# lachinov/brats2019

Measured on AMD Instinct MI355X. Metric: volumes_per_sec_fwd_bwd_128cubed_x4ch, higher is better.
Workload: dtype bf16

## Files before the change

brats2019_amd/_lib.py:

```python
from __future__ import annotations

import ctypes as C
import os

import torch

_PKG = os.path.dirname(os.path.abspath(__file__))
LIB_PATH = os.environ.get("RU_LIB_PATH") or os.path.join(_PKG, "lib", "libresunet_hip.so")

_lib = None
PRECISIONS = {"f32": 0, "bf16x3": 1}
GRAD_PRECISIONS = {"bf16x3": 1, "bf16": 2}
FUSE_GN_BWD_STATS, FUSE_GN_BWD_APPLY, FUSE_SIDE_STREAM, FUSE_BATCH_WREDUCE, FUSE_TAIL_FINALIZE, FUSE_PW_DGRAD = 1, 2, 4, 8, 16, 32

_vp, _f, _d, _i, _sz = C.c_void_p, C.c_float, C.c_double, C.c_int, C.c_size_t

SIGNATURES = {
    "ru_last_error": (C.c_char_p, []),
    "ru_version": (_i, []),
    "ru_device_ok": (_i, []),
    "ru_conv3d_workspace_bytes": (_sz, [_i] * 7),
    "ru_conv3d_fwd": (_i, [_vp, _vp, _vp, _vp] + [_i] * 7 + [_vp, _sz, _vp]),
    "ru_conv3d_bwd_data": (_i, [_vp, _vp, _vp] + [_i] * 7 + [_vp, _sz, _vp]),
    "ru_conv3d_fwd_p": (_i, [_vp, _vp, _vp, _vp] + [_i] * 8 + [_vp, _sz, _vp]),
    "ru_conv3d_bwd_data_p": (_i, [_vp, _vp, _vp] + [_i] * 8 + [_vp, _sz, _vp]),
    "ru_conv3d_bwd_weight": (_i, [_vp, _vp, _vp, _vp] + [_i] * 7 + [_vp, _sz, _vp]),
    "ru_conv3d_bwd_weight_p": (_i, [_vp, _vp, _vp, _vp] + [_i] * 8 + [_vp, _sz, _vp]),
    "ru_groupnorm_workspace_bytes": (_sz, [_i, _i, _sz]),
    "ru_groupnorm_fwd": (_i, [_vp] * 7 + [_i, _i, _sz, _i, _f, _f, _vp, _sz, _vp]),
    "ru_groupnorm_bwd": (_i, [_vp] * 9 + [_i, _i, _sz, _i, _f, _vp, _sz, _vp]),
    "ru_leaky_relu_fwd": (_i, [_vp, _vp, _sz, _f, _vp]),
    "ru_leaky_relu_bwd": (_i, [_vp, _vp, _vp, _sz, _f, _vp]),
    "ru_upsample2x_trilinear_fwd": (_i, [_vp, _vp] + [_i] * 5 + [_vp]),
    "ru_upsample2x_trilinear_bwd": (_i, [_vp, _vp] + [_i] * 5 + [_vp]),
    "ru_sigmoid_fwd": (_i, [_vp, _vp, _sz, _vp]),
    "ru_criterion_workspace_bytes": (_sz, [_i, _i, _sz]),
    "ru_criterion_sums": (_i, [_vp, _vp, _vp, _i, _i, _sz, _f, _vp, _sz, _vp]),
    "ru_criterion_grad": (_i, [_vp, _vp, _vp, _d, _f, _f, _f, _f, _vp, _i, _i, _sz, _vp]),
    "ru_criterion_value": (_i, [C.POINTER(_d), _i, _d, _d, C.POINTER(_d), C.POINTER(_d)]),
    "ru_criterion_value_device": (_i, [_vp, _i, _d, _d, _d, _d, _vp, _vp]),
    "ru_crit_moments_workspace_bytes": (_sz, [_i, _i, _sz]),
    "ru_crit_moments": (_i, [_vp, _vp, _i, _i, _sz, C.c_uint, _vp, _vp, _sz, _vp]),
    "ru_crit_reduce": (_i, [_vp, _i, _i, _vp, _vp]),
    "ru_crit_eval": (_i, [_vp, _vp, _i, _i, _d, _d, _vp, _i, _vp, _vp, _vp]),
    "ru_crit_grad": (_i, [_vp, _vp, _vp, _vp, _i, _i, _sz, _i, _vp, _vp]),
    "ru_adam_amsgrad_step": (_i, [_vp] * 5 + [_sz] + [_f] * 5 + [_i, _vp]),
    "ru_adam_step": (_i, [_vp] * 5 + [_sz] + [_f] * 5 + [_i, _vp]),
    "ru_unet_create": (_vp, [_i, C.POINTER(_i), C.POINTER(_i), C.POINTER(_i), _i]),
    "ru_unet_destroy": (None, [_vp]),
    "ru_unet_set_precision": (_i, [_vp, _i]),
    "ru_unet_freeze_params": (_i, [_vp, _i]),
    "ru_unet_get_precision": (_i, [_vp]),
    "ru_unet_set_grad_precision": (_i, [_vp, _i]),
    "ru_unet_get_grad_precision": (_i, [_vp]),
    "ru_unet_set_fusion": (_i, [_vp, C.c_uint]),
    "ru_unet_probe": (_i, [_vp, _i]),
    "ru_unet_probe_read": (_i, [_vp, C.POINTER(C.c_double), C.POINTER(_i)]),
    "ru_unet_probe_read_families": (_i, [_vp, C.POINTER(C.c_double), C.POINTER(_i), _i]),
    "ru_unet_param_count": (_i, [_vp]),
    "ru_unet_param_name": (C.c_char_p, [_vp, _i]),
    "ru_unet_param_ndim": (_i, [_vp, _i]),
    "ru_unet_param_dim": (_i, [_vp, _i, _i]),
    "ru_unet_param_offset": (_sz, [_vp, _i]),
    "ru_unet_param_total": (_sz, [_vp]),
    "ru_unet_param_is_dead": (_i, [_vp, _i]),
    "ru_unet_workspace_bytes": (_sz, [_vp] + [_i] * 5),
    "ru_unet_forward": (_i, [_vp, _vp, _vp, _vp] + [_i] * 5 + [_vp, _sz, _vp]),
    "ru_unet_backward": (_i, [_vp] * 6),
    "ru_unet_backward_criterion": (_i, [_vp, _vp, _vp, _vp, _d, _f, _f, _f, _f, _vp, _vp, _vp]),
    "ru_unet_gn_stats": (_i, [_vp, _i, _vp, _vp, _vp]),
    "ru_comm_unique_id": (_i, [_vp]),
    "ru_comm_init": (_i, [C.POINTER(_vp), _vp, _i, _i]),
    "ru_comm_destroy": (_i, [_vp]),
    "ru_comm_rank": (_i, [_vp]),
    "ru_comm_world": (_i, [_vp]),
    "ru_allreduce": (_i, [_vp, _vp, _sz, _i, _vp]),
    "ru_comm_group_begin": (_i, []),
    "ru_comm_group_end": (_i, []),
    "ru_tta_merge": (_i, [_vp, _i, C.c_uint, _vp, _vp, _vp, _i, _i, _i, _i, _vp]),
    "ru_compose_labels": (_i, [_vp, _vp, C.c_ulonglong, _vp, _sz, _vp]),
    "ru_dice_counts": (_i, [_vp, _vp, _vp, _i, _i, _sz, _vp]),
    "ru_dice_accumulate": (_i, [_vp, _vp, _i, _i, _i, _vp]),
    "ru_hausdorff_workspace_bytes": (_sz, [_i] * 6),
    "ru_hausdorff_sq": (_i, [_vp, _vp] + [_i] * 6 + [_vp, _vp, _sz, _vp]),
    "ru_hausdorff_accumulate": (_i, [_vp, _vp] + [_i] * 4 + [_vp]),
    "ru_label_confusion": (_i, [_vp, _vp, _i, _i, _i, _sz, _vp, _vp, _vp]),
    "ru_overlap_accumulate": (_i, [_vp, _i, _i, _i, _i, _vp, _vp, _vp]),
    "ru_dice1d_accumulate": (_i, [_vp, _vp, _i, _i, _i, _vp]),
# ... 13 lines not shown
    "ru_case_stats": (_i, [_vp, _vp, _i, _i, _i, _i, C.POINTER(_i), C.POINTER(_i), _vp, _sz, _vp]),
    "ru_case_prepare": (_i, [_vp, _vp, _vp, _i, _i, _i, _i, C.POINTER(_i), C.POINTER(_i), C.POINTER(_i), C.POINTER(_i), _i, C.c_uint, _vp]),
    "ru_tta_merge_box": (_i, [_vp, _i, C.c_uint, _vp, _vp, _vp, _i, _i, _i, _i, C.POINTER(_i), C.POINTER(_i), _vp]),
    "ru_cc_workspace_bytes": (_sz, [_i, _i, _i]),
    "ru_cc_reject": (_i, [_vp, _i, _i, _i, _d, _vp, _sz, _vp]),
    "ru_paste_labels": (_i, [_vp, _vp, _i, _i, _i, C.POINTER(_i), C.POINTER(_i), _vp]),
    "ru_postprocess_workspace_bytes": (_sz, [_i, _i, _i, _i]),
    "ru_postprocess_regions": (_i, [_vp, _vp, _i, _i, _i, _i, C.POINTER(C.c_longlong), C.POINTER(C.c_ulonglong), C.c_uint, C.c_uint, _i, _vp, _vp, _vp, _vp, _sz, _vp]),
    "ru_ens_accumulate": (_i, [_vp, _i, C.c_uint, _vp, _i, _i, _i, _i, _i, C.POINTER(_i), C.POINTER(_i), _vp]),
    "ru_ens_finalize": (_i, [_vp, _i, _vp, _vp, _vp, _i, _sz, _vp]),
    "ru_ens_accumulate_finalize": (_i, [_vp, _i, C.c_uint, _vp, _i, _i, _vp, _vp, _vp, _i, _i, _i, _i, C.POINTER(_i), C.POINTER(_i), _vp]),
    "ru_ens_argmax": (_i, [_vp, _i, _vp, _i, _sz, _vp]),
    "ru_paste_probs": (_i, [_vp, _vp, _i, _i, _i, _i, C.POINTER(_i), C.POINTER(_i), _vp]),
    "ru_unc_accumulate": (_i, [_vp, _i, C.c_uint, _vp, _vp, _i, _i, _i, _i, _i, C.POINTER(_i), C.POINTER(_i), _vp]),
    "ru_unc_accumulate_finalize": (_i, [_vp, _i, C.c_uint, _vp, _vp, _i, _i, _i, _vp, _vp, _vp, _vp, _i, _i, _i, _i, C.POINTER(_i), C.POINTER(_i), _vp]),
    "ru_unc_finalize": (_i, [_vp, _vp, _i, _i, _i, _vp, _vp, _vp, _vp, _i, _sz, _vp]),
    "ru_unc_histogram": (_i, [_vp, _vp, _vp, _i, _i, _i, _vp, _vp, _vp]),
    "ru_unc_score": (_i, [_vp, C.POINTER(_i), _i, _vp, _vp, _vp]),
    "ru_paste_u8c": (_i, [_vp, _vp, _i, _i, _i, _i, C.POINTER(_i), C.POINTER(_i), _vp]),
    "ru_zscore_workspace_bytes": (_sz, [_i, _sz]),
    "ru_zscore_stats": (_i, [_vp, _vp, _i, _sz, _vp, _sz, _vp]),
    "ru_augment_patch": (_i, [_vp, _vp, _vp, _vp, _i, _i, _i, _i, _vp, _vp, _vp, _i, _vp, _vp, _vp, _vp, _vp]),
    "ru_augment_patch_soft": (_i, [_vp, _vp, _vp, _vp, _vp, _i, _i, _i, _i, _vp, _vp, _vp, _i, _vp, _vp, _vp, _vp, _vp]),
    "ru_augment_patch_affine": (_i, [_vp, _vp, _vp, _vp, _vp, _i, _i, _i, _i, _vp, _vp, _vp, _i, _vp, _vp, _i, _vp, _vp, _vp]),
    "ru_elastic_workspace_bytes": (_sz, [_i, _i, _i]),
    "ru_elastic_noise": (_i, [C.c_ulonglong, _i, _i, _i, _vp, _vp]),
    "ru_elastic_field": (_i, [_vp, _d, _d, _i, _i, _i, _vp, _vp, _sz, _vp]),
    "ru_elastic_warp": (_i, [_vp, _i, _vp, _i, _vp, _i, _i, _i, _i, _vp, _vp, _vp, _vp, _vp]),
    "ru_intensity_workspace_bytes": (_sz, [_i, _i, _i, _i]),
    "ru_intensity_augment": (_i, [_vp, _vp, _i, _i, _i, _i, _vp, _vp, _sz, _vp]),
    "ru_layout_convert": (_i, [_vp, _vp, _i, _i, _sz, _i, _vp]),
    "ru_upsample2x_trilinear_fwd_l": (_i, [_vp, _vp] + [_i] * 5 + [_f, _vp]),
    "ru_upsample2x_trilinear_bwd_l": (_i, [_vp, _vp] + [_i] * 5 + [_vp]),
    "ru_conv3d_fwd_l": (_i, [_vp, _vp, _vp, _vp] + [_i] * 7 + [_vp, _sz, _vp]),
    "ru_conv3d_bwd_weight_l": (_i, [_vp, _vp, _vp] + [_i] * 7 + [_vp, _sz, _vp]),
    "ru_conv1_l_workspace_bytes": (_sz, [_i, _i, _i]),
    "ru_conv1_l": (_i, [_vp, _i, _vp, _i, _vp, _i, _vp, _vp, _i, _vp, _f, _vp, _f, _i, _i, _sz, _i, _i, _i, _i, _vp, _vp, _f, _vp, _sz,
                        C.POINTER(_i), C.POINTER(_i), _vp, _sz, _vp]),
    "ru_conv3_l_workspace_bytes": (_sz, [_i] * 7),
    "ru_conv3_l": (_i, [_vp, _vp, _vp, _vp] + [_i] * 8 + [_vp, _vp, _vp, _f, _vp, _vp, _i, _i, _vp, _vp, _f, _vp, _sz, C.POINTER(_i), C.POINTER(_i), _vp, _sz, _vp]),
    "ru_wgrad1_l_workspace_bytes": (_sz, [_i, _i, _i, _sz]),
    "ru_wgrad3_l_workspace_bytes": (_sz, [_i] * 7),
    "ru_wgrad3_l": (_i, [_vp, _vp, _vp] + [_i] * 8 + [_vp, _vp, _f, _i, _i, _vp, _vp, _vp, _vp, _vp, _f, _vp, C.POINTER(_i), _vp, _sz, _vp]),
    "ru_wgrad1_l": (_i, [_vp, _vp, _i, _vp, _vp, _i, _i, _i, _i, _sz] + [_i] * 6 + [_vp, _i, _vp, _vp, _f, C.POINTER(_i), _vp, _sz, _vp]),
}


CRIT_KINDS = {"Dice_loss_joint": 0, "BCE_Loss": 1, "MSE_Loss": 2, "CE_Loss": 3, "Dice1D": 4, "GDL_joint": 5, "sens_loss_joint": 6,
              "Dice_loss_separate": 7}
CRIT_MOMENTS, CRIT_MAX_TERMS = 7, 8
CRIT_MASK_LOGS, CRIT_MASK_ALL = (1 << 4) | (1 << 5), 0x7F
CRIT_M_D2 = 6

CONF_PROB, CONF_LABEL, OVERLAP_MAX_LABELS = 0, 1, 8
OVERLAP_MODES = {"itk": 0, "wt": 1, "validate": 2}

UNC_MEASURES = {"std": 0, "entropy": 1}
UNC_REGIONS, UNC_LEVELS, UNC_CLASSES = 3, 101, 4

SURFACE_PROB, SURFACE_LABEL, SURFACE_REGIONS, SURFACE_COUNTS = 0, 1, 3, 6
SURFACE_COLUMNS = {"dice": 0, "sensitivity": 1, "specificity": 2, "hd95": 3}

LESION_COUNTS, LESION_TABLE_COLUMNS, LESION_CHUNK = 6, 5, 8
LESION_COLUMNS = {"dice": 0, "hd95": 1}

POSTPROCESS_MASKS, POSTPROCESS_LABELS, POSTPROCESS_REGIONS, POSTPROCESS_STATS = 0, 1, 3, 6


INT_BLUR, INT_LOWRES, INT_NOISE, INT_BRIGHTNESS, INT_CONTRAST, INT_GAMMA, INT_GAMMA_INVERT, INT_GAMMA_RETAIN = 1, 2, 4, 8, 16, 32, 64, 128
INT_MAXC, INT_MAX_RADIUS = 8, 8


AFFINE_MAPPINGS = {"default": 0, "row": 1, "brick": 2}


class IntensityParams(C.Structure):
    _fields_ = [("mask", _i * 8), ("blur_sigma", _d * 8), ("lowres_zoom", _d * 8), ("noise_variance", _d * 8), ("noise_seed", C.c_ulonglong * 8),
# ... 66 lines not shown
```

brats2019_amd/csrc/engine.hip:

```cpp
#include "ru_common.h"

#include <vector>
#include <math.h>
#include <stdlib.h>
#include <string.h>

#include <string>
#include <vector>

namespace ru {

static thread_local char g_err[512] = "";
void set_error(const char* fmt, ...) {
    va_list ap;
    va_start(ap, fmt);
    vsnprintf(g_err, sizeof(g_err), fmt, ap);
    va_end(ap);
}
int hip_fail(hipError_t e, const char* what) {
    set_error("%s: %s", what, hipGetErrorString(e));
    return RU_EHIP;
}

constexpr float kSlope = 1e-2f;
// ... 15 lines not shown
        return reinterpret_cast<float*>(base + o);
    }
    float* alloc_keep(size_t nfloats) {
        keep += align_up(nfloats * sizeof(float), 256);
        if (dry) return nullptr;
        const size_t top = cap & ~(size_t)255;
        if (off + keep > top) { failed = true; return nullptr; }
        return reinterpret_cast<float*>(base + top - keep);
    }
    void rewind(size_t mark) { off = mark; }
    size_t need() const { return peak + keep; }
};

static bool env_is(const char* name, char c) { const char* e = getenv(name); return e && *e == c; }
Switches switches_from_env() {
    Switches sw;
    sw.wz = !env_is("RU_WZ", '0');
    sw.wz32 = !(conv3_wz16_form_built() && env_is("RU_WZ32", '0'));
    sw.mx = !env_is("RU_MX", '0');
    sw.mx_wz = sw.mx && !env_is("RU_MX", '1');
    sw.mxg = !env_is("RU_MXG", '0');
    sw.head_form = !env_is("RU_HEAD_FORM", '0');
    sw.head_res = !env_is("RU_HEAD_RES", '0');
    return sw;
}
bool env_trace() { static const bool on = [] { const char* e = getenv("RU_TRACE"); return e && *e && *e != '0'; }(); return on; }
bool env_f32c_off() { static const bool off = env_is("RU_F32C", '0'); return off; }
bool env_sb1_no22() { static const bool on = env_is("RU_SB1_NO22", '1'); return on; }
int env_c1_scatter_cob() { static const int forced = [] { const char* e = getenv("RU_C1_SCATTER_COB"); return e ? atoi(e) : 0; }(); return forced; }
bool env_c1_pair_off() { static const bool off = env_is("RU_C1_PAIR", '0'); return off; }
unsigned env_fusion(unsigned fusion) {
    if (env_is("RU_SIDE_STREAM", '0')) fusion &= ~(unsigned)RU_FUSE_SIDE_STREAM;
    if (const char* e = getenv("RU_FUSION_OFF")) fusion &= ~(unsigned)strtoul(e, nullptr, 0);
    if (const char* e = getenv("RU_FUSION_ON")) fusion |= (unsigned)strtoul(e, nullptr, 0) & 63u;
    return fusion;
}

static int trace_sync(const char* what, hipStream_t s) {
    fprintf(stderr, "[ru] %s\n", what);
    const hipError_t e = hipStreamSynchronize(s);
    if (e != hipSuccess) { fprintf(stderr, "[ru]   -> %s\n", hipGetErrorString(e)); return hip_fail(e, what); }
    return RU_OK;
}

enum { FAM_CONV_L0 = 0, FAM_CONV_DEEP, FAM_WGRAD_L0, FAM_WGRAD_DEEP, FAM_GN, FAM_PW, FAM_OTHER, FAM_COUNT };
enum { INST_CONV16_FWD = 0, INST_CONV16_DGRAD, INST_CONV_DEEP_FWD, INST_CONV_DEEP_DGRAD, INST_WGRAD16_FUSED, INST_WGRAD16_PLAIN, INST_WGRAD_DEEP, INST_COUNT };
struct FamilySink {
    std::vector<hipEvent_t> ev;
    std::vector<int> fam;
    std::vector<int> inst;
    size_t used = 0;
    ~FamilySink() { for (hipEvent_t e : ev) (void)hipEventDestroy(e); }
};
static thread_local FamilySink* t_sink = nullptr;
static thread_local int t_hint_c = 16;
static thread_local int t_hint_inst = -1;
struct RedQueues { WgradRedList main, side; hipStream_t side_stream = nullptr; };
static thread_local RedQueues* t_red = nullptr;
static WgradRedList* red_for(hipStream_t s) { return t_red ? ((t_red->side_stream && s == t_red->side_stream) ? &t_red->side : &t_red->main) : nullptr; }
static int family_of(const char* call) {
    auto has = [&](const char* k) { return strstr(call, k) != nullptr; };
    if (has("wgrad3_launch")) return t_hint_c <= 16 ? FAM_WGRAD_L0 : FAM_WGRAD_DEEP;
    if (has("wgrad_reduce_flush")) return FAM_WGRAD_DEEP;
    if (has("conv3_launch") || has("conv3_sb_launch")) return t_hint_c <= 16 ? FAM_CONV_L0 : FAM_CONV_DEEP;
    if (has("gn_")) return FAM_GN;
    if (has("conv1_") || has("wgrad1_launch") || has("up2_") || has("s2d_launch") || has("d2s_launch") || has("lrelu_bwd_launch")) return FAM_PW;
    return FAM_OTHER;
// ... 51 lines not shown
    size_t offset, numel;
    bool dead;
};

struct BlockP {
    int down = -1, conv1 = -1, conv2 = -1, n1w = -1, n1b = -1, n2w = -1, n2b = -1;
    int cin_down = 0, c = 0;
    size_t pk_f1 = 0, pk_f2 = 0, pk_d1 = 0, pk_d2 = 0, pk_downT = 0, pk_down16 = 0;
    size_t fk_f1 = 0, fk_f2 = 0, fk_d1 = 0, fk_d2 = 0;
};

struct GNSave {
    float *mean = nullptr, *rstd = nullptr, *scale = nullptr, *shift = nullptr;
    float act_slope = 0.01f;
    float* k = nullptr;
};

struct BlockSave {
    const BlockP* bp = nullptr;
    const float* xprev = nullptr;
    float* xs2d = nullptr;
    const float* x = nullptr;
    const GNSave* xg = nullptr;
    float *y1 = nullptr, *y2 = nullptr, *out = nullptr;
    GNSave g1, g2;
    int N = 0, C = 0, D = 0, H = 0, W = 0;
};

struct DecSave {
    const float* z = nullptr;
    float *u = nullptr, *v = nullptr, *c = nullptr;
    const float* skip = nullptr;
    int level = 0;
};

constexpr int kOneProduct = 0x100;
struct ru_unet {
    int depth = 0, nout = 0;
    std::vector<int> enc, dec, ch;
    std::vector<ParamInfo> params;
    size_t total = 0;
    std::vector<std::vector<BlockP>> enc_blocks, dec_blocks;
    std::vector<BlockP> first_blocks;
    std::vector<int> up_w, dec1_w;
    std::vector<size_t> pk_upT, pk_decT;
    int conv_in = -1, nin_w = -1, nin_b = -1, conv_out_w = -1, conv_out_b = -1;
    size_t pk_in = 0, pk_out = 0, pk_out_d = 0, pk_total = 0;
    size_t fk_in = 0, fk_out = 0, fk_out_d = 0, fk_total = 0;
    int precision = RU_PREC_F32;
    unsigned fusion = RU_FUSE_GN_BWD_STATS | RU_FUSE_GN_BWD_APPLY | RU_FUSE_SIDE_STREAM | RU_FUSE_BATCH_WREDUCE | RU_FUSE_PW_DGRAD;
    int grad_precision = RU_PREC_BF16X3;
    int grad_products() const { return (precision == RU_PREC_BF16X3 && grad_precision == RU_PREC_BF16) ? 1 : 3; }
    int wgrad_mode() const { return precision | (grad_products() == 1 ? kOneProduct : 0); }
    bool c16 = false;
    char* fpack = nullptr;

    bool have_fwd = false, training = false;
    int N = 0, D = 0, H = 0, W = 0;
    char* ws = nullptr;
    size_t ws_bytes = 0, fwd_end = 0, fwd_keep = 0;
    float* pack = nullptr;
    const float* x_in = nullptr;
    const float* x_in4 = nullptr;
    bool x_in4_planned = false;
    bool params_frozen = false;
    const float* packed_params = nullptr;
    const void* packed_base = nullptr;
    int packed_prec = -1;
    bool packed_c16 = false;
    ru::Switches sw;
    ru::Switches pack_sw;
    float *y0 = nullptr, *t0 = nullptr, *probs = nullptr;
    GNSave g0;
    const float* head_in = nullptr;
    std::vector<BlockSave> first_s;
    std::vector<std::vector<BlockSave>> enc_s, dec_s;
    std::vector<DecSave> dstage;
    std::vector<const float*> skips;
    std::vector<GNSave> gn_order;
    bool probe_on = false;
    bool probe_families = false;
    ru::FamilySink* sink = nullptr;
    std::vector<hipEvent_t> probe_ev;
// ... 111 lines not shown
    h->pk_out_d = h->pk_total; h->pk_total += conv3_packed_floats(number_of_outputs, ch[0]);
    h->fk_total = 0;
    h->fk_in = h->fk_total; h->fk_total += conv3_sb_frag_bytes(kInCh, ch[0]);
    h->fk_out = h->fk_total; h->fk_total += conv3_sb_frag_bytes(ch[0], number_of_outputs);
    h->fk_out_d = h->fk_total; h->fk_total += conv3_sb_frag_bytes(number_of_outputs, ch[0]);
    for (auto& b : h->first_blocks) assign_block_packs(h, b);
    for (auto& lv : h->enc_blocks) for (auto& b : lv) assign_block_packs(h, b);
    for (int i = 0; i < depth - 1; ++i) for (auto& b : h->dec_blocks[i]) assign_block_packs(h, b);
    for (int i = 0; i < depth - 1; ++i) {
        h->pk_upT.push_back(h->pk_total); h->pk_total += (size_t)ch[i + 1] * ch[i];
        h->pk_decT.push_back(h->pk_total); h->pk_total += (size_t)2 * ch[i] * ch[i];
    }
    return h;
}

extern "C" void ru_unet_destroy(ru_unet_t h) { delete h; }
extern "C" int ru_unet_set_precision(ru_unet_t h, int precision) {
    RU_REQUIRE(h && (precision == RU_PREC_F32 || precision == RU_PREC_BF16X3), "ru_unet_set_precision: bad argument");
    h->precision = precision;
    h->have_fwd = false;
    return RU_OK;
}
extern "C" int ru_unet_get_precision(ru_unet_t h) { return h ? h->precision : -1; }
extern "C" int ru_unet_set_fusion(ru_unet_t h, unsigned mask) {
    RU_REQUIRE(h && (mask & ~(unsigned)(RU_FUSE_GN_BWD_STATS | RU_FUSE_GN_BWD_APPLY | RU_FUSE_SIDE_STREAM | RU_FUSE_BATCH_WREDUCE | RU_FUSE_TAIL_FINALIZE | RU_FUSE_PW_DGRAD)) == 0, "ru_unet_set_fusion: bad argument");
    if ((mask & RU_FUSE_TAIL_FINALIZE) && !h->tickets) {
        hipError_t e = hipMalloc((void**)&h->tickets, 256 * sizeof(unsigned));
        if (e != hipSuccess) { h->tickets = nullptr; (void)hipGetLastError(); }
    }
    h->fusion = mask;
    h->have_fwd = false;
    return RU_OK;
}
extern "C" int ru_unet_probe(ru_unet_t h, int enable) {
    RU_REQUIRE(h, "ru_unet_probe: null handle");
    h->probe_on = enable == 1;
    h->probe_families = enable == 2;
    h->probe_used = 0;
    if (h->probe_families && !h->sink) h->sink = new ru::FamilySink();
    if (h->sink) h->sink->used = 0;
    return RU_OK;
}
extern "C" int ru_unet_probe_read_families(ru_unet_t h, double* ms, int* launches, int nfam) {
    RU_REQUIRE(h && ms && launches && (nfam == ru::FAM_COUNT || nfam == ru::FAM_COUNT + ru::INST_COUNT),
               "ru_unet_probe_read_families: %d families (+ %d instance rows behind them)", (int)ru::FAM_COUNT, (int)ru::INST_COUNT);
    for (int f = 0; f < nfam; ++f) { ms[f] = 0.0; launches[f] = 0; }
    if (!h->sink) return RU_OK;
    ru::FamilySink& k = *h->sink;
    for (size_t i = 0; i + 1 < k.used; i += 2) {
        hipError_t e = hipEventSynchronize(k.ev[i + 1]);
        if (e != hipSuccess) return hip_fail(e, "hipEventSynchronize(family probe)");
        float t = 0.f;
        e = hipEventElapsedTime(&t, k.ev[i], k.ev[i + 1]);
        if (e != hipSuccess) return hip_fail(e, "hipEventElapsedTime(family probe)");
        ms[k.fam[i / 2]] += t;
        launches[k.fam[i / 2]] += 1;
        const int in = k.inst[i / 2];
        if (in >= 0 && ru::FAM_COUNT + in < nfam) { ms[ru::FAM_COUNT + in] += t; launches[ru::FAM_COUNT + in] += 1; }
    }
    k.used = 0;
    return RU_OK;
}
extern "C" int ru_unet_probe_read(ru_unet_t h, double* total_ms, int* launches) {
    RU_REQUIRE(h && total_ms && launches, "ru_unet_probe_read: null argument");
    double sum = 0.0;
    for (size_t i = 0; i + 1 < h->probe_used; i += 2) {
// ... 246 lines not shown
    }
    const float* cur = stem_fused ? h->y0 : h->t0;
    h->first_s.assign(h->first_blocks.size(), BlockSave());
    for (size_t j = 0; j < h->first_blocks.size(); ++j) {
        rc = block_fwd(h, params, A, s, h->first_blocks[j], cur, N, Dl[0], Hl[0], Wl[0], h->first_s[j], &cur, (stem_fused && j == 0) ? &h->g0 : nullptr);
        if (rc) return rc;
    }
    h->skips.assign(depth - 1, nullptr);
    h->enc_s.assign(depth - 1, {});
    for (int i = 0; i < depth - 1; ++i) {
        h->skips[i] = cur;
        h->enc_s[i].assign(h->enc_blocks[i].size(), BlockSave());
        for (size_t j = 0; j < h->enc_blocks[i].size(); ++j) {
            const int lv = j == 0 ? i : i + 1;
            rc = block_fwd(h, params, A, s, h->enc_blocks[i][j], cur, N, Dl[lv], Hl[lv], Wl[lv], h->enc_s[i][j], &cur);
            if (rc) return rc;
        }
    }
    h->dstage.assign(depth - 1, DecSave());
    h->dec_s.assign(depth - 1, {});
    for (int i = depth - 2; i >= 0; --i) {
        DecSave& ds = h->dstage[i];
        ds.level = i;
        ds.z = cur;
        ds.skip = h->skips[i];
        const int Ci = h->ch[i], Cc = h->ch[i + 1];
        const bool recycle = !h->training;
        float* c_early = recycle ? A.alloc((size_t)N * Ci * Vl(i)) : nullptr;
        const size_t dmark = A.off;
        if (!h->c16) {
            ds.u = A.alloc((size_t)N * Cc * Vl(i));
            RU_RUN(up2_fwd_launch(cur, ds.u, N, Cc, Dl[i + 1], Hl[i + 1], Wl[i + 1], s));
        }
        ds.v = A.alloc((size_t)N * Ci * Vl(i));
        Conv1Args c1{};
        c1.x0 = ds.u; c1.C0 = Cc; c1.y = ds.v; c1.out_slope = kSlope;
        c1.N = N; c1.Cout = Ci; c1.V = Vl(i);
        ds.c = recycle ? c_early : A.alloc((size_t)N * Ci * Vl(i));
        Conv1Args c2{};
        c2.x0 = ds.skip; c2.C0 = Ci; c2.x1 = ds.v; c2.C1 = Ci;
        c2.y = ds.c; c2.out_slope = 1.f; c2.N = N; c2.Cout = Ci; c2.V = Vl(i);
        if (h->c16) {
            float* zc = A.alloc((size_t)N * Ci * Vl(i + 1));
            c1.x0 = cur; c1.y = zc; c1.out_slope = 1.f; c1.V = Vl(i + 1);
            c1.wT = P(h, params, h->up_w[i]); c1.ldw = Cc;
            RU_RUN(conv1_16_launch(c1, s));
            RU_RUN(up2_fwd16_launch(zc, ds.v, N, Ci, Dl[i + 1], Hl[i + 1], Wl[i + 1], kSlope, s));
            c2.wT = P(h, params, h->dec1_w[i]); c2.ldw = 2 * Ci;
            RU_RUN(conv1_16_launch(c2, s));
        } else {
            c1.wT = h->pack + h->pk_upT[i]; c1.ldw = Ci;
            RU_RUN(conv1_launch(c1, s));
            c2.wT = h->pack + h->pk_decT[i]; c2.ldw = Ci;
            RU_RUN(conv1_launch(c2, s));
        }
        if (recycle) A.rewind(dmark);
        cur = ds.c;
        h->dec_s[i].assign(h->dec_blocks[i].size(), BlockSave());
        for (size_t j = 0; j < h->dec_blocks[i].size(); ++j) {
            const bool defer = i == 0 && j + 1 == h->dec_blocks[i].size() && h->c16 &&
                               (h->precision == RU_PREC_BF16X3 ? conv3_sb_head_takes_residual(h->sw, N, C0, h->nout, Dl[0], Hl[0], Wl[0])
                                                               : (!h->training && conv3_f32c_head_takes_residual(h->sw, C0, h->nout, Wl[0])));
            rc = block_fwd(h, params, A, s, h->dec_blocks[i][j], cur, N, Dl[i], Hl[i], Wl[i], h->dec_s[i][j], &cur, nullptr, defer);
            if (rc) return rc;
            if (defer) head_block = &h->dec_s[i][j];
        }
    }
    h->head_in = cur;
    t_hint_c = C0;
    float* pdst = probs_out;
    h->probs = probs_out;
    Conv3Args a{};
    a.x = cur; a.wp = h->pack + h->pk_out; a.bias = P(h, params, h->conv_out_b); a.y = pdst; a.sigmoid = 1;
    a.mode = h->precision; a.wfrag = h->fpack + h->fk_out; a.in_c16 = h->c16;
    a.N = N; a.Cin = C0; a.Cout = h->nout; a.D = Dl[0]; a.H = Hl[0]; a.W = Wl[0];
    if (head_block) {
        a.x = head_block->y2; a.in_scale = head_block->g2.scale; a.in_shift = head_block->g2.shift; a.in_slope = kSlope; a.in_res = head_block->x;
        a.in_sum_out = head_block->out;
    }
    RU_RUN(conv3_launch(a, h->sw, s));
// ... 285 lines not shown
    const BlockSave* hb = (depth >= 2 && !h->dec_s[0].empty()) ? &h->dec_s[0].back() : nullptr;
    FusedSums hsums;
    if (head4 && hb && !no_bst && conv3_sb_bst_usable(N, C0, Dl[0], Hl[0], Wl[0])) {
        dh.bst_y = hb->y2; dh.bst_k = hb->g2.k; dh.bst_slope = kSlope;
        hsums.nblk = sb_nblk(h, dh);
        hsums.part = A.alloc((size_t)N * C0 * hsums.nblk * 2);
        hsums.coef = A.alloc((size_t)N * C0 * 3);
        dh.stat_partials = hsums.part;
        if (!A.dry && h->tails()) {
            const BlockP& lb = *hb->bp;
            fill_bwd_tail(h, dh.fin, hsums, hb->g2, P(h, params, lb.n2w), G(h, grads, lb.n2w), G(h, grads, lb.n2b), N, C0, Vl(0), 1);
            hsums.done = true;
        }
    }
    RU_RUN(conv3_launch(dh, h->sw, s));
    const float* dcur = dcur_buf;
    std::vector<const float*> dskip(depth - 1, nullptr);
    FusedSums carry = hsums;
    for (int i = 0; i <= depth - 2; ++i) {
        for (int j = (int)h->dec_s[i].size() - 1; j >= 0; --j) {
            const bool fused2 = carry.nblk > 0 && j == (int)h->dec_s[i].size() - 1;
            const FusedSums sin = carry;
            rc = block_bwd(h, params, grads, A, s, h->dec_s[i][j], dcur, &dcur, nullptr, nullptr, fused2 ? &sin : nullptr);
            if (rc) return rc;
        }
        carry = FusedSums();
        const DecSave& ds = h->dstage[i];
        const int Ci = h->ch[i], Cc = h->ch[i + 1];
        const size_t V = Vl(i);
        const float* wdec = P(h, params, h->dec1_w[i]);
        float* gdec = G(h, grads, h->dec1_w[i]);
        float* dsk = A.alloc((size_t)N * Ci * V);
        float* dv = A.alloc((size_t)N * Ci * V);
        float* dpre = A.alloc((size_t)N * Ci * V);
        const bool dg_fused = c16 && Ci <= 32 && (h->fusion & RU_FUSE_PW_DGRAD);
        if (c16) {
            Wgrad1Args w{};
            w.x = ds.skip; w.x1 = ds.v; w.C0 = Ci; w.dy = dcur; w.dw = gdec; w.ldw = 2 * Ci; w.c16 = 1; w.defer = red_for(s);
            w.ws_bytes = wgrad1_workspace_bytes(N, 2 * Ci, Ci, V);
            w.ws = A.alloc(w.ws_bytes / sizeof(float));
            w.N = N; w.Cin = 2 * Ci; w.Cout = Ci; w.V = V;
            if (dg_fused) { w.dg_w = wdec; w.dg_ldw = 2 * Ci; w.dg_y0 = dsk; w.dg_y1 = dpre; w.dg_mask_slope = kSlope; }
            RU_RUN(wgrad1_launch(w, s));
        } else {
            rc = wgrad1_run(A, s, ds.skip, dcur, gdec, 2 * Ci, N, Ci, Ci, V, c16);
            if (rc) return rc;
            rc = wgrad1_run(A, s, ds.v, dcur, A.dry ? nullptr : gdec + Ci, 2 * Ci, N, Ci, Ci, V, c16);
            if (rc) return rc;
        }
        Conv1Args a1{};
        a1.x0 = dcur; a1.C0 = Ci; a1.y = dsk; a1.out_slope = 1.f; a1.N = N; a1.Cout = Ci; a1.V = V;
        Conv1Args a2 = a1;
        a2.y = dv;
        if (dg_fused) {
        } else if (c16) {
            a1.wT = h->pack + h->pk_decT[i]; a1.ldw = Ci;
            a2.wT = h->pack + h->pk_decT[i] + (size_t)Ci * Ci; a2.ldw = Ci;
            a2.y = dpre; a2.mask = ds.v; a2.mask_slope = kSlope;
            Conv1Args a12 = a1;
            a12.Cout = 2 * Ci; a12.Cout0 = Ci; a12.y1 = dpre; a12.mask = ds.v; a12.mask_slope = kSlope;
            RU_RUN(conv1_16_launch(a12, s));
        } else {
            a1.wT = wdec; a1.ldw = 2 * Ci;
            a2.wT = A.dry ? nullptr : wdec + Ci; a2.ldw = 2 * Ci;
            RU_RUN(conv1_launch(a1, s));
            RU_RUN(conv1_launch(a2, s));
        }
        dskip[i] = dsk;
        if (!c16) RU_RUN(lrelu_bwd_launch(ds.v, dv, dpre, (size_t)N * Ci * V, kSlope, s));
        Conv1Args a3{};
        a3.x0 = dpre; a3.C0 = Ci; a3.out_slope = 1.f; a3.N = N; a3.Cout = Cc; a3.V = V;
        float* dz = A.alloc((size_t)N * Cc * Vl(i + 1));
        float* du = nullptr;
        if (c16) {
            float* dzc = A.alloc((size_t)N * Ci * Vl(i + 1));
            RU_RUN(up2_bwd16_launch(dpre, dzc, N, Ci, Dl[i + 1], Hl[i + 1], Wl[i + 1], s));
            rc = wgrad1_run(A, s, ds.z, dzc, G(h, grads, h->up_w[i]), Cc, N, Cc, Ci, Vl(i + 1), true);
            if (rc) return rc;
            a3.x0 = dzc; a3.y = dz; a3.V = Vl(i + 1);
            a3.wT = h->pack + h->pk_upT[i]; a3.ldw = Ci;
            carry = FusedSums();
            const BlockSave* zb = (i + 1 <= depth - 2) ? (!h->dec_s[i + 1].empty() ? &h->dec_s[i + 1].back() : nullptr)
                                  : (!h->enc_s[depth - 2].empty() ? &h->enc_s[depth - 2].back() : nullptr);
            if (zb && (zb->g2.k || A.dry) && (h->fusion & RU_FUSE_GN_BWD_STATS) && conv1_16_bst_nblk(a3) > 0) {
                carry.nblk = conv1_16_bst_nblk(a3);
                carry.part = A.alloc((size_t)N * Cc * carry.nblk * 2);
                carry.coef = A.alloc((size_t)N * Cc * 3);
                a3.bst_y = zb->y2; a3.bst_k = zb->g2.k; a3.bst_slope = kSlope; a3.stat_partials = carry.part;
            }
            RU_RUN(conv1_16_launch(a3, s));
        } else {
            rc = wgrad1_run(A, s, ds.u, dpre, G(h, grads, h->up_w[i]), Cc, N, Cc, Ci, V, false);
            if (rc) return rc;
            du = A.alloc((size_t)N * Cc * V);
            a3.y = du;
            a3.wT = P(h, params, h->up_w[i]); a3.ldw = Cc;
            RU_RUN(conv1_launch(a3, s));
            RU_RUN(up2_bwd_launch(du, dz, N, Cc, Dl[i + 1], Hl[i + 1], Wl[i + 1], s));
        }
        dcur = dz;
    }
    for (int i = depth - 2; i >= 0; --i) {
        bool joined = false;
        FusedSums snext = carry;
        carry = FusedSums();
        for (int j = (int)h->enc_s[i].size() - 1; j >= 0; --j) {
            GNNext nx{};
            nx.slope = kSlope;
            const BlockSave* pb = j >= 1 ? &h->enc_s[i][j - 1] : (i >= 1 ? (h->enc_s[i - 1].empty() ? nullptr : &h->enc_s[i - 1].back())
// ... 441 lines not shown

extern "C" int ru_tta_merge(const float* probs, int K, unsigned flips, float* mean_out, unsigned char* mask, unsigned long long* counts,
                            int C, int D, int H, int W, ru_stream_t stream) {
    RU_REQUIRE(probs && mask && counts, "ru_tta_merge: null argument");
    return tta_merge_launch(probs, K, flips, mean_out, mask, counts, C, D, H, W, (hipStream_t)stream);
}
extern "C" int ru_compose_labels(const unsigned char* mask, const unsigned long long* counts, unsigned long long et_min, unsigned char* labels,
                                 size_t V, ru_stream_t stream) {
    RU_REQUIRE(mask && counts && labels, "ru_compose_labels: null argument");
    return compose_labels_launch(mask, counts, et_min, labels, V, (hipStream_t)stream);
}

extern "C" int ru_dice_accumulate(const unsigned long long* counts, double* acc, int N, int C, int nacc, ru_stream_t stream) {
    return dice_accumulate_launch(counts, acc, N, C, nacc, (hipStream_t)stream);
}
extern "C" int ru_dice_counts(const float* p, const float* g, unsigned long long* counts, int N, int C, size_t V, ru_stream_t stream) {
    RU_REQUIRE(p && g && counts && N > 0 && C > 0, "ru_dice_counts: bad argument");
    return dice_counts_launch(p, g, counts, N * C, V, (hipStream_t)stream);
}

extern "C" int ru_layout_convert(const float* src, float* dst, int N, int C, size_t V, int to_c16, ru_stream_t stream) {
    RU_REQUIRE(src && dst && N > 0, "ru_layout_convert: bad argument");
    return layout_convert_launch(src, dst, N, C, V, to_c16, (hipStream_t)stream);
}

extern "C" int ru_upsample2x_trilinear_fwd_l(const float* x, float* y, int N, int C, int D, int H, int W, float out_slope, ru_stream_t stream) {
    RU_REQUIRE(x && y && N > 0 && C > 0 && D > 0 && H > 0 && W > 0, "ru_upsample2x_trilinear_fwd_l: bad argument");
    return up2_fwd16_launch(x, y, N, C, D, H, W, out_slope, (hipStream_t)stream);
}
extern "C" int ru_upsample2x_trilinear_bwd_l(const float* dy, float* dx, int N, int C, int D, int H, int W, ru_stream_t stream) {
    RU_REQUIRE(dy && dx && N > 0 && C > 0 && D > 0 && H > 0 && W > 0, "ru_upsample2x_trilinear_bwd_l: bad argument");
    return up2_bwd16_launch(dy, dx, N, C, D, H, W, (hipStream_t)stream);
}
extern "C" int ru_conv3d_fwd_l(const float* x, const float* w, const float* bias, float* y, int N, int Cin, int Cout, int D, int H, int W,
                               int flags, void* ws, size_t ws_bytes, ru_stream_t stream) {
    RU_REQUIRE(x && w && y, "ru_conv3d_fwd_l: null argument");
    const Switches sw = switches_from_env();
    hipStream_t s = (hipStream_t)stream;
    WsCarver C(ws, ws_bytes);
    Conv3Args a{};
    void* wf = C.take(conv3_sb_frag_bytes(Cin, Cout) / 4 + 64);
    RU_WS_OK(C);
    const bool f32 = (flags & 16) != 0;
    a.products = (flags & 32) ? 2 : 0;
    RU_REQUIRE(!f32 || ((flags & 3) != 0 && !(flags & (4 | 8))), "ru_conv3d_fwd_l: the exact-f32 form needs a voxel-major side and takes neither the 4-channel copy nor a split-form input");
    const bool gop = (flags & 64) && !f32 && (flags & 3) == 3 && !(flags & (4 | 8)) && !bias && conv3_mxg_usable(sw, N, Cin, Cout, D, H, W);
    int rc = f32 ? conv3_f32c_pack_weights(w, wf, Cin, Cout, 0, s) : conv3_sb_pack_weights(w, wf, Cin, Cout, 0, s, gop);
    if (rc) return rc;
    a.mode = f32 ? RU_PREC_F32 : RU_PREC_BF16X3; a.wfrag = wf;
    a.in_c16 = flags & 1; a.out_c16 = (flags >> 1) & 1;
    a.in_s16 = (flags >> 3) & 1;
    RU_REQUIRE(!a.in_s16 || a.in_c16, "ru_conv3d_fwd_l: the split form is a voxel-major layout");
    a.x = x; a.bias = bias; a.y = y; a.N = N; a.Cin = Cin; a.Cout = Cout; a.D = D; a.H = H; a.W = W;
    if (gop) {
        const size_t nvox = (size_t)N * D * H * W;
        float* g16 = C.take(nvox * 16);
        RU_WS_OK(C);
        rc = conv3_mxg_split_launch(x, g16, nvox, s);
        if (rc) return rc;
        a.x = g16; a.in_s16 = 1; a.in_g16 = 1; a.products = 0;
    }
    if (flags & 4) {
        RU_REQUIRE(!(flags & 1) && conv3_sb4_usable(N, Cin, Cout, D, H, W), "ru_conv3d_fwd_l: shape does not fit the 4-channel kernel");
        const size_t V = (size_t)D * H * W;
        float* x4 = C.take((size_t)N * 4 * V);
        void* wf4 = C.take(conv3_sb4_frag_bytes(Cout) / 4 + 64);
        RU_WS_OK(C);
        rc = pad_to_c4_launch(x, x4, N, Cin, V, s);
        if (rc) return rc;
        rc = conv3_sb4_pack_weights(w, wf4, Cin, Cout, 0, s);
        if (rc) return rc;
        a.x = x4; a.wfrag = wf4; a.in_c4 = 1;
    }
    return f32 ? conv3_launch(a, sw, s) : conv3_sb_launch(a, sw, s);
}

extern "C" int ru_conv3d_bwd_weight_l(const float* x, const float* dy, float* dw, int N, int Cin, int Cout, int D, int H, int W,
                                      int flags, void* ws, size_t ws_bytes, ru_stream_t stream) {
    RU_REQUIRE(x && dy && dw, "ru_conv3d_bwd_weight_l: null argument");
    WsCarver C(ws, ws_bytes);
    Wgrad3Args a{};
    a.x = x; a.dy = dy; a.dw = dw; a.mode = RU_PREC_BF16X3; a.x_c16 = flags & 1; a.dy_c16 = (flags >> 1) & 1;
    a.N = N; a.Cin = Cin; a.Cout = Cout; a.D = D; a.H = H; a.W = W;
    a.ws_bytes = wgrad3_workspace_bytes(N, Cin, Cout, D, H, W);
    a.ws = C.take(a.ws_bytes / 4);
    RU_WS_OK(C);
    return wgrad3_launch(a, (hipStream_t)stream);
}

extern "C" size_t ru_conv1_l_workspace_bytes(int C0, int Cout, int s2d) {
    return 4096 + (s2d ? 2 * align_up((size_t)C0 * Cout * sizeof(float), 256) : 0);
}
extern "C" int ru_conv1_l(const float* x0, int C0, const float* x1, int C1, const float* w, int ldw, float* y, float* y1, int Cout0,
                          const float* add, float out_slope, const float* mask, float mask_slope, int N, int Cout, size_t V,
                          int s2d, int Dc, int Hc, int Wc, const float* bst_y, const float* bst_k, float bst_slope,
                          float* stat_partials, size_t stat_floats, int* nblk, int* inst, void* ws, size_t ws_bytes, ru_stream_t stream) {
    RU_REQUIRE(x0 && w && y, "ru_conv1_l: null argument");
    RU_REQUIRE(s2d >= 0 && s2d <= 2, "ru_conv1_l: s2d is 0 (plain), 1 (gather) or 2 (scatter)");
    hipStream_t s = (hipStream_t)stream;
    WsCarver C(ws, ws_bytes);
    Conv1Args a{};
    a.x0 = x0; a.C0 = C0; a.x1 = x1; a.C1 = C1; a.wT = w; a.ldw = ldw; a.y = y; a.add = add; a.out_slope = out_slope;
    a.N = N; a.Cout = Cout; a.V = V; a.s2d = s2d; a.Dc = Dc; a.Hc = Hc; a.Wc = Wc; a.mask = mask; a.mask_slope = mask_slope;
    a.y1 = y1; a.Cout0 = Cout0; a.bst_y = bst_y; a.bst_k = bst_k; a.bst_slope = bst_slope; a.stat_partials = stat_partials;
    if (s2d) {
        RU_REQUIRE(C0 > 0 && Cout > 0 && (s2d == 1 ? C0 : Cout) % 8 == 0, "ru_conv1_l: stride-2 modes need 8 x channels on the gathered side");
        const int co = s2d == 1 ? Cout : C0, ci = (s2d == 1 ? C0 : Cout) / 8;
        float* wd = C.take((size_t)8 * ci * co);
        float* wdT = C.take((size_t)8 * ci * co);
        RU_WS_OK(C);
        int rc = pack_down16_launch(w, wd, wdT, co, ci, s);
        if (rc) return rc;
        a.wT = s2d == 1 ? wd : wdT;
        a.ldw = C0;
    }
    if (inst) *inst = conv1_16_choose(a).packed();
    if (nblk) *nblk = 0;
    if (bst_y) {
        const int nb = conv1_16_bst_nblk(a);
        RU_REQUIRE(nb == 0 || (stat_partials && stat_floats >= (size_t)N * (s2d == 2 ? Cout / 8 : Cout) * nb * 2), "ru_conv1_l: statistics buffer too small");
        if (nblk) *nblk = nb;
    }
    return conv1_16_launch(a, s);
}

static size_t c3l_frag_bytes(int Cin, int Cout) { const size_t sb = conv3_sb_frag_bytes(Cin, Cout), f = conv3_f32c_frag_bytes(Cin, Cout); return sb > f ? sb : f; }
extern "C" size_t ru_conv3_l_workspace_bytes(int N, int Cin, int Cout, int D, int H, int W, int flags) {
    const size_t nvox = (size_t)N * D * H * W;
    return 4096 + align_up(c3l_frag_bytes(Cin, Cout) + 256, 256) + ((flags & 4) ? align_up(nvox * 16, 256) + align_up(conv3_sb4_frag_bytes(Cout) + 256, 256) : 0) +
           ((flags & 64) ? align_up(nvox * 64, 256) : 0);
}
extern "C" int ru_conv3_l(const float* x, const float* w, const float* bias, float* y, int N, int Cin, int Cout, int D, int H, int W, int flags, int weight_mode,
                          const float* add, const float* in_scale, const float* in_shift, float in_slope, const float* in_res, float* in_sum_out,
                          int sigmoid, int products, const float* bst_y, const float* bst_k, float bst_slope, float* stat_partials, size_t stat_floats,
                          int* nblk, int* route, void* ws, size_t ws_bytes, ru_stream_t stream) {
    RU_REQUIRE(x && w && y, "ru_conv3_l: null argument");
    RU_REQUIRE(N > 0 && Cin > 0 && Cout > 0 && D > 0 && H > 0 && W > 0, "ru_conv3_l: bad shape");
// ... 16 lines not shown
    RU_REQUIRE(!a.in_s16 || a.in_c16, "ru_conv3_l: the split form is a voxel-major layout");
    a.x = x; a.bias = bias; a.y = y; a.N = N; a.Cin = Cin; a.Cout = Cout; a.D = D; a.H = H; a.W = W;
    a.add = add; a.in_scale = in_scale; a.in_shift = in_shift; a.in_slope = in_slope; a.in_res = in_res; a.in_sum_out = in_sum_out; a.sigmoid = sigmoid;
    a.bst_y = bst_y; a.bst_k = bst_k; a.bst_slope = bst_slope; a.stat_partials = stat_partials;
    if (gop) {
        const size_t nvox = (size_t)N * D * H * W;
        float* g16 = C.take(nvox * 16);
        RU_WS_OK(C);
        rc = conv3_mxg_split_launch(x, g16, nvox, s);
        if (rc) return rc;
        a.x = g16; a.in_s16 = 1; a.in_g16 = 1; a.products = 0;
    }
    if (flags & 4) {
        RU_REQUIRE(!(flags & 1) && conv3_sb4_usable(N, Cin, Cout, D, H, W), "ru_conv3_l: shape does not fit the 4-channel kernel");
        const size_t V = (size_t)D * H * W;
        float* x4 = C.take((size_t)N * 4 * V);
        void* wf4 = C.take(conv3_sb4_frag_bytes(Cout) / 4 + 64);
        RU_WS_OK(C);
        rc = pad_to_c4_launch(x, x4, N, Cin, V, s);
        if (rc) return rc;
        rc = conv3_sb4_pack_weights(w, wf4, Cin_f, Cout_f, weight_mode, s);
        if (rc) return rc;
        a.x = x4; a.wfrag = wf4; a.in_c4 = 1;
    }
    const int r = f32 ? conv3_f32c_route(a) : conv3_sb_route(a, sw);
    if (route) *route = r;
    const int nb = f32 ? conv3_f32c_tiles_per_sample(N, Cin, Cout, D, H, W) : conv3_sb_route_nblk(r, N, Cout, D, H, W);
    if (nblk) *nblk = nb;
    RU_REQUIRE(!stat_partials || stat_floats >= (size_t)N * Cout * nb * 2, "ru_conv3_l: statistics buffer too small");
    return f32 ? conv3_launch(a, sw, s) : conv3_sb_launch(a, sw, s);
}

extern "C" size_t ru_wgrad1_l_workspace_bytes(int N, int Cin, int Cout, size_t V) { return 4096 + align_up(wgrad1_workspace_bytes(N, Cin, Cout, V), 256); }
extern "C" int ru_wgrad1_l(const float* x, const float* x1, int C0, const float* dy, float* dw, int ldw, int N, int Cin, int Cout, size_t V,
                           int c16, int s2d, int Dc, int Hc, int Wc, int tap_split, const float* dg_w, int dg_ldw, float* dg_y0, float* dg_y1,
                           float dg_mask_slope, int* inst, void* ws, size_t ws_bytes, ru_stream_t stream) {
    RU_REQUIRE(x && dy && dw, "ru_wgrad1_l: null argument");
    WsCarver C(ws, ws_bytes);
    Wgrad1Args a{};
    a.x = x; a.x1 = x1; a.C0 = C0; a.dy = dy; a.dw = dw; a.ldw = ldw; a.N = N; a.Cin = Cin; a.Cout = Cout; a.V = V;
    a.c16 = c16; a.s2d = s2d; a.Dc = Dc; a.Hc = Hc; a.Wc = Wc; a.tap_split = tap_split;
    a.dg_w = dg_w; a.dg_ldw = dg_ldw; a.dg_y0 = dg_y0; a.dg_y1 = dg_y1; a.dg_mask_slope = dg_mask_slope;
    RU_REQUIRE(N > 0 && Cin > 0 && Cout > 0 && V > 0, "ru_wgrad1_l: bad shape");
    a.ws_bytes = wgrad1_workspace_bytes(N, Cin, Cout, V);
    a.ws = C.take(a.ws_bytes / 4);
    RU_WS_OK(C);
    if (inst) *inst = wgrad1_inst(a);
    return wgrad1_launch(a, (hipStream_t)stream);
}

extern "C" size_t ru_wgrad3_l_workspace_bytes(int N, int Cin, int Cout, int D, int H, int W, int flags) {
    return 4096 + align_up(wgrad3_tr_workspace_bytes(N, Cin, Cout, D, H, W), 256) + ((flags & 2) ? align_up((size_t)N * D * H * W * 16, 256) : 0) + ((flags & 4) ? align_up((size_t)N * D * H * W * 16, 256) : 0);
}
extern "C" int ru_wgrad3_l(const float* x, const float* dy, float* dw, int N, int Cin, int Cout, int D, int H, int W, int flags, int products,
                           const float* in_scale, const float* in_shift, float in_slope, int dw_cin, int dw_cout,
                           const float* gb_y, const float* gb_d, const float* gb_scale, const float* gb_shift, const float* gb_coef, float gb_slope, float* gb_out,
                           int* inst, void* ws, size_t ws_bytes, ru_stream_t stream) {
    RU_REQUIRE(x && (dy || gb_y) && dw, "ru_wgrad3_l: null argument");
    RU_REQUIRE(N > 0 && Cin > 0 && Cout > 0 && D > 0 && H > 0 && W > 0, "ru_wgrad3_l: bad shape");
    hipStream_t s = (hipStream_t)stream;
    WsCarver C(ws, ws_bytes);
    Wgrad3Args a{};
    a.x = x; a.dy = dy ? dy : gb_y; a.dw = dw; a.mode = RU_PREC_BF16X3; a.x_c16 = 1; a.dy_c16 = 1;
    a.N = N; a.Cin = Cin; a.Cout = Cout; a.D = D; a.H = H; a.W = W;
    a.in_scale = in_scale; a.in_shift = in_shift; a.in_slope = in_slope; a.dw_cin = dw_cin; a.dw_cout = dw_cout;
    a.dy_s16 = flags & 1; a.x_c4 = (flags >> 1) & 1; a.dy_c4 = (flags >> 2) & 1; a.swapped = (flags >> 3) & 1; a.gb_g16 = (flags >> 4) & 1; a.products = products;
    a.gb_y = gb_y; a.gb_d = gb_d; a.gb_scale = gb_scale; a.gb_shift = gb_shift; a.gb_coef = gb_coef; a.gb_slope = gb_slope; a.gb_out = gb_out;
    a.ws_bytes = wgrad3_tr_workspace_bytes(N, Cin, Cout, D, H, W);
    a.ws = C.take(a.ws_bytes / 4);
    RU_WS_OK(C);
    for (int side = 0; side < 2; ++side) {
        if (!(side == 0 ? a.x_c4 : a.dy_c4)) continue;
        const int cfew = side == 0 ? dw_cin : dw_cout;
        const size_t V = (size_t)D * H * W;
        RU_REQUIRE(cfew > 0 && cfew <= 4 && (side == 0 || dy), "ru_wgrad3_l: a 4-channel copy holds 1..4 channels (dw_cin / dw_cout)");
// ... 47 lines not shown
```

brats2019_amd/csrc/pointwise_c16.hip:

```cpp
#include "pw_helpers.hpp"
#include "fin_tail.hpp"
#include <type_traits>
#include <stdlib.h>

namespace ru {

typedef float f32x4_c16 __attribute__((ext_vector_type(4)));
template <int I, int N, class F> __device__ __forceinline__ void static_for_c1_impl(F&& f) {
    if constexpr (I < N) { f(std::integral_constant<int, I>{}); static_for_c1_impl<I + 1, N>(f); }
}
template <int N, class F> __device__ __forceinline__ void static_for_c1(F&& f) { static_for_c1_impl<0, N>(f); }

static inline dim3 c16_grid(size_t V, int blocks_nc, unsigned cap = 2048) {
    size_t bx = (V * 4 + 255) / 256;
    if (bx > cap) bx = cap;
    if (bx < 1) bx = 1;
    return dim3((unsigned)bx, (unsigned)blocks_nc);
}

template <int RES, bool NT = false>
__global__ __launch_bounds__(256) void gn_apply16_kernel(const float* __restrict__ x, const float* __restrict__ scale, const float* __restrict__ shift,
                                                         const float* __restrict__ res, float* __restrict__ y, int C, size_t V, float slope,
                                                         const float* __restrict__ rscale, const float* __restrict__ rshift, float rslope) {
    const int nb = blockIdx.y, CB = C >> 4;
// ... 209 lines not shown
#undef RU_UPX
#pragma unroll
        for (int dz = 0; dz < 2; ++dz) {
            const int zo = 2 * kz + 1 + dz;
            if (zo < 0 || zo >= Do) continue;
            int z0, z1; float lz0, lz1;
            up2_src(zo, D, z0, z1, lz0, lz1);
#pragma unroll
            for (int dy = 0; dy < 2; ++dy) {
                const int yo = 2 * ky + 1 + dy;
                if (yo < 0 || yo >= Ho) continue;
                int y0, y1; float ly0, ly1;
                up2_src(yo, H, y0, y1, ly0, ly1);
                float4 o;
#define RU_UP2(c) o.c = lrelu(lz0 * (ly0 * e00.c + ly1 * e01.c) + lz1 * (ly0 * e10.c + ly1 * e11.c), slope)
                RU_UP2(x); RU_UP2(y); RU_UP2(z); RU_UP2(w);
#undef RU_UP2
                if (nt_out) __builtin_nontemporal_store(f32x4_c16{o.x, o.y, o.z, o.w}, reinterpret_cast<f32x4_c16*>(yp + (((size_t)zo * Ho + yo) * Wo + xo) * 4 + q));
                else yp[(((size_t)zo * Ho + yo) * Wo + xo) * 4 + q] = o;
            }
        }
    }
}
int up2_fwd16_launch(const float* x, float* y, int N, int C, int D, int H, int W, float slope, hipStream_t s) {
    RU_REQUIRE(C % 16 == 0, "up2_fwd16: C must be a multiple of 16");
    const size_t total = (size_t)(D + 1) * (H + 1) * (2 * W) * 4;
    size_t bx = (total + 255) / 256;
    if (bx > 16384) bx = 16384;
    hipLaunchKernelGGL(up2_fwd16_kernel, dim3((unsigned)bx, (unsigned)(N * (C / 16))), dim3(256), 0, s, x, y, D, H, W, slope);
    RU_CHECK_LAUNCH("up2_fwd16_kernel");
    return RU_OK;
}

#ifndef RU_UP2B_ZC
#define RU_UP2B_ZC 8
#endif
constexpr int UP2B_ZC = RU_UP2B_ZC;
__global__ __launch_bounds__(256) void up2_bwd16_kernel(const float* __restrict__ dy, float* __restrict__ dx, int D, int H, int W) {
    const int Do = 2 * D, Ho = 2 * H, Wo = 2 * W;
    const size_t nb = blockIdx.y;
    const size_t Vi = (size_t)D * H * W, Vo = Vi * 8;
    const float4* dp = reinterpret_cast<const float4*>(dy) + nb * Vo * 4;
    float4* op = reinterpret_cast<float4*>(dx) + nb * Vi * 4;
    const int nch = (D + UP2B_ZC - 1) / UP2B_ZC;
    const size_t total = (size_t)nch * H * W * 4;
    for (size_t f = (size_t)blockIdx.x * 256 + threadIdx.x; f < total; f += (size_t)gridDim.x * 256) {
        const int q = (int)(f & 3);
        size_t r = f >> 2;
        const int kx = (int)(r % W); r /= W;
        const int ky = (int)(r % H);
        const int k0 = (int)(r / H) * UP2B_ZC;
        const int k1 = k0 + UP2B_ZC < D ? k0 + UP2B_ZC : D;
        float wy[4], wx[4];
        size_t oy[4], ox[4];
#pragma unroll
        for (int t = 0; t < 4; ++t) {
            const int y = 2 * ky - 1 + t, xx = 2 * kx - 1 + t;
            wy[t] = (y >= 0 && y < Ho) ? up2_coef(y, H, ky) : 0.f;
            wx[t] = (xx >= 0 && xx < Wo) ? up2_coef(xx, W, kx) : 0.f;
            oy[t] = (size_t)(y < 0 ? 0 : (y >= Ho ? Ho - 1 : y)) * Wo;
            ox[t] = (size_t)(xx < 0 ? 0 : (xx >= Wo ? Wo - 1 : xx)) * 4 + q;
        }
        float4 accP = make_float4(0.f, 0.f, 0.f, 0.f), accC = accP;
        for (int m = k0; m <= k1; ++m) {
#pragma unroll
            for (int h = 0; h < 2; ++h) {
                const int z = 2 * m - 1 + h;
                const bool in = z >= 0 && z < Do;
                const size_t zrow = (size_t)(z < 0 ? 0 : (z >= Do ? Do - 1 : z)) * Ho * Wo;
                float4 pz = make_float4(0.f, 0.f, 0.f, 0.f);
#pragma unroll
                for (int b = 0; b < 4; ++b) {
                    const float4* row = dp + (zrow + oy[b]) * 4;
                    const float4 p0 = row[ox[0]], p1 = row[ox[1]], p2 = row[ox[2]], p3 = row[ox[3]];
                    pz.x += wy[b] * (wx[0] * p0.x + wx[1] * p1.x + wx[2] * p2.x + wx[3] * p3.x);
                    pz.y += wy[b] * (wx[0] * p0.y + wx[1] * p1.y + wx[2] * p2.y + wx[3] * p3.y);
                    pz.z += wy[b] * (wx[0] * p0.z + wx[1] * p1.z + wx[2] * p2.z + wx[3] * p3.z);
                    pz.w += wy[b] * (wx[0] * p0.w + wx[1] * p1.w + wx[2] * p2.w + wx[3] * p3.w);
                }
                const float cP = (in && m - 1 >= k0) ? up2_coef(z, D, m - 1) : 0.f;
                const float cC = (in && m < k1) ? up2_coef(z, D, m) : 0.f;
                accP.x += cP * pz.x; accP.y += cP * pz.y; accP.z += cP * pz.z; accP.w += cP * pz.w;
                accC.x += cC * pz.x; accC.y += cC * pz.y; accC.z += cC * pz.z; accC.w += cC * pz.w;
            }
            if (m - 1 >= k0) op[(((size_t)(m - 1) * H + ky) * W + kx) * 4 + q] = accP;
            accP = accC;
            accC = make_float4(0.f, 0.f, 0.f, 0.f);
        }
    }
}
int up2_bwd16_launch(const float* dy, float* dx, int N, int C, int D, int H, int W, hipStream_t s) {
    RU_REQUIRE(C % 16 == 0, "up2_bwd16: C must be a multiple of 16");
    const size_t total = (size_t)((D + UP2B_ZC - 1) / UP2B_ZC) * H * W * 4;
    size_t bx = (total + 255) / 256;
    if (bx > 16384) bx = 16384;
    hipLaunchKernelGGL(up2_bwd16_kernel, dim3((unsigned)bx, (unsigned)(N * (C / 16))), dim3(256), 0, s, dy, dx, D, H, W);
    RU_CHECK_LAUNCH("up2_bwd16_kernel");
    return RU_OK;
}

__global__ void pack_down16_kernel(const float* __restrict__ w, float* __restrict__ wd, float* __restrict__ wdT, int Cout, int Cin) {
    const int i = blockIdx.x * blockDim.x + threadIdx.x;
    if (i >= Cout * Cin * 8) return;
    const int tap = i & 7, c = (i >> 3) % Cin, o = i / (8 * Cin);
    const float v = w[i];
    wd[(size_t)o * 8 * Cin + tap * Cin + c] = v;
    wdT[(size_t)(tap * Cin + c) * Cout + o] = v;
}
int pack_down16_launch(const float* w, float* wd, float* wdT, int Cout, int Cin, hipStream_t s) {
    const int total = Cout * Cin * 8;
    hipLaunchKernelGGL(pack_down16_kernel, dim3(cdiv(total, 256)), dim3(256), 0, s, w, wd, wdT, Cout, Cin);
    RU_CHECK_LAUNCH("pack_down16_kernel");
    return RU_OK;
}

template <int COB, int S2D, int NSLOT, bool PAIR = false>
__global__ __launch_bounds__(256, (PAIR || NSLOT > 0) ? 2 : 1) void conv1_16_kernel(const Conv1Args a, int nvt) {
    static_assert(!PAIR || (S2D == 2 && COB == 4 && (NSLOT == 1 || NSLOT == 2)), "paired stores: the scatter mode with statistics, four blocks per workgroup");
    constexpr bool BST = NSLOT > 0;
    constexpr int NSL = BST ? NSLOT : 1;
    __shared__ float red[BST ? 4 * NSL * 16 * 2 : 1];
    const int lane = threadIdx.x & 63, wave = threadIdx.x >> 6;
    const int n = blockIdx.z, cog = blockIdx.y;
    const size_t V = a.V;
    const int r = lane & 15, g = lane >> 4;
    const int nkb0 = a.C0 >> 4, nkb1 = a.C1 >> 4, nkb = nkb0 + nkb1, CBo = a.Cout >> 4;
    const int Hf = 2 * a.Hc, Wf = 2 * a.Wc;
    const size_t Vf = V * 8;
    const int CBf_out = CBo >> 3;
    const int Cstat = S2D == 2 ? (a.Cout >> 3) : a.Cout;
    f32x4_c16 bs1[NSL], bs2[NSL], bk[NSL][3];
    if constexpr (BST) {
#pragma unroll
        for (int sl = 0; sl < NSL; ++sl) {
            bs1[sl] = f32x4_c16{0.f, 0.f, 0.f, 0.f}; bs2[sl] = f32x4_c16{0.f, 0.f, 0.f, 0.f};
            const int cob = cog * COB + sl, chb = S2D == 2 ? cob % CBf_out : cob;
            const float* kp = a.bst_k + (size_t)n * 3 * Cstat + (cob < CBo ? chb : 0) * 16 + 4 * g;
#pragma unroll
            for (int t3 = 0; t3 < 3; ++t3) { const float4 q = *reinterpret_cast<const float4*>(kp + (size_t)t3 * Cstat); bk[sl][t3] = f32x4_c16{q.x, q.y, q.z, q.w}; }
        }
    }
    const bool nt_out = (size_t)a.N * a.Cout * V * sizeof(float) >= ((size_t)128 << 20);
    const int vt = blockIdx.x * 4 + wave;
    const bool live = vt < nvt;
    if (!live) { if constexpr (!BST) return; }
    if (live) {
    const size_t v0 = (size_t)vt * 64;
    size_t vb[4], fv[4];
#pragma unroll
    for (int t = 0; t < 4; ++t) {
        size_t v = v0 + 16 * t + r;
        if (v >= V) v = V - 1;
        vb[t] = v * 16 + 4 * g;
        fv[t] = 0;
        if constexpr (S2D != 0) {
            const int xc = (int)(v % a.Wc);
            const size_t rr = v / a.Wc;
            const int yc = (int)(rr % a.Hc), zc = (int)(rr / a.Hc);
            fv[t] = ((size_t)(2 * zc) * Hf + 2 * yc) * Wf + 2 * xc;
        }
    }
    const float* wrow[COB];
#pragma unroll
    for (int cb = 0; cb < COB; ++cb) {
        const int cob = cog * COB + cb;
        wrow[cb] = a.wT + (size_t)((cob < CBo ? cob : CBo - 1) * 16 + r) * a.ldw + 4 * g;
    }
    f32x4_c16 acc[4][COB];
#pragma unroll
    for (int t = 0; t < 4; ++t)
#pragma unroll
        for (int cb = 0; cb < COB; ++cb) acc[t][cb] = f32x4_c16{0.f, 0.f, 0.f, 0.f};
    const int CBf_in = nkb0 >> 3;
    auto kstep = [&](int kb) __attribute__((always_inline)) {
        float4 xb[4];
        if constexpr (S2D == 1) {
            const int tap = kb / CBf_in, cbf = kb - tap * CBf_in;
            const size_t toff = ((size_t)(tap >> 2) * Hf + ((tap >> 1) & 1)) * Wf + (tap & 1);
            const float* src = a.x0 + ((size_t)(n * CBf_in + cbf) * Vf) * 16 + 4 * g;
#pragma unroll
            for (int t = 0; t < 4; ++t) xb[t] = *reinterpret_cast<const float4*>(src + (fv[t] + toff) * 16);
        } else {
            const float* src = kb < nkb0 ? a.x0 + ((size_t)(n * nkb0 + kb) * V) * 16 : a.x1 + ((size_t)(n * nkb1 + kb - nkb0) * V) * 16;
#pragma unroll
            for (int t = 0; t < 4; ++t) xb[t] = *reinterpret_cast<const float4*>(src + vb[t]);
        }
#pragma unroll
        for (int cb = 0; cb < COB; ++cb) {
            const float4 wv = *reinterpret_cast<const float4*>(wrow[cb] + kb * 16);
#pragma unroll
            for (int t = 0; t < 4; ++t) {
                acc[t][cb] = __builtin_amdgcn_mfma_f32_16x16x4f32(wv.x, xb[t].x, acc[t][cb], 0, 0, 0);
                acc[t][cb] = __builtin_amdgcn_mfma_f32_16x16x4f32(wv.y, xb[t].y, acc[t][cb], 0, 0, 0);
                acc[t][cb] = __builtin_amdgcn_mfma_f32_16x16x4f32(wv.z, xb[t].z, acc[t][cb], 0, 0, 0);
                acc[t][cb] = __builtin_amdgcn_mfma_f32_16x16x4f32(wv.w, xb[t].w, acc[t][cb], 0, 0, 0);
            }
        }
    };
    int kb = 0;
    for (; kb + 1 < nkb; kb += 2) { kstep(kb); kstep(kb + 1); }
    if (kb < nkb) kstep(kb);
    if constexpr (PAIR) {
        const int k = r & 1;
        constexpr int CBf = NSLOT;
        const bool has_add = a.add != nullptr;
        const float* addp = has_add ? a.add : a.bst_y;
#pragma unroll
        for (int t = 0; t < 4; ++t) {
            size_t idx[2][2];
            bool ok[2];
            int srcl[2];
            float4 dadd[2][2], dyq[2][2];
#pragma unroll
            for (int h = 0; h < 2; ++h) {
// ... 185 lines not shown
    }
    if constexpr (BST) {
#pragma unroll
        for (int sl = 0; sl < NSL; ++sl) {
#pragma unroll
            for (int e = 0; e < 4; ++e) {
#pragma unroll
                for (int o = 1; o < 16; o <<= 1) { bs1[sl][e] += __shfl_xor(bs1[sl][e], o); bs2[sl][e] += __shfl_xor(bs2[sl][e], o); }
            }
            if (r == 0) {
#pragma unroll
                for (int e = 0; e < 4; ++e) { red[((wave * NSL + sl) * 16 + 4 * g + e) * 2] = bs1[sl][e]; red[((wave * NSL + sl) * 16 + 4 * g + e) * 2 + 1] = bs2[sl][e]; }
            }
        }
        __syncthreads();
        const int nblk = S2D == 2 ? gridDim.x * gridDim.y : gridDim.x;
        const int blk = S2D == 2 ? blockIdx.y * gridDim.x + blockIdx.x : blockIdx.x;
        for (int i = threadIdx.x; i < NSL * 16; i += 256) {
            const int slot = i >> 4, c = i & 15;
            const int cob0 = cog * COB + slot;
            if (cob0 >= CBo) continue;
            const int chb = S2D == 2 ? cob0 % CBf_out : cob0;
            float u1 = 0.f, u2 = 0.f;
#pragma unroll
            for (int w = 0; w < 4; ++w) { u1 += red[((w * NSL + slot) * 16 + c) * 2]; u2 += red[((w * NSL + slot) * 16 + c) * 2 + 1]; }
            float* p = a.stat_partials + (((size_t)n * Cstat + chb * 16 + c) * nblk + blk) * 2;
            p[0] = u1; p[1] = u2;
        }
    }
}
Conv1Inst conv1_16_choose(const Conv1Args& a) {
    const int CBo = a.Cout / 16;
    Conv1Inst c{CBo >= 4 ? 4 : (CBo >= 2 ? 2 : 1), a.s2d, 0, 0};
    if (a.s2d == 2) {
        const int forced = env_c1_scatter_cob();
        if ((forced == 2 || forced == 4 || forced == 1) && forced <= CBo) c.cob = forced;
    }
    if (a.bst_y) c.nslot = a.s2d == 2 ? (CBo >> 3) : c.cob;
    c.pair = a.s2d == 2 && a.bst_y && !env_c1_pair_off() && a.Wc % 8 == 0 && c.cob == 4 && !a.mask && (c.nslot == 1 || c.nslot == 2);
    return c;
}
int conv1_16_bst_nblk(const Conv1Args& a) {
    if (a.s2d == 1 || a.y1 || a.Cout % 16 || a.V == 0) return 0;
    const int nvt = (int)((a.V + 63) / 64), CBo = a.Cout / 16;
    const int cob = conv1_16_choose(a).cob;
    const int gx = cdiv(nvt, 4), gy = cdiv(CBo, cob);
    if (a.s2d == 2) {
        const int cbf = CBo >> 3;
        if (a.Cout % 128 || (cbf != 1 && cbf != 2 && cbf != 4) || !(cob % cbf == 0 || cbf % cob == 0)) return 0;
        if (cbf > cob) return 0;
        return gx * gy;
    }
    return gx;
}
int conv1_16_launch(const Conv1Args& a, hipStream_t s) {
    RU_REQUIRE(a.N > 0 && a.C0 > 0 && a.Cout > 0 && a.V > 0, "conv1_16: bad shape");
    RU_REQUIRE(a.C0 % 16 == 0 && a.C1 % 16 == 0 && a.Cout % 16 == 0 && a.ldw >= a.C0 + a.C1 && a.ldw % 4 == 0, "conv1_16: channels must be multiples of 16");
    RU_REQUIRE(!a.y1 || (!a.s2d && !a.add && a.Cout0 > 0 && a.Cout0 < a.Cout && a.Cout0 % 16 == 0), "conv1_16: a split output needs the plain mode, no residual and a split at a multiple of 16");
    if (a.s2d) {
        RU_REQUIRE(a.Dc > 0 && a.Hc > 0 && a.Wc > 0 && (size_t)a.Dc * a.Hc * a.Wc == a.V && a.C1 == 0, "conv1_16: bad stride-2 geometry");
        RU_REQUIRE(a.s2d == 1 ? a.C0 % 128 == 0 : a.Cout % 128 == 0, "conv1_16: stride-2 modes need 8 x (multiple of 16) channels");
    }
    const int nvt = (int)((a.V + 63) / 64), CBo = a.Cout / 16;
    const Conv1Inst c = conv1_16_choose(a);
    const bool bst = a.bst_y != nullptr;
    RU_REQUIRE(!bst || (a.bst_k && a.stat_partials && a.s2d != 1 && !a.y1 && conv1_16_bst_nblk(a) > 0), "conv1_16: fused GroupNorm-backward statistics need the plain or scatter mode with whole channel blocks per workgroup");
    dim3 grid((unsigned)cdiv(nvt, 4), (unsigned)cdiv(CBo, c.cob), (unsigned)a.N);
    switch (c.packed()) {
#define RU_C1_CASE(COB_, S2D_, NSLOT_, PAIR_)                                                                      \
    case COB_ | (S2D_ << 4) | (NSLOT_ << 8) | (PAIR_ << 12):                                                        \
        hipLaunchKernelGGL((conv1_16_kernel<COB_, S2D_, NSLOT_, PAIR_ != 0>), grid, dim3(256), 0, s, a, nvt);       \
        break
        RU_C1_CASE(4, 0, 0, 0); RU_C1_CASE(2, 0, 0, 0); RU_C1_CASE(1, 0, 0, 0);
        RU_C1_CASE(4, 0, 4, 0); RU_C1_CASE(2, 0, 2, 0); RU_C1_CASE(1, 0, 1, 0);
        RU_C1_CASE(4, 1, 0, 0); RU_C1_CASE(2, 1, 0, 0); RU_C1_CASE(1, 1, 0, 0);
        RU_C1_CASE(4, 2, 0, 0); RU_C1_CASE(2, 2, 0, 0); RU_C1_CASE(1, 2, 0, 0);
        RU_C1_CASE(4, 2, 1, 1); RU_C1_CASE(4, 2, 2, 1);
        RU_C1_CASE(4, 2, 1, 0); RU_C1_CASE(4, 2, 2, 0); RU_C1_CASE(4, 2, 4, 0);
        RU_C1_CASE(2, 2, 1, 0); RU_C1_CASE(2, 2, 2, 0); RU_C1_CASE(1, 2, 1, 0);
#undef RU_C1_CASE
    default:
        set_error("conv1_16: no kernel for cob %d, mode %d, %d statistic slots", c.cob, c.s2d, c.nslot);
        return RU_EINVAL;
    }
    RU_CHECK_LAUNCH("conv1_16_kernel");
    return RU_OK;
}

}
```

brats2019_amd/csrc/pw_helpers.hpp:

```cpp
#pragma once
#include "ru_common.h"

namespace ru {

__device__ __forceinline__ float wave_sum(float v) {
#pragma unroll
    for (int o = 32; o > 0; o >>= 1) v += __shfl_xor(v, o);
    return v;
}
__device__ __forceinline__ double wave_sum_d(double v) {
#pragma unroll
    for (int o = 32; o > 0; o >>= 1) v += __shfl_xor(v, o);
    return v;
}
__device__ __forceinline__ float block_sum(float v, float* buf) {
    v = wave_sum(v);
    __syncthreads();
    if ((threadIdx.x & 63) == 0) buf[threadIdx.x >> 6] = v;
    __syncthreads();
    return buf[0] + buf[1] + buf[2] + buf[3];
}
__device__ __forceinline__ double block_sum_d(double v, double* buf) {
    v = wave_sum_d(v);
    __syncthreads();
    if ((threadIdx.x & 63) == 0) buf[threadIdx.x >> 6] = v;
    __syncthreads();
    return buf[0] + buf[1] + buf[2] + buf[3];
}
__device__ __forceinline__ float lrelu(float v, float slope) { return v > 0.f ? v : v * slope; }

static inline unsigned grid1d(size_t n, int per_block, unsigned cap = 1u << 20) {
    size_t b = (n + per_block - 1) / per_block;
    if (b < 1) b = 1;
    return (unsigned)(b > cap ? cap : b);
}

typedef __bf16 pw_bf16x2 __attribute__((ext_vector_type(2)));
typedef unsigned int pw_u32x4 __attribute__((ext_vector_type(4)));
__device__ __forceinline__ void pw_split8(const float (&t)[8], pw_u32x4& hi, pw_u32x4& lo) {
    split_n<4>(t, hi, lo);
}

__device__ __forceinline__ void up2_src(int o, int n, int& i0, int& i1, float& l0, float& l1) {
    float src = 0.5f * (float)o - 0.25f;
    if (src < 0.f) src = 0.f;
    i0 = (int)src;
    l1 = src - (float)i0;
    l0 = 1.f - l1;
    i1 = i0 + (i0 < n - 1 ? 1 : 0);
}

__device__ __forceinline__ float up2_coef(int o, int n, int k) {
    int i0, i1; float l0, l1;
    up2_src(o, n, i0, i1, l0, l1);
    return (i0 == k ? l0 : 0.f) + (i1 == k ? l1 : 0.f);
}

}
```

brats2019_amd/csrc/ru_common.h:

```cpp
#pragma once
#include <hip/hip_runtime.h>
#include <stddef.h>
#include <stdint.h>
#include <stdio.h>
#include <stdarg.h>

#include <vector>

#include "../../include/resunet_hip.h"
#include "switches.hpp"

namespace ru {

typedef __bf16 ru_bf16x2 __attribute__((ext_vector_type(2)));
__device__ __forceinline__ void split_pair(float a, float b, unsigned& hb, unsigned& lb) {
    ru_bf16x2 h;
    h[0] = (__bf16)a;
    h[1] = (__bf16)b;
    hb = __builtin_bit_cast(unsigned, h);
    const float h0 = __builtin_bit_cast(float, __builtin_amdgcn_perm(hb, hb, 0x01000c0cu));
    const float h1 = __builtin_bit_cast(float, hb & 0xffff0000u);
    ru_bf16x2 l;
    l[0] = (__bf16)(a - h0);
    l[1] = (__bf16)(b - h1);
// ... 212 lines not shown
size_t wgrad3_workspace_bytes(int N, int Cin, int Cout, int D, int H, int W);
int wgrad3_launch(const Wgrad3Args& a, hipStream_t s);
struct WgradRedEntry { const float* partials; float* dw; int nparts, taps, CoP, CiP, Cout, Cin, so, sc, split, flip, lo, blk0; };
struct WgradRedList { std::vector<WgradRedEntry> e; };
int wgrad_reduce_launch(const float* partials, int nparts, int taps, int CoP, int CiP, int Cout, int Cin, float* dw, int so, int sc, int split, hipStream_t s,
                        int flip_taps = 0, WgradRedList* defer = nullptr);
int wgrad_reduce_flush(WgradRedList& l, hipStream_t s);
size_t wgrad3_sb_workspace_bytes(int N, int Cin, int Cout, int D, int H, int W);
int wgrad3_sb_launch(const Wgrad3Args& a, hipStream_t s);
size_t wgrad3_tr_workspace_bytes(int N, int Cin, int Cout, int D, int H, int W);
int wgrad3_tr_launch(const Wgrad3Args& a, hipStream_t s);
int wgrad3_tr_inst(const Wgrad3Args& a);

struct Wgrad1Args {
    const float* x;
    const float* dy;
    float* dw;
    int ldw;
    void* ws;
    size_t ws_bytes;
    int N, Cin, Cout;
    size_t V;
    int c16;
    int s2d, Dc, Hc, Wc;
    int tap_split;
    const float* x1;
    int C0;
    struct WgradRedList* defer;
    const float* dg_w;
    int dg_ldw;
    float* dg_y0;
    float* dg_y1;
    float dg_mask_slope;
};
size_t wgrad1_workspace_bytes(int N, int Cin, int Cout, size_t V);
int wgrad1_launch(const Wgrad1Args& a, hipStream_t s);
int wgrad1_inst(const Wgrad1Args& a);

struct Conv1Args {
    const float* x0; int C0;
    const float* x1; int C1;
    const float* wT;
    int ldw;
    float* y;
    const float* add;
    float out_slope;
    int N, Cout;
    size_t V;
    int s2d, Dc, Hc, Wc;
    const float* mask;
    float mask_slope;
    float* y1;
    int Cout0;
    const float* bst_y;
    const float* bst_k;
    float bst_slope;
    float* stat_partials;
};
int conv1_16_bst_nblk(const Conv1Args& a);
int conv1_launch(const Conv1Args& a, hipStream_t s);
int transpose_launch(const float* src, float* dst, int rows, int cols, hipStream_t s);
int layout_convert_launch(const float* src, float* dst, int N, int C, size_t V, int to_c16, hipStream_t s);
int pad_to_c16_launch(const float* src, float* dst, int N, int C, size_t V, hipStream_t s);
int pad_to_c4_launch(const float* src, float* dst, int N, int C, size_t V, hipStream_t s);

int s2d_launch(const float* x, float* y, int N, int C, int D, int H, int W, hipStream_t s);
int d2s_launch(const float* y, float* x, int N, int C, int D, int H, int W, hipStream_t s);

int gn_stats_tiles(size_t V);
int gn_stats_launch(const float* x, float* partials, int N, int C, size_t V, hipStream_t s);
int gn_finalize_launch(const float* partials, int nblk, const float* gamma, const float* beta, float* mean, float* rstd,
                       float* scale, float* shift, int N, int C, size_t V, int G, float eps, hipStream_t s, float* bst_k = nullptr,
                       bool centred = false);
int gn_apply_launch(const float* x, const float* scale, const float* shift, const float* res, float* y,
                    int N, int C, size_t V, float slope, hipStream_t s);
int gn_bwd_tiles(size_t V);
int gn_bwd_reduce_launch(const float* x, const float* dy, const float* scale, const float* shift, const float* mean,
                         const float* rstd, float slope, float* partials, int N, int C, size_t V, int G, hipStream_t s);
int gn_bwd_finalize_launch(const float* partials, int nblk, const float* gamma, const float* mean, const float* rstd,
                           float* coef, float* dgamma, float* dbeta, int N, int C, size_t V, int G, hipStream_t s, int s2_sign = 0);
bool conv3_sb_bst_usable(int N, int Cout, int D, int H, int W);
int gn_bwd_apply_launch(const float* x, const float* dy, const float* scale, const float* shift, const float* coef,
                        float slope, float* dx, int N, int C, size_t V, hipStream_t s);

int lrelu_fwd_launch(const float* x, float* y, size_t n, float slope, hipStream_t s);
int lrelu_bwd_launch(const float* y, const float* dy, float* dx, size_t n, float slope, hipStream_t s);
int sigmoid_launch(const float* x, float* y, size_t n, hipStream_t s);
int sigmoid_bwd_launch(const float* p, const float* dp, float* dz, size_t n, hipStream_t s);
int add_launch(const float* a, const float* b, float* y, size_t n, hipStream_t s);
int fill_launch(float* p, float v, size_t n, hipStream_t s);
int up2_fwd_launch(const float* x, float* y, int N, int C, int D, int H, int W, hipStream_t s);
int up2_bwd_launch(const float* dy, float* dx, int N, int C, int D, int H, int W, hipStream_t s);
int bias_grad_launch(const float* dy, float* db, int N, int C, size_t V, void* ws, size_t ws_bytes, hipStream_t s);
size_t bias_grad_workspace_bytes(int N, int C, size_t V);
int head_grad_c4_launch(const float* p, const float* dp, float* d4, float* db, int N, int C, size_t V, void* ws, size_t ws_bytes, hipStream_t s);
struct CritGradArgs { const float* target; const double* sums; double count; float w_dice, w_bce, bgw, priority; };
int head_grad_c4_crit_launch(const float* p, const CritGradArgs& cg, float* d4, float* db, int N, int C, size_t V, void* ws, size_t ws_bytes, hipStream_t s);

int gn_apply16_launch(const float* x, const float* scale, const float* shift, const float* res, float* y, int N, int C, size_t V, float slope, hipStream_t s,
                      const float* rscale = nullptr, const float* rshift = nullptr, float rslope = 1.f);
int gn_bwd_tiles16(size_t V);
int gn_bwd_reduce16_launch(const float* x, const float* dy, const float* scale, const float* shift, const float* mean, const float* rstd,
                           float slope, float* partials, int N, int C, size_t V, int G, hipStream_t s, const FinTail* fin = nullptr);
int gn_bwd_apply16_launch(const float* x, const float* dy, const float* scale, const float* shift, const float* coef, float slope, float* dx,
                          int N, int C, size_t V, int split, hipStream_t s);
int up2_fwd16_launch(const float* x, float* y, int N, int C, int D, int H, int W, float slope, hipStream_t s);
int up2_bwd16_launch(const float* dy, float* dx, int N, int C, int D, int H, int W, hipStream_t s);
int pack_down16_launch(const float* w, float* wd, float* wdT, int Cout, int Cin, hipStream_t s);
int conv1_16_launch(const Conv1Args& a, hipStream_t s);
struct Conv1Inst { int cob, s2d, nslot, pair; int packed() const { return cob | (s2d << 4) | (nslot << 8) | (pair << 12); } };
Conv1Inst conv1_16_choose(const Conv1Args& a);

int crit_tiles(size_t total);
int crit_sums_launch(const float* p, const float* g, double* sums, int N, int C, size_t V, float bgw, void* ws, size_t ws_bytes, hipStream_t s);
int crit_grad_launch(const float* p, const float* g, const double* sums, double count, float w_dice, float w_bce,
                     float bgw, float priority, float* dp, int N, int C, size_t V, hipStream_t s);
int crit_value_launch(const double* sums, int C, double count, double priority, double w_dice, double w_bce, double* out3, hipStream_t s);
int tta_merge_launch(const float* p, int K, unsigned flips, float* mean_out, unsigned char* mask, unsigned long long* counts, int C, int D, int H, int W, hipStream_t s);
int compose_labels_launch(const unsigned char* mask, const unsigned long long* counts, unsigned long long et_min, unsigned char* labels, size_t V, hipStream_t s);
int dice_counts_launch(const float* p, const float* g, unsigned long long* counts, int rows, size_t V, hipStream_t s);
int dice_accumulate_launch(const unsigned long long* counts, double* acc, int N, int C, int nacc, hipStream_t s);
constexpr int RU_AUG_MAXC = 8;
struct AugmentArgs {
    const float* image;
    const unsigned char* label;
    const float* soft;
    float* data;
    float* target;
    int C, D, H, W;
    int lo[3], P[3];
    double scale[3];
    int flags;
    float mean[RU_AUG_MAXC], istd[RU_AUG_MAXC], gain[RU_AUG_MAXC], bias[RU_AUG_MAXC];
};
size_t zscore_workspace_bytes(int C, size_t V);
int zscore_stats_launch(const float* x, double* stats, int C, size_t V, void* ws, size_t ws_bytes, hipStream_t s);
int augment_patch_launch(const AugmentArgs& a, hipStream_t s);
int adam_launch(float* w, const float* g, float* m, float* v, float* vmax, size_t n, float lr, float b1, float b2,
                float eps, float wd, int step, hipStream_t s);

}
```

brats2019_amd/csrc/wgrad_f32.hip:

```cpp
#include "ru_common.h"

namespace ru {

typedef float f32x4 __attribute__((ext_vector_type(4)));

constexpr int pad2mod4(int v) { return v + ((2 - (v & 3)) & 3); }

template <int TZ, int TY, int OT, int CT>
struct W3 {
    static constexpr int HZ = TZ + 2, HY = TY + 2, HX = 18;
    static constexpr int HVOL = HZ * HY * HX, TVOL = TZ * TY * 16;
    static constexpr int DS = pad2mod4(TVOL), CS = pad2mod4(HVOL);
    static constexpr int LDS_FLOATS = OT * 16 * DS + CT * 16 * CS;
};

template <int NSX, int NSD>
struct W3Slots {
    int gx[NSX];
    int lx[NSX];
    long gd[NSD];
    int n;
};

template <int TZ, int TY, int OT, int CT>
__global__ __launch_bounds__(512, 4) void wgrad3_f32_kernel(const Wgrad3Args a, float* __restrict__ partials,
                                                           int ntz, int nty, int ntx, int ncg, int CoP, int CiP) {
    using P = W3<TZ, TY, OT, CT>;
    constexpr int DS = P::DS, CS = P::CS, HY = P::HY, HX = P::HX, HVOL = P::HVOL, TVOL = P::TVOL;
    constexpr int NROW = P::HZ * HY;
    constexpr int NT = 512;
    constexpr int NSX = (NROW * 6 + NT - 1) / NT;
    constexpr int Q4 = TVOL / 4;
    constexpr int NSD = (OT * 16 * Q4 + NT - 1) / NT;
// ... 344 lines not shown
        hipError_t e = hipFuncSetAttribute(reinterpret_cast<const void*>(wgrad3_f32_kernel<TZ, TY, OT, CT>),
                                           hipFuncAttributeMaxDynamicSharedMemorySize, (int)lds);
        if (e != hipSuccess) return hip_fail(e, "hipFuncSetAttribute(wgrad3)");
        attr_done.set();
    }
    const int CoP = round_up(a.Cout, 16), CiP = round_up(a.Cin, 16);
    dim3 grid(c.nbx, c.ngroups);
    hipLaunchKernelGGL((wgrad3_f32_kernel<TZ, TY, OT, CT>), grid, dim3(512), lds, s, a, (float*)a.ws,
                       cdiv(a.D, TZ), cdiv(a.H, TY), cdiv(a.W, 16), c.ncg, CoP, CiP);
    RU_CHECK_LAUNCH("wgrad3_f32_kernel");
    return wgrad_reduce_launch((const float*)a.ws, (OT == 2 ? 1 : 2) * c.nbx, 27, CoP, CiP, a.Cout, a.Cin, a.dw, a.Cin * 27, 27, 0, s, 0, a.defer);
}

int wgrad3_launch(const Wgrad3Args& a, hipStream_t s) {
    RU_REQUIRE(a.N > 0 && a.Cin > 0 && a.Cout > 0 && a.D > 0 && a.H > 0 && a.W > 0, "wgrad3: bad shape");
    if (a.x_c16 || a.dy_c16) {
        RU_REQUIRE(a.mode == RU_PREC_BF16X3, "wgrad3: voxel-major tensors need the split-bf16 kernel");
        if (a.x_c16 && a.dy_c16) return wgrad3_tr_launch(a, s);
        return wgrad3_sb_launch(a, s);
    }
    if (a.mode == RU_PREC_BF16X3 && (a.W & 3) == 0) return wgrad3_sb_launch(a, s);
    const W3Choice c = wgrad3_choose(a.N, a.Cin, a.Cout, a.D, a.H, a.W);
    if (a.ws_bytes < wgrad3_f32_workspace_bytes(a.N, a.Cin, a.Cout, a.D, a.H, a.W) || !a.ws) {
        set_error("wgrad3: workspace too small");
        return RU_ENOMEM;
    }
    if (c.ot == 2) return wgrad3_cfg<2, 4, 2, 2>(a, c, s);
    return wgrad3_cfg<2, 8, 1, 1>(a, c, s);
}

constexpr int W1_VC = 256;
constexpr int W1_RS = pad2mod4(W1_VC);

template <int OT, int CT>
__global__ __launch_bounds__(256, 2) void wgrad1_f32_kernel(const Wgrad1Args a, float* __restrict__ partials,
                                                           int nchunk, int ncg, int CoP, int CiP) {
    extern __shared__ __attribute__((aligned(16))) float smem[];
    float* dys = smem;
    float* xs = smem + OT * 16 * W1_RS;
    const int tid = threadIdx.x, lane = tid & 63;
    const int wave = __builtin_amdgcn_readfirstlane(tid >> 6);
    const int og = blockIdx.y / ncg, cgp = blockIdx.y % ncg;
    const int o0 = og * OT * 16, c0 = cgp * CT * 16;
    const size_t V = a.V;
    f32x4 acc[OT][CT];
#pragma unroll
    for (int p = 0; p < OT; ++p)
#pragma unroll
        for (int q = 0; q < CT; ++q) acc[p][q] = f32x4{0.f, 0.f, 0.f, 0.f};
    const int abase = (lane & 15) * W1_RS + (lane >> 4) + wave * 64;
    const long ntot = (long)a.N * nchunk;
    const bool dgrad = a.dg_w != nullptr;
    float dgw[CT][OT * 4];
    if (dgrad) {
#pragma unroll
        for (int q = 0; q < CT; ++q)
#pragma unroll
            for (int ks = 0; ks < OT * 4; ++ks) dgw[q][ks] = a.dg_w[(size_t)(4 * ks + (lane >> 4)) * a.dg_ldw + c0 + q * 16 + (lane & 15)];
    }
    for (long t = blockIdx.x; t < ntot; t += gridDim.x) {
        const int n = (int)(t / nchunk);
        const size_t v0 = (size_t)(t % nchunk) * W1_VC;
        __syncthreads();
        if (a.c16) {
            constexpr int ND = OT * 16 * W1_VC / 4 / 256, NX = CT * 16 * W1_VC / 4 / 256;
            float4 dv[ND], xv[NX];
            const int xCB0 = a.x1 ? a.C0 >> 4 : a.Cin >> 4, xCB1 = a.x1 ? (a.Cin - a.C0) >> 4 : 1;
            const float* xsecond = a.x1 ? a.x1 : a.x;
#pragma unroll
            for (int j = 0; j < ND; ++j) {
                const int e4 = tid + j * 256, q = e4 & 3, r = (e4 >> 2) % W1_VC, p = e4 / (4 * W1_VC);
                const int ob = (o0 >> 4) + p;
                const bool ok = v0 + r < V && ob < (a.Cout >> 4);
                const float4 t4 = *reinterpret_cast<const float4*>(a.dy + (ok ? (((size_t)n * (a.Cout >> 4) + ob) * V + v0 + r) * 16 + 4 * q : 0));
                dv[j] = ok ? t4 : make_float4(0.f, 0.f, 0.f, 0.f);
            }
#pragma unroll
            for (int j = 0; j < NX; ++j) {
                const int e4 = tid + j * 256, q = e4 & 3, r = (e4 >> 2) % W1_VC, p = e4 / (4 * W1_VC);
                const bool ok = v0 + r < V && (c0 >> 4) + p < (a.Cin >> 4);
                const size_t vv = ok ? v0 + r : 0;
                size_t off;
                if (a.s2d) {
                    const int CBf = a.Cin >> 7, kb = ok ? (c0 >> 4) + p : 0, tap = kb / CBf, cbf = kb - tap * CBf;
                    const int xc = (int)(vv % a.Wc);
                    const size_t rr = vv / a.Wc;
                    const int yc = (int)(rr % a.Hc), zc = (int)(rr / a.Hc);
                    const size_t fvx = ((size_t)(2 * zc + (tap >> 2)) * (2 * a.Hc) + 2 * yc + ((tap >> 1) & 1)) * (2 * a.Wc) + 2 * xc + (tap & 1);
                    off = (((size_t)n * CBf + cbf) * (V * 8) + fvx) * 16 + 4 * q;
                } else {
                    off = (((size_t)n * (a.Cin >> 4) + (c0 >> 4) + p) * V + vv) * 16 + 4 * q;
                }
                const int kbx = ok ? (c0 >> 4) + p : 0;
                const bool second = kbx >= xCB0;
                const float* xsrc = second ? xsecond : a.x;
                if (!a.s2d) off = (((size_t)n * (second ? xCB1 : xCB0) + (second ? kbx - xCB0 : kbx)) * V + vv) * 16 + 4 * q;
                const float4 t4 = *reinterpret_cast<const float4*>(xsrc + off);
                xv[j] = ok ? t4 : make_float4(0.f, 0.f, 0.f, 0.f);
            }
#pragma unroll
            for (int j = 0; j < ND; ++j) {
                const int e4 = tid + j * 256, q = e4 & 3, r = (e4 >> 2) % W1_VC, p = e4 / (4 * W1_VC);
                float* d = dys + (p * 16 + 4 * q) * W1_RS + r;
                d[0] = dv[j].x; d[W1_RS] = dv[j].y; d[2 * W1_RS] = dv[j].z; d[3 * W1_RS] = dv[j].w;
            }
#pragma unroll
            for (int j = 0; j < NX; ++j) {
                const int e4 = tid + j * 256, q = e4 & 3, r = (e4 >> 2) % W1_VC, p = e4 / (4 * W1_VC);
                float* d = xs + (p * 16 + 4 * q) * W1_RS + r;
                d[0] = xv[j].x; d[W1_RS] = xv[j].y; d[2 * W1_RS] = xv[j].z; d[3 * W1_RS] = xv[j].w;
            }
        } else if ((V & 3) == 0) {
            constexpr int Q4 = W1_VC / 4;
            constexpr int ND = OT * 16 * Q4 / 256, NX = CT * 16 * Q4 / 256;
            float4 dv[ND], xv[NX];
#pragma unroll
            for (int j = 0; j < ND; ++j) {
                const int e4 = tid + j * 256, ch = e4 / Q4, r = (e4 % Q4) * 4, o = o0 + ch;
                const bool ok = o < a.Cout && v0 + r < V;
                const float4 t4 = *reinterpret_cast<const float4*>(a.dy + (ok ? ((size_t)n * a.Cout + o) * V + v0 + r : 0));
                dv[j] = ok ? t4 : make_float4(0.f, 0.f, 0.f, 0.f);
            }
#pragma unroll
            for (int j = 0; j < NX; ++j) {
                const int e4 = tid + j * 256, ch = e4 / Q4, r = (e4 % Q4) * 4, c = c0 + ch;
                const bool ok = c < a.Cin && v0 + r < V;
                const float4 t4 = *reinterpret_cast<const float4*>(a.x + (ok ? ((size_t)n * a.Cin + c) * V + v0 + r : 0));
                xv[j] = ok ? t4 : make_float4(0.f, 0.f, 0.f, 0.f);
            }
#pragma unroll
// ... 10 lines not shown
            }
        } else {
        for (int e = tid; e < OT * 16 * W1_VC; e += 256) {
                const int ch = e / W1_VC, r = e % W1_VC;
                const int o = o0 + ch;
                float v = 0.f;
                if (o < a.Cout && v0 + r < V) v = a.dy[((size_t)n * a.Cout + o) * V + v0 + r];
                dys[ch * W1_RS + r] = v;
            }
            for (int e = tid; e < CT * 16 * W1_VC; e += 256) {
                const int ch = e / W1_VC, r = e % W1_VC;
                const int c = c0 + ch;
                float v = 0.f;
                if (c < a.Cin && v0 + r < V) v = a.x[((size_t)n * a.Cin + c) * V + v0 + r];
                xs[ch * W1_RS + r] = v;
            }
        }
        __syncthreads();
#pragma unroll
        for (int ks = 0; ks < 16; ++ks) {
            float af[OT], bf[CT];
#pragma unroll
            for (int p = 0; p < OT; ++p) af[p] = dys[abase + p * 16 * W1_RS + ks * 4];
#pragma unroll
            for (int q = 0; q < CT; ++q) bf[q] = xs[abase + q * 16 * W1_RS + ks * 4];
#pragma unroll
            for (int p = 0; p < OT; ++p)
#pragma unroll
                for (int q = 0; q < CT; ++q)
                    acc[p][q] = __builtin_amdgcn_mfma_f32_16x16x4f32(af[p], bf[q], acc[p][q], 0, 0, 0);
        }
        if (dgrad) {
            const int xCB0 = a.x1 ? a.C0 >> 4 : a.Cin >> 4, xCB1 = a.x1 ? (a.Cin - a.C0) >> 4 : 1;
#pragma unroll
            for (int vt = 0; vt < 4; ++vt) {
                const int vl = wave * 64 + vt * 16 + (lane & 15);
                const size_t v = v0 + vl;
#pragma unroll
                for (int q = 0; q < CT; ++q) {
                    f32x4 d = f32x4{0.f, 0.f, 0.f, 0.f};
#pragma unroll
                    for (int ks = 0; ks < OT * 4; ++ks)
                        d = __builtin_amdgcn_mfma_f32_16x16x4f32(dgw[q][ks], dys[(4 * ks + (lane >> 4)) * W1_RS + vl], d, 0, 0, 0);
                    const int kb = (c0 >> 4) + q;
                    const bool second = kb >= xCB0;
                    if (second) {
#pragma unroll
                        for (int r = 0; r < 4; ++r) d[r] = xs[(q * 16 + 4 * (lane >> 4) + r) * W1_RS + vl] > 0.f ? d[r] : d[r] * a.dg_mask_slope;
                    }
                    float* dst = second ? a.dg_y1 : a.dg_y0;
                    const size_t idx = (((size_t)n * (second ? xCB1 : xCB0) + (second ? kb - xCB0 : kb)) * V + v) * 16 + 4 * (lane >> 4);
                    if (v < V && kb < (a.Cin >> 4)) *reinterpret_cast<float4*>(dst + idx) = make_float4(d[0], d[1], d[2], d[3]);
                }
            }
        }
    }
    __syncthreads();
    float* red = smem;
#pragma unroll
    for (int p = 0; p < OT; ++p)
#pragma unroll
        for (int q = 0; q < CT; ++q)
#pragma unroll
            for (int r = 0; r < 4; ++r) red[((wave * OT * CT + p * CT + q) * 4 + r) * 64 + lane] = acc[p][q][r];
    __syncthreads();
    for (int e = tid; e < OT * CT * 256; e += 256) {
        const int pq = e >> 8, r = (e >> 6) & 3, ln = e & 63;
        const float v = (red[((0 * OT * CT + pq) * 4 + r) * 64 + ln] + red[((1 * OT * CT + pq) * 4 + r) * 64 + ln]) +
                        (red[((2 * OT * CT + pq) * 4 + r) * 64 + ln] + red[((3 * OT * CT + pq) * 4 + r) * 64 + ln]);
        const int p = pq / CT, q = pq - p * CT;
        const int c = c0 + q * 16 + (ln & 15), o = o0 + p * 16 + (ln >> 4) * 4 + r;
        if (o < CoP && c < CiP) partials[((size_t)blockIdx.x * CoP + o) * CiP + c] = v;
    }
}

constexpr int W1S_NG = 4;
__global__ __launch_bounds__(256, 2) void wgrad1_s2d_kernel(const Wgrad1Args a, float* __restrict__ partials, int nchunk, int ncgb, int CoP, int CiP) {
    constexpr int OT = 2, CT = 2, NG = W1S_NG;
    extern __shared__ __attribute__((aligned(16))) float smem[];
    float* dys = smem;
    float* xs = smem + OT * 16 * W1_RS;
    const int tid = threadIdx.x, lane = tid & 63;
    const int wave = __builtin_amdgcn_readfirstlane(tid >> 6);
    const int og = blockIdx.y / ncgb, cgb = blockIdx.y % ncgb;
    const int o0 = og * OT * 16, cbase = cgb * NG * CT * 16;
// ... 108 lines not shown
static int wgrad1_s2d_nbx(int N, int Cin, int Cout, size_t V) {
    const int ngroups = (Cout / 32) * (Cin / (W1S_NG * 32));
    long nbx = 512 / ngroups;
    if (nbx < 1) nbx = 1;
    const long ntot = (long)N * (long)((V + W1_VC - 1) / W1_VC);
    return (int)(nbx > ntot ? ntot : nbx);
}

struct W1Choice { int ot, ct, nbx, ngroups, ncg, nchunk; };

static W1Choice wgrad1_choose(int N, int Cin, int Cout, size_t V) {
    W1Choice c;
    const int CoP = round_up(Cout, 16), CiP = round_up(Cin, 16);
    c.ot = CoP >= 32 ? 2 : 1;
    c.ct = CiP >= 32 ? 2 : 1;
    c.ncg = cdiv(CiP, 16 * c.ct);
    c.ngroups = cdiv(CoP, 16 * c.ot) * c.ncg;
    c.nchunk = (int)((V + W1_VC - 1) / W1_VC);
    long nbx = 512 / c.ngroups;
    if (nbx < 1) nbx = 1;
    const long ntot = (long)N * c.nchunk;
    if (nbx > ntot) nbx = ntot;
    c.nbx = (int)nbx;
    return c;
}

size_t wgrad1_workspace_bytes(int N, int Cin, int Cout, size_t V) {
    const W1Choice c = wgrad1_choose(N, Cin, Cout, V);
    int nbx = c.nbx;
    if (wgrad1_s2d_usable(Cin, Cout)) { const int n2 = wgrad1_s2d_nbx(N, Cin, Cout, V); if (n2 > nbx) nbx = n2; }
    return (size_t)nbx * round_up(Cout, 16) * round_up(Cin, 16) * sizeof(float);
}

template <int OT, int CT>
static int wgrad1_cfg(const Wgrad1Args& a, const W1Choice& c, hipStream_t s) {
    static PerDevice attr_done;
    const size_t lds = (size_t)(OT + CT) * 16 * W1_RS * sizeof(float);
    if (!attr_done.get()) {
        hipError_t e = hipFuncSetAttribute(reinterpret_cast<const void*>(wgrad1_f32_kernel<OT, CT>),
                                           hipFuncAttributeMaxDynamicSharedMemorySize, (int)lds);
        if (e != hipSuccess) return hip_fail(e, "hipFuncSetAttribute(wgrad1)");
        attr_done.set();
    }
    const int CoP = round_up(a.Cout, 16), CiP = round_up(a.Cin, 16);
    hipLaunchKernelGGL((wgrad1_f32_kernel<OT, CT>), dim3(c.nbx, c.ngroups), dim3(256), lds, s, a, (float*)a.ws, c.nchunk, c.ncg, CoP, CiP);
    RU_CHECK_LAUNCH("wgrad1_f32_kernel");
    return wgrad_reduce_launch((const float*)a.ws, c.nbx, 1, CoP, CiP, a.Cout, a.Cin, a.dw, a.ldw, 1, a.tap_split, s, 0, a.defer);
}

int wgrad1_inst(const Wgrad1Args& a) {
    const W1Choice c = wgrad1_choose(a.N, a.Cin, a.Cout, a.V);
    return c.ot | (c.ct << 4) | ((a.s2d && wgrad1_s2d_usable(a.Cin, a.Cout)) ? 256 : 0) | (a.dg_w ? 512 : 0);
}

int wgrad1_launch(const Wgrad1Args& a, hipStream_t s) {
    RU_REQUIRE(a.N > 0 && a.Cin > 0 && a.Cout > 0 && a.V > 0 && a.ldw >= a.Cin, "wgrad1: bad shape");
    RU_REQUIRE(!a.c16 || (a.Cin % 16 == 0 && a.Cout % 16 == 0), "wgrad1: C16 tensors need channel counts that are multiples of 16");
    RU_REQUIRE(!a.s2d || (a.c16 && a.Cin % 128 == 0 && (size_t)a.Dc * a.Hc * a.Wc == a.V), "wgrad1: bad stride-2 geometry");
    RU_REQUIRE(!a.x1 || (a.c16 && !a.s2d && a.C0 > 0 && a.C0 < a.Cin && a.C0 % 16 == 0), "wgrad1: a second input tensor needs voxel-major tensors and a split at a multiple of 16");
    const W1Choice c = wgrad1_choose(a.N, a.Cin, a.Cout, a.V);
    RU_REQUIRE(!a.dg_w || (a.c16 && !a.s2d && a.Cout == c.ot * 16 && a.Cin % (c.ct * 16) == 0 && a.dg_y0 && (a.dg_y1 || !a.x1) && a.dg_ldw >= a.Cin),
               "wgrad1: the fused data gradient needs voxel-major tensors, Cout <= 32 and whole channel tiles");
    if (!a.ws || a.ws_bytes < wgrad1_workspace_bytes(a.N, a.Cin, a.Cout, a.V)) {
        set_error("wgrad1: workspace too small");
        return RU_ENOMEM;
    }
    const int inst = wgrad1_inst(a);
    if (inst & 256) {
        static PerDevice attr_done;
        const size_t lds = (size_t)4 * 16 * W1_RS * sizeof(float);
        if (!attr_done.get()) {
            hipError_t e = hipFuncSetAttribute(reinterpret_cast<const void*>(wgrad1_s2d_kernel), hipFuncAttributeMaxDynamicSharedMemorySize, (int)lds);
            if (e != hipSuccess) return hip_fail(e, "hipFuncSetAttribute(wgrad1_s2d)");
            attr_done.set();
        }
        const int nbx = wgrad1_s2d_nbx(a.N, a.Cin, a.Cout, a.V), ncgb = a.Cin / (W1S_NG * 32);
        hipLaunchKernelGGL(wgrad1_s2d_kernel, dim3(nbx, (a.Cout / 32) * ncgb), dim3(256), lds, s, a, (float*)a.ws, c.nchunk, ncgb, a.Cout, a.Cin);
        RU_CHECK_LAUNCH("wgrad1_s2d_kernel");
        return wgrad_reduce_launch((const float*)a.ws, nbx, 1, a.Cout, a.Cin, a.Cout, a.Cin, a.dw, a.ldw, 1, a.tap_split, s, 0, a.defer);
    }
    switch (inst & 255) {
    case 2 | (2 << 4): return wgrad1_cfg<2, 2>(a, c, s);
    case 2 | (1 << 4): return wgrad1_cfg<2, 1>(a, c, s);
    case 1 | (2 << 4): return wgrad1_cfg<1, 2>(a, c, s);
    default: return wgrad1_cfg<1, 1>(a, c, s);
    }
}

}
```

brats2019_amd/engine.py:

```python
from __future__ import annotations

import ctypes as C
from collections import OrderedDict

import torch

from . import _lib as L

DEFAULT_CFG = dict(depth=4, encoder_layers=[1, 2, 2, 4], decoder_layers=[1, 1, 1, 1],
                   number_of_channels=[16, 32, 64, 128], number_of_outputs=3)


class ParamLayout:

    def __init__(self, depth, encoder_layers, decoder_layers, number_of_channels, number_of_outputs):
        lib = L.load()
        self.cfg = dict(depth=int(depth), encoder_layers=[int(v) for v in encoder_layers],
                        decoder_layers=[int(v) for v in decoder_layers],
                        number_of_channels=[int(v) for v in number_of_channels], number_of_outputs=int(number_of_outputs))
        arr = lambda v: (C.c_int * len(v))(*v)
        self.handle = lib.ru_unet_create(self.cfg["depth"], arr(self.cfg["encoder_layers"]), arr(self.cfg["decoder_layers"]),
                                         arr(self.cfg["number_of_channels"]), self.cfg["number_of_outputs"])
        if not self.handle:
            raise RuntimeError("ru_unet_create failed: " + L.last_error())
# ... 16 lines not shown
    def views(self, flat):
        out = OrderedDict()
        for name, (shape, off, _dead) in self.entries.items():
            n = 1
            for s in shape:
                n *= s
            out[name] = flat[off:off + n].view(shape)
        return out


class UNetEngine:

    def __init__(self, depth=4, encoder_layers=(1, 2, 2, 4), decoder_layers=(1, 1, 1, 1),
                 number_of_channels=(16, 32, 64, 128), number_of_outputs=3, precision="f32"):
        self.layout = ParamLayout(depth, encoder_layers, decoder_layers, number_of_channels, number_of_outputs)
        self.h = self.layout.handle
        self.grad_precision = "bf16x3"
        self.set_precision(precision)
        self.n_out = int(number_of_outputs)
        self._ws = None
        self._ws_key = None
        self.generation = 0

    def set_precision(self, precision):
        L.check(L.load().ru_unet_set_precision(self.h, L.PRECISIONS[precision]), "ru_unet_set_precision")
        self.precision = precision

    def set_grad_precision(self, grad_precision):
        if grad_precision not in L.GRAD_PRECISIONS:
            raise ValueError("grad_precision must be one of %s" % sorted(L.GRAD_PRECISIONS))
        L.check(L.load().ru_unet_set_grad_precision(self.h, L.GRAD_PRECISIONS[grad_precision]), "ru_unet_set_grad_precision")
        self.grad_precision = grad_precision

    def set_fusion(self, gn_bwd_stats=True, gn_bwd_apply=True, side_stream=True, batch_wreduce=True, tail_finalize=False, pw_dgrad=True):
        mask = ((L.FUSE_GN_BWD_STATS if gn_bwd_stats else 0) | (L.FUSE_GN_BWD_APPLY if gn_bwd_apply else 0) | (L.FUSE_SIDE_STREAM if side_stream else 0) |
                (L.FUSE_BATCH_WREDUCE if batch_wreduce else 0) | (L.FUSE_TAIL_FINALIZE if tail_finalize else 0) | (L.FUSE_PW_DGRAD if pw_dgrad else 0))
        L.check(L.load().ru_unet_set_fusion(self.h, mask), "ru_unet_set_fusion")
        self._ws_key = None

    FAMILIES = ("conv3_l0", "conv3_deep", "wgrad3_l0", "wgrad3_deep", "groupnorm", "pointwise_1x1_s2_up", "other")

    def probe(self, enable=True):
        L.check(L.load().ru_unet_probe(self.h, int(enable)), "ru_unet_probe")

    INSTANCES = ("conv16_fwd", "conv16_dgrad", "conv_deep_fwd", "conv_deep_dgrad", "wgrad16_fused_apply", "wgrad16_plain", "wgrad_deep")

    def probe_read_families(self, instances=False):
        import ctypes
        names = self.FAMILIES + (self.INSTANCES if instances else ())
        n = len(names)
        ms, cnt = (ctypes.c_double * n)(), (ctypes.c_int * n)()
        L.check(L.load().ru_unet_probe_read_families(self.h, ms, cnt, n), "ru_unet_probe_read_families")
        got = {f: (ms[i], cnt[i]) for i, f in enumerate(names)}
        if not instances:
            return got
        return {f: got[f] for f in self.FAMILIES}, {f: got[f] for f in self.INSTANCES}

    def probe_read(self):
        import ctypes
        ms, n = ctypes.c_double(0.0), ctypes.c_int(0)
        L.check(L.load().ru_unet_probe_read(self.h, ctypes.byref(ms), ctypes.byref(n)), "ru_unet_probe_read")
        return ms.value, n.value

    def freeze_params(self, frozen=True):
        frozen = bool(frozen)
        if frozen and getattr(self, "_frozen", False):
            return
        L.check(L.load().ru_unet_freeze_params(self.h, int(frozen)), "ru_unet_freeze_params")
        self._frozen = frozen

# ... 59 lines not shown
```

brats2019_amd/ops.py:

```python
from __future__ import annotations

import collections
import ctypes as C

import torch

from . import _lib as L

LEAKY_SLOPE = 1e-2


def _dims5(x):
    if x.dim() != 5:
        raise ValueError("expected an NCDHW tensor, got shape %s" % (tuple(x.shape),))
    return [int(v) for v in x.shape]


def _prep(t):
    L.require_gpu()
    if t is None:
        return None
    return t.contiguous().float() if (not t.is_contiguous() or t.dtype != torch.float32) else t


# ... 747 lines not shown
    x = _prep(x)
    n, c, d, h, w = _dims5(x)
    y = torch.empty((n, c // 16, d, h, w, 16), dtype=torch.float32, device=x.device)
    L.check(L.load().ru_layout_convert(L.f32(x), L.f32(y), n, c, d * h * w, 1, L.stream()), "ru_layout_convert")
    return y


def from_c16(x):
    x = _prep(x)
    n, cb, d, h, w, _ = (int(v) for v in x.shape)
    y = torch.empty((n, cb * 16, d, h, w), dtype=torch.float32, device=x.device)
    L.check(L.load().ru_layout_convert(L.f32(x), L.f32(y), n, cb * 16, d * h * w, 0, L.stream()), "ru_layout_convert")
    return y


def upsample2x_c16(x, out_slope=1.0):
    x = _prep(x)
    n, cb, d, h, w, _ = (int(v) for v in x.shape)
    y = torch.empty((n, cb, 2 * d, 2 * h, 2 * w, 16), dtype=torch.float32, device=x.device)
    L.check(L.load().ru_upsample2x_trilinear_fwd_l(L.f32(x), L.f32(y), n, cb * 16, d, h, w, float(out_slope), L.stream()),
            "ru_upsample2x_trilinear_fwd_l")
    return y


def upsample2x_bwd_c16(dy):
    dy = _prep(dy)
    n, cb, d2, h2, w2, _ = (int(v) for v in dy.shape)
    dx = torch.empty((n, cb, d2 // 2, h2 // 2, w2 // 2, 16), dtype=torch.float32, device=dy.device)
    L.check(L.load().ru_upsample2x_trilinear_bwd_l(L.f32(dy), L.f32(dx), n, cb * 16, d2 // 2, h2 // 2, w2 // 2, L.stream()),
            "ru_upsample2x_trilinear_bwd_l")
    return dx


def to_split_c16(x_c16):
    hi = x_c16.to(torch.bfloat16)
    lo = (x_c16 - hi.to(torch.float32)).to(torch.bfloat16)
    return torch.cat([hi, lo], dim=-1).contiguous().view(torch.float32)


def conv3d_layout(x, w, bias=None, in_c16=False, out_c16=False, few_channels=False, in_split=False, exact_f32=False, activations=False, gradient=False):
    x, w, bias = _prep(x), _prep(w), _prep(bias)
    if in_c16:
        n, cb, d, h, wd, _ = (int(v) for v in x.shape)
        cin = cb * 16
    else:
        n, cin, d, h, wd = _dims5(x)
    cout = int(w.shape[0])
    y = torch.empty((n, cout // 16, d, h, wd, 16) if out_c16 else (n, cout, d, h, wd), dtype=torch.float32, device=x.device)
    lib = L.load()
    ws = L.workspace(lib.ru_conv3d_workspace_bytes(n, cin, cout, d, h, wd, 3) + (n * d * h * wd * 16 + 65536 if few_channels else 0)
                     + (n * d * h * wd * 64 + 65536 if gradient else 0), x.device)
    L.check(lib.ru_conv3d_fwd_l(L.f32(x), L.f32(w), L.ptr(bias, True), L.f32(y), n, cin, cout, d, h, wd,
                                int(in_c16) | (int(out_c16) << 1) | (int(few_channels) << 2) | (int(in_split) << 3) | (int(exact_f32) << 4) | (int(activations) << 5) | (int(gradient) << 6),
                                L.ptr(ws), ws.numel(), L.stream()), "ru_conv3d_fwd_l")
    return y


def conv3d_bwd_weight_layout(x, dy, x_c16=False, dy_c16=False):
    x, dy = _prep(x), _prep(dy)
    if x_c16:
        n, cb, d, h, wd, _ = (int(v) for v in x.shape)
        cin = cb * 16
    else:
        n, cin, d, h, wd = _dims5(x)
    cout = int(dy.shape[1]) * 16 if dy_c16 else int(dy.shape[1])
    dw = torch.empty((cout, cin, 3, 3, 3), dtype=torch.float32, device=x.device)
    lib = L.load()
    ws = L.workspace(lib.ru_conv3d_workspace_bytes(n, cin, cout, d, h, wd, 3), x.device)
    L.check(lib.ru_conv3d_bwd_weight_l(L.f32(x), L.f32(dy), L.f32(dw), n, cin, cout, d, h, wd, int(x_c16) | (int(dy_c16) << 1),
                                       L.ptr(ws), ws.numel(), L.stream()), "ru_conv3d_bwd_weight_l")
    return dw


Conv1Result = collections.namedtuple("Conv1Result", "y y1 partials nblk inst")
Wgrad1Result = collections.namedtuple("Wgrad1Result", "dw dx0 dx1 inst")


def conv1_inst(packed):
    return packed & 15, (packed >> 4) & 15, (packed >> 8) & 15, bool((packed >> 12) & 1)


def wgrad1_inst(packed):
    return packed & 15, (packed >> 4) & 15, bool(packed & 256), bool(packed & 512)


def conv1x1_c16(x0, w, x1=None, add=None, out_slope=1.0, mask=None, mask_slope=LEAKY_SLOPE, cout0=0, s2d=0,
                bst_y=None, bst_k=None, bst_slope=LEAKY_SLOPE):
    x0, w, x1, add, mask, bst_y, bst_k = (_prep(t) for t in (x0, w, x1, add, mask, bst_y, bst_k))
    lib = L.load()
    n, cb0, d, h, wd, _ = (int(v) for v in x0.shape)
    c0, c1 = cb0 * 16, (int(x1.shape[1]) * 16 if x1 is not None else 0)
    dc, hc, wc, ldw = d, h, wd, 0
    if s2d == 0:
        cout, ldw = int(w.shape[0]), int(w.shape[1])
        out_sp, cstat = (d, h, wd), cout
    elif s2d == 1:
        cout, c0 = int(w.shape[0]), 8 * c0
        dc, hc, wc = d // 2, h // 2, wd // 2
        out_sp, cstat = (dc, hc, wc), cout
    else:
        cout = 8 * int(w.shape[1])
        out_sp, cstat = (2 * d, 2 * h, 2 * wd), cout // 8
    v = dc * hc * wc
    dev = x0.device
    y1 = None
    if cout0:
        y = torch.empty((n, cout0 // 16) + (d, h, wd) + (16,), dtype=torch.float32, device=dev)
        y1 = torch.empty((n, (cout - cout0) // 16) + (d, h, wd) + (16,), dtype=torch.float32, device=dev)
    else:
        y = torch.empty((n, cstat // 16) + out_sp + (16,), dtype=torch.float32, device=dev)
    part, cap = None, 0
    if bst_y is not None:
        cap = n * cstat * ((v + 255) // 256) * max(cout // 16, 1) * 2
        part = torch.zeros(cap, dtype=torch.float32, device=dev)
    ws = L.workspace(lib.ru_conv1_l_workspace_bytes(c0, cout, s2d), dev)
    nblk, inst = C.c_int(0), C.c_int(0)
    L.check(lib.ru_conv1_l(L.f32(x0), c0, L.ptr(x1, True), c1, L.f32(w), ldw, L.f32(y), L.ptr(y1, True), cout0, L.ptr(add, True), float(out_slope),
                           L.ptr(mask, True), float(mask_slope), n, cout, v, s2d, dc, hc, wc, L.ptr(bst_y, True), L.ptr(bst_k, True), float(bst_slope),
                           L.ptr(part, True), cap, C.byref(nblk), C.byref(inst), L.ptr(ws), ws.numel(), L.stream()), "ru_conv1_l")
    if part is not None:
        part = part[:n * cstat * nblk.value * 2].view(n, cstat, nblk.value, 2)
    return Conv1Result(y, y1, part, nblk.value, inst.value)


def conv1x1_bwd_weight_c16(x, dy, x1=None, ldw=None, s2d=False, tap_split=False, dg_w=None, dg_mask_slope=LEAKY_SLOPE):
    x, dy, x1, dg_w = (_prep(t) for t in (x, dy, x1, dg_w))
    lib = L.load()
    n, cbo, d, h, wd, _ = (int(v) for v in dy.shape)
    c0 = int(x.shape[1]) * 16
    cin = 8 * c0 if s2d else c0 + (int(x1.shape[1]) * 16 if x1 is not None else 0)
    cout, v = cbo * 16, d * h * wd
    ldw = cin if ldw is None else int(ldw)
    dev = x.device
    dw = torch.zeros((cout, cin // 8, 2, 2, 2) if tap_split else (cout, ldw), dtype=torch.float32, device=dev)
    dx0 = torch.empty_like(x) if dg_w is not None else None
    dx1 = torch.empty_like(x1) if dg_w is not None and x1 is not None else None
    ws = L.workspace(lib.ru_wgrad1_l_workspace_bytes(n, cin, cout, v), dev)
    inst = C.c_int(0)
    L.check(lib.ru_wgrad1_l(L.f32(x), L.ptr(x1, True), c0 if x1 is not None else 0, L.f32(dy), L.f32(dw), ldw, n, cin, cout, v, 1, int(bool(s2d)), d, h, wd,
                            cin // 8 if tap_split else 0, L.ptr(dg_w, True), int(dg_w.shape[1]) if dg_w is not None else 0, L.ptr(dx0, True), L.ptr(dx1, True),
                            float(dg_mask_slope), C.byref(inst), L.ptr(ws), ws.numel(), L.stream()), "ru_wgrad1_l")
    return Wgrad1Result(dw, dx0, dx1, inst.value)


Conv3Result = collections.namedtuple("Conv3Result", "y in_sum partials nblk route")
Conv3Route = collections.namedtuple("Conv3Route", "family tz ty in16 out16 multi bst add np head grad")
CONV3_FAMILIES = {1: "sb", 2: "sb2", 3: "sb2c4", 4: "wz32", 5: "wz32mx", 6: "mx", 7: "f32c", 8: "wz16"}


def conv3_route(packed):
    bit = lambda b: bool((packed >> b) & 1)
    return Conv3Route(CONV3_FAMILIES.get(packed & 15, "none"), (packed >> 4) & 15, (packed >> 8) & 15, bit(12), bit(13), bit(14), bit(15), bit(16),
                      (packed >> 20) & 3, bit(17), bit(18))


def conv3_fused(x, w, bias=None, in_c16=False, out_c16=False, few_channels=False, in_split=False, exact_f32=False, activations=False, gradient=False,
                add=None, in_scale=None, in_shift=None, in_slope=LEAKY_SLOPE, in_res=None, in_sum_out=None, sigmoid=False, products=0,
                bst_y=None, bst_k=None, bst_slope=LEAKY_SLOPE, stats=None, weight_mode=0):
    x, w, bias, add, in_scale, in_shift, in_res, bst_y, bst_k = (_prep(t) for t in (x, w, bias, add, in_scale, in_shift, in_res, bst_y, bst_k))
    if in_c16:
        n, cb, d, h, wd, _ = (int(v) for v in x.shape)
        cin = cb * 16
    else:
        n, cin, d, h, wd = _dims5(x)
    cout = int(w.shape[1 if weight_mode else 0])
    dev = x.device
    y = torch.empty((n, cout // 16, d, h, wd, 16) if out_c16 else (n, cout, d, h, wd), dtype=torch.float32, device=dev)
    if in_sum_out is True:
        in_sum_out = torch.full_like(x, float("nan"))
    part, cap = None, 0
    if stats is None:
        stats = bst_y is not None
    if stats:
        cap = n * cout * max(((d + 1) // 2) * ((h + 1) // 2) * ((wd + 15) // 16), 1024) * 2
# ... 50 lines not shown
```

include/resunet_hip.h:

```cpp
#ifndef RESUNET_HIP_H_
#define RESUNET_HIP_H_

#include <stddef.h>
#include <stdint.h>

#ifdef __cplusplus
extern "C" {
#endif

#define RU_OK 0
#define RU_EINVAL (-1)
#define RU_ENOMEM (-2)
#define RU_EHIP (-3)
#define RU_ESTATE (-4)

#define RU_PREC_F32 0
#define RU_PREC_BF16X3 1
#define RU_PREC_BF16 2

typedef void* ru_stream_t;
typedef struct ru_unet* ru_unet_t;

const char* ru_last_error(void);
int ru_version(void);
// ... 71 lines not shown
    double priority;
    double bg_weight;
} ru_crit_term_t;
size_t ru_crit_moments_workspace_bytes(int N, int C, size_t V);
int ru_crit_moments(const float* p, const float* g, int N, int C, size_t V, unsigned mask, double* moments,
                    void* ws, size_t ws_bytes, ru_stream_t stream);
int ru_crit_reduce(const double* moments, int N, int C, double* out, ru_stream_t stream);
int ru_crit_eval(const double* totals, const double* moments, int N, int C, double count, double n_global,
                 const ru_crit_term_t* terms, int nterms, double* values, float* coef, ru_stream_t stream);
int ru_crit_grad(const float* p, const float* g, const float* coef, const float* scale, int N, int C, size_t V, int with_logs,
                 float* dp, ru_stream_t stream);

int ru_adam_amsgrad_step(float* w, const float* g, float* m, float* v, float* vmax, size_t n,
                         float lr, float beta1, float beta2, float eps, float weight_decay, int step,
                         ru_stream_t stream);
int ru_adam_step(float* w, const float* g, float* m, float* v, float* vmax_or_null, size_t n,
                 float lr, float beta1, float beta2, float eps, float weight_decay, int step,
                 ru_stream_t stream);

ru_unet_t ru_unet_create(int depth, const int* encoder_layers, const int* decoder_layers,
                         const int* number_of_channels, int number_of_outputs);
void ru_unet_destroy(ru_unet_t h);
int ru_unet_set_precision(ru_unet_t h, int precision);
int ru_unet_freeze_params(ru_unet_t h, int frozen);
int ru_unet_get_precision(ru_unet_t h);
int ru_unet_set_grad_precision(ru_unet_t h, int precision);
int ru_unet_get_grad_precision(ru_unet_t h);
#define RU_FUSE_GN_BWD_STATS 1
#define RU_FUSE_GN_BWD_APPLY 2
#define RU_FUSE_SIDE_STREAM 4
#define RU_FUSE_BATCH_WREDUCE 8
#define RU_FUSE_TAIL_FINALIZE 16
#define RU_FUSE_PW_DGRAD 32
int ru_unet_set_fusion(ru_unet_t h, unsigned mask);
int ru_unet_probe(ru_unet_t h, int enable);
int ru_unet_probe_read(ru_unet_t h, double* total_ms, int* launches);
#define RU_PROBE_FAMILIES 7
#define RU_PROBE_INSTANCES 7
int ru_unet_probe_read_families(ru_unet_t h, double* ms, int* launches, int nfam);
int ru_unet_param_count(ru_unet_t h);
const char* ru_unet_param_name(ru_unet_t h, int i);
int ru_unet_param_ndim(ru_unet_t h, int i);
int ru_unet_param_dim(ru_unet_t h, int i, int d);
size_t ru_unet_param_offset(ru_unet_t h, int i);
size_t ru_unet_param_total(ru_unet_t h);
int ru_unet_param_is_dead(ru_unet_t h, int i);
size_t ru_unet_workspace_bytes(ru_unet_t h, int N, int D, int H, int W, int training);
int ru_unet_forward(ru_unet_t h, const float* params, const float* x, float* probs,
                    int N, int D, int H, int W, int training,
                    void* ws, size_t ws_bytes, ru_stream_t stream);
int ru_unet_backward(ru_unet_t h, const float* params, const float* dprobs, float* grads, float* dx,
                     ru_stream_t stream);
int ru_unet_backward_criterion(ru_unet_t h, const float* params, const float* target, const double* sums, double count,
                               float w_dice, float w_bce, float bg_weight, float priority, float* grads, float* dx,
                               ru_stream_t stream);
int ru_unet_gn_stats(ru_unet_t h, int idx, float* mean, float* rstd, ru_stream_t stream);

typedef struct ru_comm* ru_comm_t;
#define RU_COMM_ID_BYTES 128
#define RU_DT_F32 0
#define RU_DT_F64 1
int ru_comm_unique_id(void* id_out );
int ru_comm_init(ru_comm_t* out, const void* id, int rank, int world);
int ru_comm_destroy(ru_comm_t c);
int ru_comm_rank(ru_comm_t c);
int ru_comm_world(ru_comm_t c);
int ru_allreduce(ru_comm_t c, void* buf, size_t count, int dtype, ru_stream_t stream);
// ... 66 lines not shown
int ru_unc_score(const unsigned long long* hist, const int* thresholds, int T, double* out, double* acc, ru_stream_t stream);
int ru_paste_u8c(const unsigned char* src, unsigned char* full, int C, int D, int H, int W, const int* lo, const int* size, ru_stream_t stream);

int ru_layout_convert(const float* src, float* dst, int N, int C, size_t V, int to_c16, ru_stream_t stream);
int ru_conv3d_fwd_l(const float* x, const float* w, const float* bias, float* y,
                    int N, int Cin, int Cout, int D, int H, int W, int flags,
                    void* ws, size_t ws_bytes, ru_stream_t stream);
int ru_conv3d_bwd_weight_l(const float* x, const float* dy, float* dw,
                           int N, int Cin, int Cout, int D, int H, int W, int flags,
                           void* ws, size_t ws_bytes, ru_stream_t stream);

size_t ru_conv1_l_workspace_bytes(int C0, int Cout, int s2d);
int ru_conv1_l(const float* x0, int C0, const float* x1, int C1, const float* w, int ldw, float* y, float* y1, int Cout0,
               const float* add, float out_slope, const float* mask, float mask_slope, int N, int Cout, size_t V,
               int s2d, int Dc, int Hc, int Wc, const float* bst_y, const float* bst_k, float bst_slope,
               float* stat_partials, size_t stat_floats, int* nblk, int* inst, void* ws, size_t ws_bytes, ru_stream_t stream);
size_t ru_conv3_l_workspace_bytes(int N, int Cin, int Cout, int D, int H, int W, int flags);
int ru_conv3_l(const float* x, const float* w, const float* bias, float* y, int N, int Cin, int Cout, int D, int H, int W, int flags, int weight_mode,
               const float* add, const float* in_scale, const float* in_shift, float in_slope, const float* in_res, float* in_sum_out,
               int sigmoid, int products, const float* bst_y, const float* bst_k, float bst_slope, float* stat_partials, size_t stat_floats,
               int* nblk, int* route, void* ws, size_t ws_bytes, ru_stream_t stream);
size_t ru_wgrad1_l_workspace_bytes(int N, int Cin, int Cout, size_t V);
int ru_wgrad1_l(const float* x, const float* x1, int C0, const float* dy, float* dw, int ldw, int N, int Cin, int Cout, size_t V,
                int c16, int s2d, int Dc, int Hc, int Wc, int tap_split, const float* dg_w, int dg_ldw, float* dg_y0, float* dg_y1,
                float dg_mask_slope, int* inst, void* ws, size_t ws_bytes, ru_stream_t stream);
size_t ru_wgrad3_l_workspace_bytes(int N, int Cin, int Cout, int D, int H, int W, int flags);
int ru_wgrad3_l(const float* x, const float* dy, float* dw, int N, int Cin, int Cout, int D, int H, int W, int flags, int products,
                const float* in_scale, const float* in_shift, float in_slope, int dw_cin, int dw_cout,
                const float* gb_y, const float* gb_d, const float* gb_scale, const float* gb_shift, const float* gb_coef, float gb_slope, float* gb_out,
                int* inst, void* ws, size_t ws_bytes, ru_stream_t stream);

int ru_upsample2x_trilinear_fwd_l(const float* x, float* y, int N, int C, int D, int H, int W, float out_slope, ru_stream_t stream);
int ru_upsample2x_trilinear_bwd_l(const float* dy, float* dx, int N, int C, int D, int H, int W, ru_stream_t stream);

int ru_dice_counts(const float* p, const float* g, unsigned long long* counts, int N, int C, size_t V, ru_stream_t stream);
int ru_dice_accumulate(const unsigned long long* counts, double* acc, int N, int C, int nacc, ru_stream_t stream);

size_t ru_hausdorff_workspace_bytes(int N, int C, int D, int H, int W, int mode);
int ru_hausdorff_sq(const float* p, const float* g, int N, int C, int D, int H, int W, int mode, unsigned long long* out,
                    void* ws, size_t ws_bytes, ru_stream_t stream);
int ru_hausdorff_accumulate(const unsigned long long* sq, double* acc, int N, int K, int nacc, int mode, ru_stream_t stream);

#define RU_CONF_PROB 0
#define RU_CONF_LABEL 1
#define RU_OVERLAP_MAX_LABELS 8
#define RU_OVERLAP_ITK 0
#define RU_OVERLAP_WT 1
#define RU_OVERLAP_VALIDATE 2
int ru_label_confusion(const void* pred, const void* target, int kind, int N, int C, size_t V, unsigned long long* conf,
                       unsigned long long* invalid, ru_stream_t stream);
int ru_overlap_accumulate(const unsigned long long* conf, int N, int L, int mode, int nacc, double* acc, double* out, ru_stream_t stream);
int ru_dice1d_accumulate(const unsigned long long* counts, double* acc, int N, int C, int classes, ru_stream_t stream);
int ru_rmse_accumulate(const double* sums, double* acc, ru_stream_t stream);

#define RU_SURFACE_PROB 0
#define RU_SURFACE_LABEL 1
#define RU_SURFACE_REGIONS 3
#define RU_SURFACE_DICE 0
#define RU_SURFACE_SENS 1
#define RU_SURFACE_SPEC 2
#define RU_SURFACE_HD95 3
#define RU_SURFACE_COUNTS 6
#define RU_SURFACE_C_INVALID 5
size_t ru_surface_workspace_bytes(int kind, int N, int C, int D, int H, int W);
int ru_surface_metrics(const void* pred, const void* target, int kind, int N, int C, int D, int H, int W, double empty_value,
                       double* values, unsigned long long* counts, void* ws, size_t ws_bytes, ru_stream_t stream);
// ... 64 lines not shown
```

Measured before the change: 271.1.

## Store decoder upsample at half depth and expand inside the pointwise convs

The decoder's trilinear 2x upsample now writes only an H/W-upsampled, half-depth intermediate. The 1x1 decoder conv and its weight-gradient kernel expand it along depth on the fly, applying the leaky slope as they read. In the backward pass the fused data-gradient can also emit a half-width gradient that a matching upsample-backward kernel consumes. The goal is to cut memory traffic and allocation for the full-resolution upsampled tensor in both passes, at the cost of more index arithmetic in the consuming kernels and a required consistent fusion mask across forward and backward.

New measurement: 269.6. About the same (-0.6%).

```diff
diff --git a/brats2019_amd/_lib.py b/brats2019_amd/_lib.py
--- a/brats2019_amd/_lib.py
+++ b/brats2019_amd/_lib.py
@@ -11,7 +11,7 @@
 _lib = None
 PRECISIONS = {"f32": 0, "bf16x3": 1}
 GRAD_PRECISIONS = {"bf16x3": 1, "bf16": 2}
-FUSE_GN_BWD_STATS, FUSE_GN_BWD_APPLY, FUSE_SIDE_STREAM, FUSE_BATCH_WREDUCE, FUSE_TAIL_FINALIZE, FUSE_PW_DGRAD = 1, 2, 4, 8, 16, 32
+FUSE_GN_BWD_STATS, FUSE_GN_BWD_APPLY, FUSE_SIDE_STREAM, FUSE_BATCH_WREDUCE, FUSE_TAIL_FINALIZE, FUSE_PW_DGRAD, FUSE_UP_HALF = 1, 2, 4, 8, 16, 32, 64
 
 _vp, _f, _d, _i, _sz = C.c_void_p, C.c_float, C.c_double, C.c_int, C.c_size_t
 
@@ -54,6 +54,7 @@
     "ru_unet_set_grad_precision": (_i, [_vp, _i]),
     "ru_unet_get_grad_precision": (_i, [_vp]),
     "ru_unet_set_fusion": (_i, [_vp, C.c_uint]),
+    "ru_unet_set_up_half": (_i, [_vp, _i]),
     "ru_unet_probe": (_i, [_vp, _i]),
     "ru_unet_probe_read": (_i, [_vp, C.POINTER(C.c_double), C.POINTER(_i)]),
     "ru_unet_probe_read_families": (_i, [_vp, C.POINTER(C.c_double), C.POINTER(_i), _i]),
@@ -133,17 +134,23 @@
     "ru_layout_convert": (_i, [_vp, _vp, _i, _i, _sz, _i, _vp]),
     "ru_upsample2x_trilinear_fwd_l": (_i, [_vp, _vp] + [_i] * 5 + [_f, _vp]),
     "ru_upsample2x_trilinear_bwd_l": (_i, [_vp, _vp] + [_i] * 5 + [_vp]),
+    "ru_upsample2x_trilinear_fwd_half_l": (_i, [_vp, _vp] + [_i] * 5 + [_vp]),
+    "ru_upsample2x_trilinear_half_expand_l": (_i, [_vp, _vp] + [_i] * 5 + [_f, _vp]),
+    "ru_upsample2x_trilinear_bwd_hx_l": (_i, [_vp, _vp] + [_i] * 5 + [_vp]),
     "ru_conv3d_fwd_l": (_i, [_vp, _vp, _vp, _vp] + [_i] * 7 + [_vp, _sz, _vp]),
     "ru_conv3d_bwd_weight_l": (_i, [_vp, _vp, _vp] + [_i] * 7 + [_vp, _sz, _vp]),
     "ru_conv1_l_workspace_bytes": (_sz, [_i, _i, _i]),
     "ru_conv1_l": (_i, [_vp, _i, _vp, _i, _vp, _i, _vp, _vp, _i, _vp, _f, _vp, _f, _i, _i, _sz, _i, _i, _i, _i, _vp, _vp, _f, _vp, _sz,
                         C.POINTER(_i), C.POINTER(_i), _vp, _sz, _vp]),
+    "ru_conv1_uph_l": (_i, [_vp, _i, _vp, _i, _vp, _i, _vp, _vp, _i, _vp, _f, _vp, _f, _i, _i, _sz, _i, _i, _i, _i, _vp, _vp, _f, _vp, _sz,
+                            C.POINTER(_i), C.POINTER(_i), _vp, _sz, _vp, _i, _i, _i, _f]),
     "ru_conv3_l_workspace_bytes": (_sz, [_i] * 7),
     "ru_conv3_l": (_i, [_vp, _vp, _vp, _vp] + [_i] * 8 + [_vp, _vp, _vp, _f, _vp, _vp, _i, _i, _vp, _vp, _f, _vp, _sz, C.POINTER(_i), C.POINTER(_i), _vp, _sz, _vp]),
     "ru_wgrad1_l_workspace_bytes": (_sz, [_i, _i, _i, _sz]),
     "ru_wgrad3_l_workspace_bytes": (_sz, [_i] * 7),
     "ru_wgrad3_l": (_i, [_vp, _vp, _vp] + [_i] * 8 + [_vp, _vp, _f, _i, _i, _vp, _vp, _vp, _vp, _vp, _f, _vp, C.POINTER(_i), _vp, _sz, _vp]),
     "ru_wgrad1_l": (_i, [_vp, _vp, _i, _vp, _vp, _i, _i, _i, _i, _sz] + [_i] * 6 + [_vp, _i, _vp, _vp, _f, C.POINTER(_i), _vp, _sz, _vp]),
+    "ru_wgrad1_uph_l": (_i, [_vp, _vp, _i, _vp, _vp, _i, _i, _i, _i, _sz] + [_i] * 6 + [_vp, _i, _vp, _vp, _f, C.POINTER(_i), _vp, _sz, _vp, _i, _i, _i, _f, _i]),
 }
 
 
diff --git a/brats2019_amd/csrc/engine.hip b/brats2019_amd/csrc/engine.hip
--- a/brats2019_amd/csrc/engine.hip
+++ b/brats2019_amd/csrc/engine.hip
@@ -71,7 +71,7 @@
 unsigned env_fusion(unsigned fusion) {
     if (env_is("RU_SIDE_STREAM", '0')) fusion &= ~(unsigned)RU_FUSE_SIDE_STREAM;
     if (const char* e = getenv("RU_FUSION_OFF")) fusion &= ~(unsigned)strtoul(e, nullptr, 0);
-    if (const char* e = getenv("RU_FUSION_ON")) fusion |= (unsigned)strtoul(e, nullptr, 0) & 63u;
+    if (const char* e = getenv("RU_FUSION_ON")) fusion |= (unsigned)strtoul(e, nullptr, 0) & 127u;
     return fusion;
 }
 
@@ -189,6 +189,7 @@
     float *u = nullptr, *v = nullptr, *c = nullptr;
     const float* skip = nullptr;
     int level = 0;
+    bool v_half = false;
 };
 
 constexpr int kOneProduct = 0x100;
@@ -205,7 +206,7 @@
     size_t pk_in = 0, pk_out = 0, pk_out_d = 0, pk_total = 0;
     size_t fk_in = 0, fk_out = 0, fk_out_d = 0, fk_total = 0;
     int precision = RU_PREC_F32;
-    unsigned fusion = RU_FUSE_GN_BWD_STATS | RU_FUSE_GN_BWD_APPLY | RU_FUSE_SIDE_STREAM | RU_FUSE_BATCH_WREDUCE | RU_FUSE_PW_DGRAD;
+    unsigned fusion = RU_FUSE_GN_BWD_STATS | RU_FUSE_GN_BWD_APPLY | RU_FUSE_SIDE_STREAM | RU_FUSE_BATCH_WREDUCE | RU_FUSE_PW_DGRAD | RU_FUSE_UP_HALF;
     int grad_precision = RU_PREC_BF16X3;
     int grad_products() const { return (precision == RU_PREC_BF16X3 && grad_precision == RU_PREC_BF16) ? 1 : 3; }
     int wgrad_mode() const { return precision | (grad_products() == 1 ? kOneProduct : 0); }
@@ -383,6 +384,12 @@
     h->have_fwd = false;
     return RU_OK;
 }
+extern "C" int ru_unet_set_up_half(ru_unet_t h, int on) {
+    RU_REQUIRE(h, "ru_unet_set_up_half: null handle");
+    h->fusion = on ? (h->fusion | RU_FUSE_UP_HALF) : (h->fusion & ~(unsigned)RU_FUSE_UP_HALF);
+    h->have_fwd = false;
+    return RU_OK;
+}
 extern "C" int ru_unet_probe(ru_unet_t h, int enable) {
     RU_REQUIRE(h, "ru_unet_probe: null handle");
     h->probe_on = enable == 1;
@@ -695,7 +702,8 @@
             ds.u = A.alloc((size_t)N * Cc * Vl(i));
             RU_RUN(up2_fwd_launch(cur, ds.u, N, Cc, Dl[i + 1], Hl[i + 1], Wl[i + 1], s));
         }
-        ds.v = A.alloc((size_t)N * Ci * Vl(i));
+        ds.v_half = h->c16 && Ci <= 32 && (h->fusion & RU_FUSE_PW_DGRAD) && (h->fusion & RU_FUSE_UP_HALF);
+        ds.v = A.alloc(ds.v_half ? (size_t)N * Ci * Vl(i + 1) * 4 : (size_t)N * Ci * Vl(i));
         Conv1Args c1{};
         c1.x0 = ds.u; c1.C0 = Cc; c1.y = ds.v; c1.out_slope = kSlope;
         c1.N = N; c1.Cout = Ci; c1.V = Vl(i);
@@ -708,7 +716,12 @@
             c1.x0 = cur; c1.y = zc; c1.out_slope = 1.f; c1.V = Vl(i + 1);
             c1.wT = P(h, params, h->up_w[i]); c1.ldw = Cc;
             RU_RUN(conv1_16_launch(c1, s));
-            RU_RUN(up2_fwd16_launch(zc, ds.v, N, Ci, Dl[i + 1], Hl[i + 1], Wl[i + 1], kSlope, s));
+            if (ds.v_half) {
+                RU_RUN(up2_fwd16_half_launch(zc, ds.v, N, Ci, Dl[i + 1], Hl[i + 1], Wl[i + 1], s));
+                c2.x1_half = 1; c2.x1h_D = Dl[i + 1]; c2.x1h_plane = (size_t)4 * Hl[i + 1] * Wl[i + 1]; c2.x1h_slope = kSlope;
+            } else {
+                RU_RUN(up2_fwd16_launch(zc, ds.v, N, Ci, Dl[i + 1], Hl[i + 1], Wl[i + 1], kSlope, s));
+            }
             c2.wT = P(h, params, h->dec1_w[i]); c2.ldw = 2 * Ci;
             RU_RUN(conv1_16_launch(c2, s));
         } else {
@@ -1060,8 +1073,10 @@
         float* gdec = G(h, grads, h->dec1_w[i]);
         float* dsk = A.alloc((size_t)N * Ci * V);
         float* dv = A.alloc((size_t)N * Ci * V);
-        float* dpre = A.alloc((size_t)N * Ci * V);
+        const bool dpre_hx = ds.v_half && wgrad1_hx_usable(Wl[i + 1]);
+        float* dpre = A.alloc(dpre_hx ? (size_t)N * Ci * V / 2 : (size_t)N * Ci * V);
         const bool dg_fused = c16 && Ci <= 32 && (h->fusion & RU_FUSE_PW_DGRAD);
+        RU_REQUIRE(!ds.v_half || dg_fused, "ru_unet_backward: the fusion mask changed between the forward and the backward pass");
         if (c16) {
             Wgrad1Args w{};
             w.x = ds.skip; w.x1 = ds.v; w.C0 = Ci; w.dy = dcur; w.dw = gdec; w.ldw = 2 * Ci; w.c16 = 1; w.defer = red_for(s);
@@ -1069,6 +1084,7 @@
             w.ws = A.alloc(w.ws_bytes / sizeof(float));
             w.N = N; w.Cin = 2 * Ci; w.Cout = Ci; w.V = V;
             if (dg_fused) { w.dg_w = wdec; w.dg_ldw = 2 * Ci; w.dg_y0 = dsk; w.dg_y1 = dpre; w.dg_mask_slope = kSlope; }
+            if (ds.v_half) { w.x1_half = 1; w.x1h_D = Dl[i + 1]; w.x1h_plane = (size_t)4 * Hl[i + 1] * Wl[i + 1]; w.x1h_slope = kSlope; w.dg_hx = dpre_hx; w.dg_hx_W = Wl[i + 1]; }
             RU_RUN(wgrad1_launch(w, s));
         } else {
             rc = wgrad1_run(A, s, ds.skip, dcur, gdec, 2 * Ci, N, Ci, Ci, V, c16);
@@ -1102,7 +1118,8 @@
         float* du = nullptr;
         if (c16) {
             float* dzc = A.alloc((size_t)N * Ci * Vl(i + 1));
-            RU_RUN(up2_bwd16_launch(dpre, dzc, N, Ci, Dl[i + 1], Hl[i + 1], Wl[i + 1], s));
+            if (dpre_hx) RU_RUN(up2_bwd16_hx_launch(dpre, dzc, N, Ci, Dl[i + 1], Hl[i + 1], Wl[i + 1], s));
+            else RU_RUN(up2_bwd16_launch(dpre, dzc, N, Ci, Dl[i + 1], Hl[i + 1], Wl[i + 1], s));
             rc = wgrad1_run(A, s, ds.z, dzc, G(h, grads, h->up_w[i]), Cc, N, Cc, Ci, Vl(i + 1), true);
             if (rc) return rc;
             a3.x0 = dzc; a3.y = dz; a3.V = Vl(i + 1);
@@ -1610,6 +1627,18 @@
     RU_REQUIRE(dy && dx && N > 0 && C > 0 && D > 0 && H > 0 && W > 0, "ru_upsample2x_trilinear_bwd_l: bad argument");
     return up2_bwd16_launch(dy, dx, N, C, D, H, W, (hipStream_t)stream);
 }
+extern "C" int ru_upsample2x_trilinear_fwd_half_l(const float* x, float* p, int N, int C, int D, int H, int W, ru_stream_t stream) {
+    RU_REQUIRE(x && p && N > 0 && C > 0 && D > 0 && H > 0 && W > 0, "ru_upsample2x_trilinear_fwd_half_l: bad argument");
+    return up2_fwd16_half_launch(x, p, N, C, D, H, W, (hipStream_t)stream);
+}
+extern "C" int ru_upsample2x_trilinear_half_expand_l(const float* p, float* y, int N, int C, int D, int H, int W, float out_slope, ru_stream_t stream) {
+    RU_REQUIRE(p && y && N > 0 && C > 0 && D > 0 && H > 0 && W > 0, "ru_upsample2x_trilinear_half_expand_l: bad argument");
+    return up2_half_expand16_launch(p, y, N, C, D, H, W, out_slope, (hipStream_t)stream);
+}
+extern "C" int ru_upsample2x_trilinear_bwd_hx_l(const float* dh, float* dx, int N, int C, int D, int H, int W, ru_stream_t stream) {
+    RU_REQUIRE(dh && dx && N > 0 && C > 0 && D > 0 && H > 0 && W > 0, "ru_upsample2x_trilinear_bwd_hx_l: bad argument");
+    return up2_bwd16_hx_launch(dh, dx, N, C, D, H, W, (hipStream_t)stream);
+}
 extern "C" int ru_conv3d_fwd_l(const float* x, const float* w, const float* bias, float* y, int N, int Cin, int Cout, int D, int H, int W,
                                int flags, void* ws, size_t ws_bytes, ru_stream_t stream) {
     RU_REQUIRE(x && w && y, "ru_conv3d_fwd_l: null argument");
@@ -1669,10 +1698,32 @@
 extern "C" size_t ru_conv1_l_workspace_bytes(int C0, int Cout, int s2d) {
     return 4096 + (s2d ? 2 * align_up((size_t)C0 * Cout * sizeof(float), 256) : 0);
 }
+static int conv1_l_run(const float* x0, int C0, const float* x1, int C1, const float* w, int ldw, float* y, float* y1, int Cout0,
+                       const float* add, float out_slope, const float* mask, float mask_slope, int N, int Cout, size_t V,
+                       int s2d, int Dc, int Hc, int Wc, const float* bst_y, const float* bst_k, float bst_slope,
+                       float* stat_partials, size_t stat_floats, int* nblk, int* inst, void* ws, size_t ws_bytes, ru_stream_t stream,
+                       int x1h_D, int x1h_H, int x1h_W, float x1h_slope);
 extern "C" int ru_conv1_l(const float* x0, int C0, const float* x1, int C1, const float* w, int ldw, float* y, float* y1, int Cout0,
                           const float* add, float out_slope, const float* mask, float mask_slope, int N, int Cout, size_t V,
                           int s2d, int Dc, int Hc, int Wc, const float* bst_y, const float* bst_k, float bst_slope,
                           float* stat_partials, size_t stat_floats, int* nblk, int* inst, void* ws, size_t ws_bytes, ru_stream_t stream) {
+    return conv1_l_run(x0, C0, x1, C1, w, ldw, y, y1, Cout0, add, out_slope, mask, mask_slope, N, Cout, V, s2d, Dc, Hc, Wc, bst_y, bst_k, bst_slope,
+                       stat_partials, stat_floats, nblk, inst, ws, ws_bytes, stream, 0, 0, 0, 1.f);
+}
+extern "C" int ru_conv1_uph_l(const float* x0, int C0, const float* x1, int C1, const float* w, int ldw, float* y, float* y1, int Cout0,
+                              const float* add, float out_slope, const float* mask, float mask_slope, int N, int Cout, size_t V,
+                              int s2d, int Dc, int Hc, int Wc, const float* bst_y, const float* bst_k, float bst_slope,
+                              float* stat_partials, size_t stat_floats, int* nblk, int* inst, void* ws, size_t ws_bytes, ru_stream_t stream,
+                              int x1h_D, int x1h_H, int x1h_W, float x1h_slope) {
+    RU_REQUIRE(x1 && x1h_D > 0 && x1h_H > 0 && x1h_W > 0, "ru_conv1_uph_l: bad argument");
+    return conv1_l_run(x0, C0, x1, C1, w, ldw, y, y1, Cout0, add, out_slope, mask, mask_slope, N, Cout, V, s2d, Dc, Hc, Wc, bst_y, bst_k, bst_slope,
+                       stat_partials, stat_floats, nblk, inst, ws, ws_bytes, stream, x1h_D, x1h_H, x1h_W, x1h_slope);
+}
+static int conv1_l_run(const float* x0, int C0, const float* x1, int C1, const float* w, int ldw, float* y, float* y1, int Cout0,
+                       const float* add, float out_slope, const float* mask, float mask_slope, int N, int Cout, size_t V,
+                       int s2d, int Dc, int Hc, int Wc, const float* bst_y, const float* bst_k, float bst_slope,
+                       float* stat_partials, size_t stat_floats, int* nblk, int* inst, void* ws, size_t ws_bytes, ru_stream_t stream,
+                       int x1h_D, int x1h_H, int x1h_W, float x1h_slope) {
     RU_REQUIRE(x0 && w && y, "ru_conv1_l: null argument");
     RU_REQUIRE(s2d >= 0 && s2d <= 2, "ru_conv1_l: s2d is 0 (plain), 1 (gather) or 2 (scatter)");
     hipStream_t s = (hipStream_t)stream;
@@ -1681,6 +1732,7 @@
     a.x0 = x0; a.C0 = C0; a.x1 = x1; a.C1 = C1; a.wT = w; a.ldw = ldw; a.y = y; a.add = add; a.out_slope = out_slope;
     a.N = N; a.Cout = Cout; a.V = V; a.s2d = s2d; a.Dc = Dc; a.Hc = Hc; a.Wc = Wc; a.mask = mask; a.mask_slope = mask_slope;
     a.y1 = y1; a.Cout0 = Cout0; a.bst_y = bst_y; a.bst_k = bst_k; a.bst_slope = bst_slope; a.stat_partials = stat_partials;
+    if (x1h_D > 0) { a.x1_half = 1; a.x1h_D = x1h_D; a.x1h_plane = (size_t)4 * x1h_H * x1h_W; a.x1h_slope = x1h_slope; }
     if (s2d) {
         RU_REQUIRE(C0 > 0 && Cout > 0 && (s2d == 1 ? C0 : Cout) % 8 == 0, "ru_conv1_l: stride-2 modes need 8 x channels on the gathered side");
         const int co = s2d == 1 ? Cout : C0, ci = (s2d == 1 ? C0 : Cout) / 8;
@@ -1763,15 +1815,38 @@
 }
 
 extern "C" size_t ru_wgrad1_l_workspace_bytes(int N, int Cin, int Cout, size_t V) { return 4096 + align_up(wgrad1_workspace_bytes(N, Cin, Cout, V), 256); }
+static int wgrad1_l_run(const float* x, const float* x1, int C0, const float* dy, float* dw, int ldw, int N, int Cin, int Cout, size_t V,
+                        int c16, int s2d, int Dc, int Hc, int Wc, int tap_split, const float* dg_w, int dg_ldw, float* dg_y0, float* dg_y1,
+                        float dg_mask_slope, int* inst, void* ws, size_t ws_bytes, ru_stream_t stream,
+                        int x1h_D, int x1h_H, int x1h_W, float x1h_slope, int half_x);
 extern "C" int ru_wgrad1_l(const float* x, const float* x1, int C0, const float* dy, float* dw, int ldw, int N, int Cin, int Cout, size_t V,
                            int c16, int s2d, int Dc, int Hc, int Wc, int tap_split, const float* dg_w, int dg_ldw, float* dg_y0, float* dg_y1,
                            float dg_mask_slope, int* inst, void* ws, size_t ws_bytes, ru_stream_t stream) {
+    return wgrad1_l_run(x, x1, C0, dy, dw, ldw, N, Cin, Cout, V, c16, s2d, Dc, Hc, Wc, tap_split, dg_w, dg_ldw, dg_y0, dg_y1, dg_mask_slope, inst, ws, ws_bytes, stream,
+                        0, 0, 0, 1.f, 0);
+}
+extern "C" int ru_wgrad1_uph_l(const float* x, const float* x1, int C0, const float* dy, float* dw, int ldw, int N, int Cin, int Cout, size_t V,
+                               int c16, int s2d, int Dc, int Hc, int Wc, int tap_split, const float* dg_w, int dg_ldw, float* dg_y0, float* dg_y1,
+                               float dg_mask_slope, int* inst, void* ws, size_t ws_bytes, ru_stream_t stream,
+                               int x1h_D, int x1h_H, int x1h_W, float x1h_slope, int half_x) {
+    RU_REQUIRE(x1 && x1h_D > 0 && x1h_H > 0 && x1h_W > 0, "ru_wgrad1_uph_l: bad argument");
+    return wgrad1_l_run(x, x1, C0, dy, dw, ldw, N, Cin, Cout, V, c16, s2d, Dc, Hc, Wc, tap_split, dg_w, dg_ldw, dg_y0, dg_y1, dg_mask_slope, inst, ws, ws_bytes, stream,
+                        x1h_D, x1h_H, x1h_W, x1h_slope, half_x);
+}
+static int wgrad1_l_run(const float* x, const float* x1, int C0, const float* dy, float* dw, int ldw, int N, int Cin, int Cout, size_t V,
+                        int c16, int s2d, int Dc, int Hc, int Wc, int tap_split, const float* dg_w, int dg_ldw, float* dg_y0, float* dg_y1,
+                        float dg_mask_slope, int* inst, void* ws, size_t ws_bytes, ru_stream_t stream,
+                        int x1h_D, int x1h_H, int x1h_W, float x1h_slope, int half_x) {
     RU_REQUIRE(x && dy && dw, "ru_wgrad1_l: null argument");
     WsCarver C(ws, ws_bytes);
     Wgrad1Args a{};
     a.x = x; a.x1 = x1; a.C0 = C0; a.dy = dy; a.dw = dw; a.ldw = ldw; a.N = N; a.Cin = Cin; a.Cout = Cout; a.V = V;
     a.c16 = c16; a.s2d = s2d; a.Dc = Dc; a.Hc = Hc; a.Wc = Wc; a.tap_split = tap_split;
     a.dg_w = dg_w; a.dg_ldw = dg_ldw; a.dg_y0 = dg_y0; a.dg_y1 = dg_y1; a.dg_mask_slope = dg_mask_slope;
+    if (x1h_D > 0) {
+        a.x1_half = 1; a.x1h_D = x1h_D; a.x1h_plane = (size_t)4 * x1h_H * x1h_W; a.x1h_slope = x1h_slope;
+        a.dg_hx = half_x && dg_w && wgrad1_hx_usable(x1h_W); a.dg_hx_W = x1h_W;
+    }
     RU_REQUIRE(N > 0 && Cin > 0 && Cout > 0 && V > 0, "ru_wgrad1_l: bad shape");
     a.ws_bytes = wgrad1_workspace_bytes(N, Cin, Cout, V);
     a.ws = C.take(a.ws_bytes / 4);
diff --git a/brats2019_amd/csrc/pointwise_c16.hip b/brats2019_amd/csrc/pointwise_c16.hip
--- a/brats2019_amd/csrc/pointwise_c16.hip
+++ b/brats2019_amd/csrc/pointwise_c16.hip
@@ -265,6 +265,80 @@
     return RU_OK;
 }
 
+__global__ __launch_bounds__(256) void up2_fwd16_half_kernel(const float* __restrict__ x, float* __restrict__ p, int D, int H, int W) {
+    const int Ho = 2 * H, Wo = 2 * W;
+    const size_t nb = blockIdx.y;
+    const size_t Vi = (size_t)D * H * W, Vp = Vi * 4;
+    const float4* xp = reinterpret_cast<const float4*>(x) + nb * Vi * 4;
+    float4* pp = reinterpret_cast<float4*>(p) + nb * Vp * 4;
+    const bool nt_out = (size_t)gridDim.y * Vp * 16 * sizeof(float) >= ((size_t)128 << 20);
+    const size_t total = (size_t)D * (H + 1) * Wo * 4;
+    for (size_t f = (size_t)blockIdx.x * 256 + threadIdx.x; f < total; f += (size_t)gridDim.x * 256) {
+        const int q = (int)(f & 3);
+        size_t r = f >> 2;
+        const int xo = (int)(r % Wo); r /= Wo;
+        const int ky = (int)(r % (H + 1)) - 1;
+        const int kz = (int)(r / (H + 1));
+        int x0, x1; float lx0, lx1;
+        up2_src(xo, W, x0, x1, lx0, lx1);
+        const int yA = ky < 0 ? 0 : ky, yB = ky + 1 > H - 1 ? H - 1 : ky + 1;
+        const size_t rA = ((size_t)kz * H + yA) * W, rB = ((size_t)kz * H + yB) * W;
+        const float4 a0 = xp[(rA + x0) * 4 + q], b0 = xp[(rA + x1) * 4 + q];
+        const float4 a1 = xp[(rB + x0) * 4 + q], b1 = xp[(rB + x1) * 4 + q];
+        float4 e0, e1;
+#define RU_UPX(c) e0.c = fmaf(lx0, a0.c, __fmul_rn(lx1, b0.c)); e1.c = fmaf(lx0, a1.c, __fmul_rn(lx1, b1.c))
+        RU_UPX(x); RU_UPX(y); RU_UPX(z); RU_UPX(w);
+#undef RU_UPX
+#pragma unroll
+        for (int dy = 0; dy < 2; ++dy) {
+            const int yo = 2 * ky + 1 + dy;
+            if (yo < 0 || yo >= Ho) continue;
+            int y0, y1; float ly0, ly1;
+            up2_src(yo, H, y0, y1, ly0, ly1);
+            float4 o;
+#define RU_UP2(c) o.c = fmaf(ly1, e1.c, __fmul_rn(ly0, e0.c))
+            RU_UP2(x); RU_UP2(y); RU_UP2(z); RU_UP2(w);
+#undef RU_UP2
+            const size_t idx = (((size_t)kz * Ho + yo) * Wo + xo) * 4 + q;
+            if (nt_out) __builtin_nontemporal_store(f32x4_c16{o.x, o.y, o.z, o.w}, reinterpret_cast<f32x4_c16*>(pp + idx));
+            else pp[idx] = o;
+        }
+    }
+}
+int up2_fwd16_half_launch(const float* x, float* p, int N, int C, int D, int H, int W, hipStream_t s) {
+    RU_REQUIRE(C % 16 == 0, "up2_fwd16_half: C must be a multiple of 16");
+    const size_t total = (size_t)D * (H + 1) * (2 * W) * 4;
+    size_t bx = (total + 255) / 256;
+    if (bx > 16384) bx = 16384;
+    hipLaunchKernelGGL(up2_fwd16_half_kernel, dim3((unsigned)bx, (unsigned)(N * (C / 16))), dim3(256), 0, s, x, p, D, H, W);
+    RU_CHECK_LAUNCH("up2_fwd16_half_kernel");
+    return RU_OK;
+}
+__global__ __launch_bounds__(256) void up2_half_expand16_kernel(const float* __restrict__ p, float* __restrict__ y, int D, size_t plane, float slope) {
+    const size_t nb = blockIdx.y;
+    const float4* pp = reinterpret_cast<const float4*>(p) + nb * D * plane * 4;
+    float4* yp = reinterpret_cast<float4*>(y) + nb * 2 * D * plane * 4;
+    const size_t total = (size_t)2 * D * plane * 4;
+    for (size_t f = (size_t)blockIdx.x * 256 + threadIdx.x; f < total; f += (size_t)gridDim.x * 256) {
+        const int zo = (int)(f / (plane * 4));
+        const size_t in = f - (size_t)zo * plane * 4;
+        int zA, zB; float lz0, lz1;
+        up2_src(zo, D, zA, zB, lz0, lz1);
+        const float4 a = pp[(size_t)zA * plane * 4 + in], b = pp[(size_t)zB * plane * 4 + in];
+        yp[f] = make_float4(up2_zstep(lz0, a.x, lz1, b.x, slope), up2_zstep(lz0, a.y, lz1, b.y, slope),
+                            up2_zstep(lz0, a.z, lz1, b.z, slope), up2_zstep(lz0, a.w, lz1, b.w, slope));
+    }
+}
+int up2_half_expand16_launch(const float* p, float* y, int N, int C, int D, int H, int W, float slope, hipStream_t s) {
+    RU_REQUIRE(C % 16 == 0, "up2_half_expand16: C must be a multiple of 16");
+    const size_t plane = (size_t)4 * H * W, total = 2 * D * plane * 4;
+    size_t bx = (total + 255) / 256;
+    if (bx > 16384) bx = 16384;
+    hipLaunchKernelGGL(up2_half_expand16_kernel, dim3((unsigned)bx, (unsigned)(N * (C / 16))), dim3(256), 0, s, p, y, D, plane, slope);
+    RU_CHECK_LAUNCH("up2_half_expand16_kernel");
+    return RU_OK;
+}
+
 #ifndef RU_UP2B_ZC
 #define RU_UP2B_ZC 8
 #endif
@@ -331,6 +405,62 @@
     RU_CHECK_LAUNCH("up2_bwd16_kernel");
     return RU_OK;
 }
+__global__ __launch_bounds__(256) void up2_bwd16_hx_kernel(const float* __restrict__ dh, float* __restrict__ dx, int D, int H, int W) {
+    const int Do = 2 * D, Ho = 2 * H;
+    const size_t nb = blockIdx.y;
+    const size_t Vi = (size_t)D * H * W, Vh = Vi * 4;
+    const float4* dp = reinterpret_cast<const float4*>(dh) + nb * Vh * 4;
+    float4* op = reinterpret_cast<float4*>(dx) + nb * Vi * 4;
+    const int nch = (D + UP2B_ZC - 1) / UP2B_ZC;
+    const size_t total = (size_t)nch * H * W * 4;
+    for (size_t f = (size_t)blockIdx.x * 256 + threadIdx.x; f < total; f += (size_t)gridDim.x * 256) {
+        const int q = (int)(f & 3);
+        size_t r = f >> 2;
+        const int kx = (int)(r % W); r /= W;
+        const int ky = (int)(r % H);
+        const int k0 = (int)(r / H) * UP2B_ZC;
+        const int k1 = k0 + UP2B_ZC < D ? k0 + UP2B_ZC : D;
+        float wy[4];
+        size_t oy[4];
+#pragma unroll
+        for (int t = 0; t < 4; ++t) {
+            const int y = 2 * ky - 1 + t;
+            wy[t] = (y >= 0 && y < Ho) ? up2_coef(y, H, ky) : 0.f;
+            oy[t] = ((size_t)(y < 0 ? 0 : (y >= Ho ? Ho - 1 : y)) * W + kx) * 4 + q;
+        }
+        float4 accP = make_float4(0.f, 0.f, 0.f, 0.f), accC = accP;
+        for (int m = k0; m <= k1; ++m) {
+#pragma unroll
+            for (int h = 0; h < 2; ++h) {
+                const int z = 2 * m - 1 + h;
+                const bool in = z >= 0 && z < Do;
+                const float4* pl = dp + (size_t)(z < 0 ? 0 : (z >= Do ? Do - 1 : z)) * Ho * W * 4;
+                float4 pz = make_float4(0.f, 0.f, 0.f, 0.f);
+#pragma unroll
+                for (int b = 0; b < 4; ++b) {
+                    const float4 hv = pl[oy[b]];
+                    pz.x = fmaf(wy[b], hv.x, pz.x); pz.y = fmaf(wy[b], hv.y, pz.y); pz.z = fmaf(wy[b], hv.z, pz.z); pz.w = fmaf(wy[b], hv.w, pz.w);
+                }
+                const float cP = (in && m - 1 >= k0) ? up2_coef(z, D, m - 1) : 0.f;
+                const float cC = (in && m < k1) ? up2_coef(z, D, m) : 0.f;
+                accP.x = fmaf(cP, pz.x, accP.x); accP.y = fmaf(cP, pz.y, accP.y); accP.z = fmaf(cP, pz.z, accP.z); accP.w = fmaf(cP, pz.w, accP.w);
+                accC.x = fmaf(cC, pz.x, accC.x); accC.y = fmaf(cC, pz.y, accC.y); accC.z = fmaf(cC, pz.z, accC.z); accC.w = fmaf(cC, pz.w, accC.w);
+            }
+            if (m - 1 >= k0) op[(((size_t)(m - 1) * H + ky) * W + kx) * 4 + q] = accP;
+            accP = accC;
+            accC = make_float4(0.f, 0.f, 0.f, 0.f);
+        }
+    }
+}
+int up2_bwd16_hx_launch(const float* dh, float* dx, int N, int C, int D, int H, int W, hipStream_t s) {
+    RU_REQUIRE(C % 16 == 0, "up2_bwd16_hx: C must be a multiple of 16");
+    const size_t total = (size_t)((D + UP2B_ZC - 1) / UP2B_ZC) * H * W * 4;
+    size_t bx = (total + 255) / 256;
+    if (bx > 16384) bx = 16384;
+    hipLaunchKernelGGL(up2_bwd16_hx_kernel, dim3((unsigned)bx, (unsigned)(N * (C / 16))), dim3(256), 0, s, dh, dx, D, H, W);
+    RU_CHECK_LAUNCH("up2_bwd16_hx_kernel");
+    return RU_OK;
+}
 
 __global__ void pack_down16_kernel(const float* __restrict__ w, float* __restrict__ wd, float* __restrict__ wdT, int Cout, int Cin) {
     const int i = blockIdx.x * blockDim.x + threadIdx.x;
@@ -347,9 +477,10 @@
     return RU_OK;
 }
 
-template <int COB, int S2D, int NSLOT, bool PAIR = false>
+template <int COB, int S2D, int NSLOT, bool PAIR = false, bool X1H = false>
 __global__ __launch_bounds__(256, (PAIR || NSLOT > 0) ? 2 : 1) void conv1_16_kernel(const Conv1Args a, int nvt) {
     static_assert(!PAIR || (S2D == 2 && COB == 4 && (NSLOT == 1 || NSLOT == 2)), "paired stores: the scatter mode with statistics, four blocks per workgroup");
+    static_assert(!X1H || (S2D == 0 && NSLOT == 0), "half-depth second operand: the plain mode without statistics");
     constexpr bool BST = NSLOT > 0;
     constexpr int NSL = BST ? NSLOT : 1;
     __shared__ float red[BST ? 4 * NSL * 16 * 2 : 1];
@@ -380,12 +511,21 @@
     if (live) {
     const size_t v0 = (size_t)vt * 64;
     size_t vb[4], fv[4];
+    [[maybe_unused]] size_t hA[4], hB[4];
+    [[maybe_unused]] float hl1[4];
 #pragma unroll
     for (int t = 0; t < 4; ++t) {
         size_t v = v0 + 16 * t + r;
         if (v >= V) v = V - 1;
         vb[t] = v * 16 + 4 * g;
         fv[t] = 0;
+        if constexpr (X1H) {
+            const unsigned plane = (unsigned)a.x1h_plane, zo = (unsigned)v / plane, in = (unsigned)v - zo * plane;
+            int zA, zB; float l0;
+            up2_src((int)zo, a.x1h_D, zA, zB, l0, hl1[t]);
+            hA[t] = ((size_t)((unsigned)zA * plane + in)) * 16 + 4 * g;
+            hB[t] = ((size_t)((unsigned)zB * plane + in)) * 16 + 4 * g;
+        }
         if constexpr (S2D != 0) {
             const int xc = (int)(v % a.Wc);
             const size_t rr = v / a.Wc;
@@ -413,6 +553,17 @@
             const float* src = a.x0 + ((size_t)(n * CBf_in + cbf) * Vf) * 16 + 4 * g;
 #pragma unroll
             for (int t = 0; t < 4; ++t) xb[t] = *reinterpret_cast<const float4*>(src + (fv[t] + toff) * 16);
+        } else if (X1H && kb >= nkb0) {
+            const float* src = a.x1 + ((size_t)(n * nkb1 + kb - nkb0) * (V >> 1)) * 16;
+            float4 pa[4], pb[4];
+#pragma unroll
+            for (int t = 0; t < 4; ++t) { pa[t] = *reinterpret_cast<const float4*>(src + hA[t]); pb[t] = *reinterpret_cast<const float4*>(src + hB[t]); }
+#pragma unroll
+            for (int t = 0; t < 4; ++t) {
+                const float l1 = hl1[t], l0 = 1.f - l1;
+                xb[t] = make_float4(up2_zstep(l0, pa[t].x, l1, pb[t].x, a.x1h_slope), up2_zstep(l0, pa[t].y, l1, pb[t].y, a.x1h_slope),
+                                    up2_zstep(l0, pa[t].z, l1, pb[t].z, a.x1h_slope), up2_zstep(l0, pa[t].w, l1, pb[t].w, a.x1h_slope));
+            }
         } else {
             const float* src = kb < nkb0 ? a.x0 + ((size_t)(n * nkb0 + kb) * V) * 16 : a.x1 + ((size_t)(n * nkb1 + kb - nkb0) * V) * 16;
 #pragma unroll
@@ -664,6 +815,7 @@
 Conv1Inst conv1_16_choose(const Conv1Args& a) {
     const int CBo = a.Cout / 16;
     Conv1Inst c{CBo >= 4 ? 4 : (CBo >= 2 ? 2 : 1), a.s2d, 0, 0};
+    c.x1h = a.x1_half ? 1 : 0;
     if (a.s2d == 2) {
         const int forced = env_c1_scatter_cob();
         if ((forced == 2 || forced == 4 || forced == 1) && forced <= CBo) c.cob = forced;
@@ -696,6 +848,8 @@
     const int nvt = (int)((a.V + 63) / 64), CBo = a.Cout / 16;
     const Conv1Inst c = conv1_16_choose(a);
     const bool bst = a.bst_y != nullptr;
+    RU_REQUIRE(!a.x1_half || (!a.s2d && !bst && a.x1 && a.C1 > 0 && a.x1h_D > 0 && a.x1h_plane > 0 && (size_t)2 * a.x1h_D * a.x1h_plane == a.V && a.V < ((size_t)1 << 31)),
+               "conv1_16: a half-depth second operand needs the plain mode without statistics and V = 2 x depth x plane < 2^31");
     RU_REQUIRE(!bst || (a.bst_k && a.stat_partials && a.s2d != 1 && !a.y1 && conv1_16_bst_nblk(a) > 0), "conv1_16: fused GroupNorm-backward statistics need the plain or scatter mode with whole channel blocks per workgroup");
     dim3 grid((unsigned)cdiv(nvt, 4), (unsigned)cdiv(CBo, c.cob), (unsigned)a.N);
     switch (c.packed()) {
@@ -711,6 +865,12 @@
         RU_C1_CASE(4, 2, 1, 0); RU_C1_CASE(4, 2, 2, 0); RU_C1_CASE(4, 2, 4, 0);
         RU_C1_CASE(2, 2, 1, 0); RU_C1_CASE(2, 2, 2, 0); RU_C1_CASE(1, 2, 1, 0);
 #undef RU_C1_CASE
+#define RU_C1H_CASE(COB_)                                                                                          \
+    case COB_ | (1 << 13):                                                                                          \
+        hipLaunchKernelGGL((conv1_16_kernel<COB_, 0, 0, false, true>), grid, dim3(256), 0, s, a, nvt);              \
+        break
+        RU_C1H_CASE(4); RU_C1H_CASE(2); RU_C1H_CASE(1);
+#undef RU_C1H_CASE
     default:
         set_error("conv1_16: no kernel for cob %d, mode %d, %d statistic slots", c.cob, c.s2d, c.nslot);
         return RU_EINVAL;
diff --git a/brats2019_amd/csrc/pw_helpers.hpp b/brats2019_amd/csrc/pw_helpers.hpp
--- a/brats2019_amd/csrc/pw_helpers.hpp
+++ b/brats2019_amd/csrc/pw_helpers.hpp
@@ -50,6 +50,10 @@
     i1 = i0 + (i0 < n - 1 ? 1 : 0);
 }
 
+__device__ __forceinline__ float up2_zstep(float lz0, float a, float lz1, float b, float slope) {
+    return lrelu(fmaf(lz0, a, __fmul_rn(lz1, b)), slope);
+}
+
 __device__ __forceinline__ float up2_coef(int o, int n, int k) {
     int i0, i1; float l0, l1;
     up2_src(o, n, i0, i1, l0, l1);
diff --git a/brats2019_amd/csrc/ru_common.h b/brats2019_amd/csrc/ru_common.h
--- a/brats2019_amd/csrc/ru_common.h
+++ b/brats2019_amd/csrc/ru_common.h
@@ -268,7 +268,12 @@
     float* dg_y0;
     float* dg_y1;
     float dg_mask_slope;
-};
+    int x1_half, x1h_D;
+    size_t x1h_plane;
+    float x1h_slope;
+    int dg_hx, dg_hx_W;
+};
+bool wgrad1_hx_usable(int W);
 size_t wgrad1_workspace_bytes(int N, int Cin, int Cout, size_t V);
 int wgrad1_launch(const Wgrad1Args& a, hipStream_t s);
 int wgrad1_inst(const Wgrad1Args& a);
@@ -292,6 +297,9 @@
     const float* bst_k;
     float bst_slope;
     float* stat_partials;
+    int x1_half, x1h_D;
+    size_t x1h_plane;
+    float x1h_slope;
 };
 int conv1_16_bst_nblk(const Conv1Args& a);
 int conv1_launch(const Conv1Args& a, hipStream_t s);
@@ -342,9 +350,12 @@
                           int N, int C, size_t V, int split, hipStream_t s);
 int up2_fwd16_launch(const float* x, float* y, int N, int C, int D, int H, int W, float slope, hipStream_t s);
 int up2_bwd16_launch(const float* dy, float* dx, int N, int C, int D, int H, int W, hipStream_t s);
+int up2_fwd16_half_launch(const float* x, float* p, int N, int C, int D, int H, int W, hipStream_t s);
+int up2_bwd16_hx_launch(const float* dh, float* dx, int N, int C, int D, int H, int W, hipStream_t s);
+int up2_half_expand16_launch(const float* p, float* y, int N, int C, int D, int H, int W, float slope, hipStream_t s);
 int pack_down16_launch(const float* w, float* wd, float* wdT, int Cout, int Cin, hipStream_t s);
 int conv1_16_launch(const Conv1Args& a, hipStream_t s);
-struct Conv1Inst { int cob, s2d, nslot, pair; int packed() const { return cob | (s2d << 4) | (nslot << 8) | (pair << 12); } };
+struct Conv1Inst { int cob, s2d, nslot, pair, x1h = 0; int packed() const { return cob | (s2d << 4) | (nslot << 8) | (pair << 12) | (x1h << 13); } };
 Conv1Inst conv1_16_choose(const Conv1Args& a);
 
 int crit_tiles(size_t total);
diff --git a/brats2019_amd/csrc/wgrad_f32.hip b/brats2019_amd/csrc/wgrad_f32.hip
--- a/brats2019_amd/csrc/wgrad_f32.hip
+++ b/brats2019_amd/csrc/wgrad_f32.hip
@@ -1,4 +1,5 @@
 #include "ru_common.h"
+#include "pw_helpers.hpp"
 
 namespace ru {
 
@@ -409,7 +410,7 @@
 constexpr int W1_VC = 256;
 constexpr int W1_RS = pad2mod4(W1_VC);
 
-template <int OT, int CT>
+template <int OT, int CT, bool XH = false, bool HX = false>
 __global__ __launch_bounds__(256, 2) void wgrad1_f32_kernel(const Wgrad1Args a, float* __restrict__ partials,
                                                            int nchunk, int ncg, int CoP, int CiP) {
     extern __shared__ __attribute__((aligned(16))) float smem[];
@@ -444,6 +445,20 @@
             float4 dv[ND], xv[NX];
             const int xCB0 = a.x1 ? a.C0 >> 4 : a.Cin >> 4, xCB1 = a.x1 ? (a.Cin - a.C0) >> 4 : 1;
             const float* xsecond = a.x1 ? a.x1 : a.x;
+            [[maybe_unused]] unsigned hoA[4], hoB[4];
+            [[maybe_unused]] float hl0[4], hl1[4];
+            if constexpr (XH) {
+                const unsigned plane = (unsigned)a.x1h_plane;
+#pragma unroll
+                for (int k = 0; k < 4; ++k) {
+                    const size_t vk = v0 + (tid >> 2) + 64 * k;
+                    const unsigned vv = vk < V ? (unsigned)vk : 0u;
+                    const unsigned zo = vv / plane, in = vv - zo * plane;
+                    int zA, zB;
+                    up2_src((int)zo, a.x1h_D, zA, zB, hl0[k], hl1[k]);
+                    hoA[k] = (unsigned)zA * plane + in; hoB[k] = (unsigned)zB * plane + in;
+                }
+            }
 #pragma unroll
             for (int j = 0; j < ND; ++j) {
                 const int e4 = tid + j * 256, q = e4 & 3, r = (e4 >> 2) % W1_VC, p = e4 / (4 * W1_VC);
@@ -472,7 +487,18 @@
                 const bool second = kbx >= xCB0;
                 const float* xsrc = second ? xsecond : a.x;
                 if (!a.s2d) off = (((size_t)n * (second ? xCB1 : xCB0) + (second ? kbx - xCB0 : kbx)) * V + vv) * 16 + 4 * q;
-                const float4 t4 = *reinterpret_cast<const float4*>(xsrc + off);
+                float4 t4;
+                if (XH && second) {
+                    const int k = j & 3;
+                    const float l0 = hl0[k], l1 = hl1[k];
+                    const float* pb = xsecond + ((size_t)n * xCB1 + (kbx - xCB0)) * (V >> 1) * 16 + 4 * q;
+                    const float4 pa4 = *reinterpret_cast<const float4*>(pb + (size_t)hoA[k] * 16);
+                    const float4 pb4 = *reinterpret_cast<const float4*>(pb + (size_t)hoB[k] * 16);
+                    t4 = make_float4(up2_zstep(l0, pa4.x, l1, pb4.x, a.x1h_slope), up2_zstep(l0, pa4.y, l1, pb4.y, a.x1h_slope),
+                                     up2_zstep(l0, pa4.z, l1, pb4.z, a.x1h_slope), up2_zstep(l0, pa4.w, l1, pb4.w, a.x1h_slope));
+                } else {
+                    t4 = *reinterpret_cast<const float4*>(xsrc + off);
+                }
                 xv[j] = ok ? t4 : make_float4(0.f, 0.f, 0.f, 0.f);
             }
 #pragma unroll
@@ -549,6 +575,7 @@
         }
         if (dgrad) {
             const int xCB0 = a.x1 ? a.C0 >> 4 : a.Cin >> 4, xCB1 = a.x1 ? (a.Cin - a.C0) >> 4 : 1;
+            [[maybe_unused]] f32x4 hx[4][CT];
 #pragma unroll
             for (int vt = 0; vt < 4; ++vt) {
                 const int vl = wave * 64 + vt * 16 + (lane & 15);
@@ -565,9 +592,56 @@
 #pragma unroll
                         for (int r = 0; r < 4; ++r) d[r] = xs[(q * 16 + 4 * (lane >> 4) + r) * W1_RS + vl] > 0.f ? d[r] : d[r] * a.dg_mask_slope;
                     }
+                    if constexpr (HX) {
+                        hx[vt][q] = d;
+                        if (second) continue;
+                    }
                     float* dst = second ? a.dg_y1 : a.dg_y0;
                     const size_t idx = (((size_t)n * (second ? xCB1 : xCB0) + (second ? kb - xCB0 : kb)) * V + v) * 16 + 4 * (lane >> 4);
                     if (v < V && kb < (a.Cin >> 4)) *reinterpret_cast<float4*>(dst + idx) = make_float4(d[0], d[1], d[2], d[3]);
+                }
+            }
+            if constexpr (HX) {
+                float* ex = dys;
+                const int cb0 = c0 >> 4, sb0 = cb0 > xCB0 ? cb0 : xCB0;
+                __syncthreads();
+#pragma unroll
+                for (int vt = 0; vt < 4; ++vt) {
+                    const int vl = wave * 64 + vt * 16 + (lane & 15);
+#pragma unroll
+                    for (int q = 0; q < CT; ++q) {
+                        const int kb = cb0 + q;
+                        if (kb < xCB0) continue;
+                        *reinterpret_cast<float4*>(ex + ((size_t)((kb - sb0) * W1_VC + vl)) * 16 + 4 * (lane >> 4)) = make_float4(hx[vt][q][0], hx[vt][q][1], hx[vt][q][2], hx[vt][q][3]);
+                    }
+                }
+                __syncthreads();
+                const int Wc = a.dg_hx_W, Wo = 2 * Wc;
+#pragma unroll
+                for (int q = 0; q < CT; ++q) {
+                    const int kb = cb0 + q;
+                    if (kb < xCB0) continue;
+                    const float* et = ex + (size_t)(kb - sb0) * W1_VC * 16;
+#pragma unroll
+                    for (int k = 0; k < 2; ++k) {
+                        const int e = tid + k * 256, qd = e & 3, hl = e >> 2;
+                        const int rl = hl / Wc, kx = hl - rl * Wc;
+                        float wx[4];
+                        float4 pv[4];
+#pragma unroll
+                        for (int t4 = 0; t4 < 4; ++t4) {
+                            const int xx = 2 * kx - 1 + t4;
+                            wx[t4] = (xx >= 0 && xx < Wo) ? up2_coef(xx, Wc, kx) : 0.f;
+                            const int xc = xx < 0 ? 0 : (xx >= Wo ? Wo - 1 : xx);
+                            pv[t4] = *reinterpret_cast<const float4*>(et + (size_t)(rl * Wo + xc) * 16 + 4 * qd);
+                        }
+                        float4 o;
+#define RU_HX(c) o.c = fmaf(wx[3], pv[3].c, fmaf(wx[2], pv[2].c, fmaf(wx[0], pv[0].c, __fmul_rn(wx[1], pv[1].c))))
+                        RU_HX(x); RU_HX(y); RU_HX(z); RU_HX(w);
+#undef RU_HX
+                        const size_t idx = (((size_t)n * xCB1 + (kb - xCB0)) * (V >> 1) + (v0 >> 1) + hl) * 16 + 4 * qd;
+                        if (v0 + (size_t)rl * Wo < V && kb < (a.Cin >> 4)) *reinterpret_cast<float4*>(a.dg_y1 + idx) = o;
+                    }
                 }
             }
         }
@@ -742,25 +816,27 @@
     return (size_t)nbx * round_up(Cout, 16) * round_up(Cin, 16) * sizeof(float);
 }
 
-template <int OT, int CT>
+template <int OT, int CT, bool XH = false, bool HX = false>
 static int wgrad1_cfg(const Wgrad1Args& a, const W1Choice& c, hipStream_t s) {
     static PerDevice attr_done;
     const size_t lds = (size_t)(OT + CT) * 16 * W1_RS * sizeof(float);
     if (!attr_done.get()) {
-        hipError_t e = hipFuncSetAttribute(reinterpret_cast<const void*>(wgrad1_f32_kernel<OT, CT>),
+        hipError_t e = hipFuncSetAttribute(reinterpret_cast<const void*>(wgrad1_f32_kernel<OT, CT, XH, HX>),
                                            hipFuncAttributeMaxDynamicSharedMemorySize, (int)lds);
         if (e != hipSuccess) return hip_fail(e, "hipFuncSetAttribute(wgrad1)");
         attr_done.set();
     }
     const int CoP = round_up(a.Cout, 16), CiP = round_up(a.Cin, 16);
-    hipLaunchKernelGGL((wgrad1_f32_kernel<OT, CT>), dim3(c.nbx, c.ngroups), dim3(256), lds, s, a, (float*)a.ws, c.nchunk, c.ncg, CoP, CiP);
+    hipLaunchKernelGGL((wgrad1_f32_kernel<OT, CT, XH, HX>), dim3(c.nbx, c.ngroups), dim3(256), lds, s, a, (float*)a.ws, c.nchunk, c.ncg, CoP, CiP);
     RU_CHECK_LAUNCH("wgrad1_f32_kernel");
     return wgrad_reduce_launch((const float*)a.ws, c.nbx, 1, CoP, CiP, a.Cout, a.Cin, a.dw, a.ldw, 1, a.tap_split, s, 0, a.defer);
 }
 
+bool wgrad1_hx_usable(int W) { return W > 0 && W1_VC % (2 * W) == 0; }
+
 int wgrad1_inst(const Wgrad1Args& a) {
     const W1Choice c = wgrad1_choose(a.N, a.Cin, a.Cout, a.V);
-    return c.ot | (c.ct << 4) | ((a.s2d && wgrad1_s2d_usable(a.Cin, a.Cout)) ? 256 : 0) | (a.dg_w ? 512 : 0);
+    return c.ot | (c.ct << 4) | ((a.s2d && wgrad1_s2d_usable(a.Cin, a.Cout)) ? 256 : 0) | (a.dg_w ? 512 : 0) | (a.x1_half ? 1024 : 0) | (a.dg_hx ? 2048 : 0);
 }
 
 int wgrad1_launch(const Wgrad1Args& a, hipStream_t s) {
@@ -768,6 +844,10 @@
     RU_REQUIRE(!a.c16 || (a.Cin % 16 == 0 && a.Cout % 16 == 0), "wgrad1: C16 tensors need channel counts that are multiples of 16");
     RU_REQUIRE(!a.s2d || (a.c16 && a.Cin % 128 == 0 && (size_t)a.Dc * a.Hc * a.Wc == a.V), "wgrad1: bad stride-2 geometry");
     RU_REQUIRE(!a.x1 || (a.c16 && !a.s2d && a.C0 > 0 && a.C0 < a.Cin && a.C0 % 16 == 0), "wgrad1: a second input tensor needs voxel-major tensors and a split at a multiple of 16");
+    RU_REQUIRE(!a.x1_half || (a.x1 && a.x1h_D > 0 && a.x1h_plane > 0 && (size_t)2 * a.x1h_D * a.x1h_plane == a.V && a.V < ((size_t)1 << 31)),
+               "wgrad1: a half-depth second input needs V = 2 x depth x plane < 2^31");
+    RU_REQUIRE(!a.dg_hx || (a.x1_half && a.dg_w && a.dg_y1 && wgrad1_hx_usable(a.dg_hx_W) && a.V % (size_t)(2 * a.dg_hx_W) == 0 && a.Cin == 2 * a.Cout && a.C0 == a.Cout),
+               "wgrad1: the half-x data gradient needs the half-depth second input, the fused data gradient of a concat of two Cout-channel halves, and rows that divide a 256-voxel chunk");
     const W1Choice c = wgrad1_choose(a.N, a.Cin, a.Cout, a.V);
     RU_REQUIRE(!a.dg_w || (a.c16 && !a.s2d && a.Cout == c.ot * 16 && a.Cin % (c.ct * 16) == 0 && a.dg_y0 && (a.dg_y1 || !a.x1) && a.dg_ldw >= a.Cin),
                "wgrad1: the fused data gradient needs voxel-major tensors, Cout <= 32 and whole channel tiles");
@@ -789,6 +869,13 @@
         RU_CHECK_LAUNCH("wgrad1_s2d_kernel");
         return wgrad_reduce_launch((const float*)a.ws, nbx, 1, a.Cout, a.Cin, a.Cout, a.Cin, a.dw, a.ldw, 1, a.tap_split, s, 0, a.defer);
     }
+    if (a.x1_half) {
+        switch (inst & 255) {
+        case 2 | (2 << 4): return a.dg_hx ? wgrad1_cfg<2, 2, true, true>(a, c, s) : wgrad1_cfg<2, 2, true>(a, c, s);
+        case 1 | (2 << 4): return a.dg_hx ? wgrad1_cfg<1, 2, true, true>(a, c, s) : wgrad1_cfg<1, 2, true>(a, c, s);
+        default: set_error("wgrad1: no kernel with a half-depth second input for these channel counts"); return RU_EINVAL;
+        }
+    }
     switch (inst & 255) {
     case 2 | (2 << 4): return wgrad1_cfg<2, 2>(a, c, s);
     case 2 | (1 << 4): return wgrad1_cfg<2, 1>(a, c, s);
diff --git a/brats2019_amd/engine.py b/brats2019_amd/engine.py
--- a/brats2019_amd/engine.py
+++ b/brats2019_amd/engine.py
@@ -72,10 +72,12 @@
         L.check(L.load().ru_unet_set_grad_precision(self.h, L.GRAD_PRECISIONS[grad_precision]), "ru_unet_set_grad_precision")
         self.grad_precision = grad_precision
 
-    def set_fusion(self, gn_bwd_stats=True, gn_bwd_apply=True, side_stream=True, batch_wreduce=True, tail_finalize=False, pw_dgrad=True):
+    def set_fusion(self, gn_bwd_stats=True, gn_bwd_apply=True, side_stream=True, batch_wreduce=True, tail_finalize=False, pw_dgrad=True, up_half=False):
         mask = ((L.FUSE_GN_BWD_STATS if gn_bwd_stats else 0) | (L.FUSE_GN_BWD_APPLY if gn_bwd_apply else 0) | (L.FUSE_SIDE_STREAM if side_stream else 0) |
                 (L.FUSE_BATCH_WREDUCE if batch_wreduce else 0) | (L.FUSE_TAIL_FINALIZE if tail_finalize else 0) | (L.FUSE_PW_DGRAD if pw_dgrad else 0))
         L.check(L.load().ru_unet_set_fusion(self.h, mask), "ru_unet_set_fusion")
+        if up_half:
+            L.check(L.load().ru_unet_set_up_half(self.h, 1), "ru_unet_set_up_half")
         self._ws_key = None
 
     FAMILIES = ("conv3_l0", "conv3_deep", "wgrad3_l0", "wgrad3_deep", "groupnorm", "pointwise_1x1_s2_up", "other")
diff --git a/brats2019_amd/ops.py b/brats2019_amd/ops.py
--- a/brats2019_amd/ops.py
+++ b/brats2019_amd/ops.py
@@ -803,6 +803,31 @@
     return dx
 
 
+def upsample2x_half_c16(x):
+    x = _prep(x)
+    n, cb, d, h, w, _ = (int(v) for v in x.shape)
+    p = torch.empty((n, cb, d, 2 * h, 2 * w, 16), dtype=torch.float32, device=x.device)
+    L.check(L.load().ru_upsample2x_trilinear_fwd_half_l(L.f32(x), L.f32(p), n, cb * 16, d, h, w, L.stream()), "ru_upsample2x_trilinear_fwd_half_l")
+    return p
+
+
+def upsample2x_half_expand_c16(p, out_slope=1.0):
+    p = _prep(p)
+    n, cb, d, h2, w2, _ = (int(v) for v in p.shape)
+    y = torch.empty((n, cb, 2 * d, h2, w2, 16), dtype=torch.float32, device=p.device)
+    L.check(L.load().ru_upsample2x_trilinear_half_expand_l(L.f32(p), L.f32(y), n, cb * 16, d, h2 // 2, w2 // 2, float(out_slope), L.stream()),
+            "ru_upsample2x_trilinear_half_expand_l")
+    return y
+
+
+def upsample2x_bwd_hx_c16(dh):
+    dh = _prep(dh)
+    n, cb, d2, h2, w, _ = (int(v) for v in dh.shape)
+    dx = torch.empty((n, cb, d2 // 2, h2 // 2, w, 16), dtype=torch.float32, device=dh.device)
+    L.check(L.load().ru_upsample2x_trilinear_bwd_hx_l(L.f32(dh), L.f32(dx), n, cb * 16, d2 // 2, h2 // 2, w, L.stream()), "ru_upsample2x_trilinear_bwd_hx_l")
+    return dx
+
+
 def to_split_c16(x_c16):
     hi = x_c16.to(torch.bfloat16)
     lo = (x_c16 - hi.to(torch.float32)).to(torch.bfloat16)
@@ -856,11 +881,14 @@
 
 
 def conv1x1_c16(x0, w, x1=None, add=None, out_slope=1.0, mask=None, mask_slope=LEAKY_SLOPE, cout0=0, s2d=0,
-                bst_y=None, bst_k=None, bst_slope=LEAKY_SLOPE):
+                bst_y=None, bst_k=None, bst_slope=LEAKY_SLOPE, x1_half_slope=None):
     x0, w, x1, add, mask, bst_y, bst_k = (_prep(t) for t in (x0, w, x1, add, mask, bst_y, bst_k))
     lib = L.load()
     n, cb0, d, h, wd, _ = (int(v) for v in x0.shape)
     c0, c1 = cb0 * 16, (int(x1.shape[1]) * 16 if x1 is not None else 0)
+    uph = x1_half_slope is not None
+    if uph and (x1 is None or tuple(x1.shape[2:5]) != (d // 2, h, wd)):
+        raise ValueError("a half-depth x1 is [N, C1/16, D/2, H, W, 16]")
     dc, hc, wc, ldw = d, h, wd, 0
     if s2d == 0:
         cout, ldw = int(w.shape[0]), int(w.shape[1])
@@ -886,31 +914,46 @@
         part = torch.zeros(cap, dtype=torch.float32, device=dev)
     ws = L.workspace(lib.ru_conv1_l_workspace_bytes(c0, cout, s2d), dev)
     nblk, inst = C.c_int(0), C.c_int(0)
-    L.check(lib.ru_conv1_l(L.f32(x0), c0, L.ptr(x1, True), c1, L.f32(w), ldw, L.f32(y), L.ptr(y1, True), cout0, L.ptr(add, True), float(out_slope),
-                           L.ptr(mask, True), float(mask_slope), n, cout, v, s2d, dc, hc, wc, L.ptr(bst_y, True), L.ptr(bst_k, True), float(bst_slope),
-                           L.ptr(part, True), cap, C.byref(nblk), C.byref(inst), L.ptr(ws), ws.numel(), L.stream()), "ru_conv1_l")
+    args = (L.f32(x0), c0, L.ptr(x1, True), c1, L.f32(w), ldw, L.f32(y), L.ptr(y1, True), cout0, L.ptr(add, True), float(out_slope),
+            L.ptr(mask, True), float(mask_slope), n, cout, v, s2d, dc, hc, wc, L.ptr(bst_y, True), L.ptr(bst_k, True), float(bst_slope),
+            L.ptr(part, True), cap, C.byref(nblk), C.byref(inst), L.ptr(ws), ws.numel(), L.stream())
+    if uph:
+        L.check(lib.ru_conv1_uph_l(*args, d // 2, h // 2, wd // 2, float(x1_half_slope)), "ru_conv1_uph_l")
+    else:
+        L.check(lib.ru_conv1_l(*args), "ru_conv1_l")
     if part is not None:
         part = part[:n * cstat * nblk.value * 2].view(n, cstat, nblk.value, 2)
     return Conv1Result(y, y1, part, nblk.value, inst.value)
 
 
-def conv1x1_bwd_weight_c16(x, dy, x1=None, ldw=None, s2d=False, tap_split=False, dg_w=None, dg_mask_slope=LEAKY_SLOPE):
+def conv1x1_bwd_weight_c16(x, dy, x1=None, ldw=None, s2d=False, tap_split=False, dg_w=None, dg_mask_slope=LEAKY_SLOPE, x1_half_slope=None, half_x=False):
     x, dy, x1, dg_w = (_prep(t) for t in (x, dy, x1, dg_w))
     lib = L.load()
     n, cbo, d, h, wd, _ = (int(v) for v in dy.shape)
     c0 = int(x.shape[1]) * 16
     cin = 8 * c0 if s2d else c0 + (int(x1.shape[1]) * 16 if x1 is not None else 0)
     cout, v = cbo * 16, d * h * wd
+    uph = x1_half_slope is not None
+    if uph and (x1 is None or tuple(x1.shape[2:5]) != (d // 2, h, wd)):
+        raise ValueError("a half-depth x1 is [N, C1/16, D/2, H, W, 16]")
     ldw = cin if ldw is None else int(ldw)
     dev = x.device
     dw = torch.zeros((cout, cin // 8, 2, 2, 2) if tap_split else (cout, ldw), dtype=torch.float32, device=dev)
     dx0 = torch.empty_like(x) if dg_w is not None else None
     dx1 = torch.empty_like(x1) if dg_w is not None and x1 is not None else None
+    if uph and dx1 is not None:
+        dx1 = torch.empty((n, int(x1.shape[1]), d, h, wd, 16), dtype=torch.float32, device=dev)
     ws = L.workspace(lib.ru_wgrad1_l_workspace_bytes(n, cin, cout, v), dev)
     inst = C.c_int(0)
-    L.check(lib.ru_wgrad1_l(L.f32(x), L.ptr(x1, True), c0 if x1 is not None else 0, L.f32(dy), L.f32(dw), ldw, n, cin, cout, v, 1, int(bool(s2d)), d, h, wd,
-                            cin // 8 if tap_split else 0, L.ptr(dg_w, True), int(dg_w.shape[1]) if dg_w is not None else 0, L.ptr(dx0, True), L.ptr(dx1, True),
-                            float(dg_mask_slope), C.byref(inst), L.ptr(ws), ws.numel(), L.stream()), "ru_wgrad1_l")
+    args = (L.f32(x), L.ptr(x1, True), c0 if x1 is not None else 0, L.f32(dy), L.f32(dw), ldw, n, cin, cout, v, 1, int(bool(s2d)), d, h, wd,
+            cin // 8 if tap_split else 0, L.ptr(dg_w, True), int(dg_w.shape[1]) if dg_w is not None else 0, L.ptr(dx0, True), L.ptr(dx1, True),
+            float(dg_mask_slope), C.byref(inst), L.ptr(ws), ws.numel(), L.stream())
+    if uph:
+        L.check(lib.ru_wgrad1_uph_l(*args, d // 2, h // 2, wd // 2, float(x1_half_slope), int(bool(half_x))), "ru_wgrad1_uph_l")
+        if dx1 is not None and inst.value & 2048:
+            dx1 = dx1.reshape(-1)[:dx1.numel() // 2].view(n, int(x1.shape[1]), d, h, wd // 2, 16)
+    else:
+        L.check(lib.ru_wgrad1_l(*args), "ru_wgrad1_l")
     return Wgrad1Result(dw, dx0, dx1, inst.value)
 
 
diff --git a/include/resunet_hip.h b/include/resunet_hip.h
--- a/include/resunet_hip.h
+++ b/include/resunet_hip.h
@@ -127,7 +127,9 @@
 #define RU_FUSE_BATCH_WREDUCE 8
 #define RU_FUSE_TAIL_FINALIZE 16
 #define RU_FUSE_PW_DGRAD 32
+#define RU_FUSE_UP_HALF 64
 int ru_unet_set_fusion(ru_unet_t h, unsigned mask);
+int ru_unet_set_up_half(ru_unet_t h, int on);
 int ru_unet_probe(ru_unet_t h, int enable);
 int ru_unet_probe_read(ru_unet_t h, double* total_ms, int* launches);
 #define RU_PROBE_FAMILIES 7
@@ -260,6 +262,18 @@
 
 int ru_upsample2x_trilinear_fwd_l(const float* x, float* y, int N, int C, int D, int H, int W, float out_slope, ru_stream_t stream);
 int ru_upsample2x_trilinear_bwd_l(const float* dy, float* dx, int N, int C, int D, int H, int W, ru_stream_t stream);
+int ru_upsample2x_trilinear_fwd_half_l(const float* x, float* p, int N, int C, int D, int H, int W, ru_stream_t stream);
+int ru_upsample2x_trilinear_half_expand_l(const float* p, float* y, int N, int C, int D, int H, int W, float out_slope, ru_stream_t stream);
+int ru_upsample2x_trilinear_bwd_hx_l(const float* dh, float* dx, int N, int C, int D, int H, int W, ru_stream_t stream);
+int ru_conv1_uph_l(const float* x0, int C0, const float* x1, int C1, const float* w, int ldw, float* y, float* y1, int Cout0,
+                   const float* add, float out_slope, const float* mask, float mask_slope, int N, int Cout, size_t V,
+                   int s2d, int Dc, int Hc, int Wc, const float* bst_y, const float* bst_k, float bst_slope,
+                   float* stat_partials, size_t stat_floats, int* nblk, int* inst, void* ws, size_t ws_bytes, ru_stream_t stream,
+                   int x1h_D, int x1h_H, int x1h_W, float x1h_slope);
+int ru_wgrad1_uph_l(const float* x, const float* x1, int C0, const float* dy, float* dw, int ldw, int N, int Cin, int Cout, size_t V,
+                    int c16, int s2d, int Dc, int Hc, int Wc, int tap_split, const float* dg_w, int dg_ldw, float* dg_y0, float* dg_y1,
+                    float dg_mask_slope, int* inst, void* ws, size_t ws_bytes, ru_stream_t stream,
+                    int x1h_D, int x1h_H, int x1h_W, float x1h_slope, int half_x);
 
 int ru_dice_counts(const float* p, const float* g, unsigned long long* counts, int N, int C, size_t V, ru_stream_t stream);
 int ru_dice_accumulate(const unsigned long long* counts, double* acc, int N, int C, int nacc, ru_stream_t stream);
```
